# yoxu515/aot-benchmark

Hardware: NVIDIA H100
Metric: frames/sec (480p, 10 obj) (higher is better)
Workload: dtype f32

## Files before the change

### aot_benchmark_b200/csrc/conv_tc.cu

```cuda
#include <type_traits>

#include "common.cuh"
#include "tc_common.cuh"

namespace aotb {
namespace tc {

constexpr int CONV_A_BYTES = 128 * 128;

template <int BN>
__device__ __forceinline__ void wgmma_conv(float* acc, uint64_t a, uint64_t b) {
    if (BN == 256) wgmma_ss_n256(acc, a, b, 1u);
    else if (BN == 128) wgmma_ss_n128(acc, a, b, 1u);
    else wgmma_ss_n64(acc, a, b, 1u);
}

template <int BN>
__device__ __forceinline__ void conv_acc_to_staging(const float* acc, float* stg, int ld) {
    const int warp = threadIdx.x >> 5, lane = threadIdx.x & 31;
    const int row0 = (warp >> 2) * 64 + (warp & 3) * 16 + (lane >> 2), cq = (lane & 3) * 2;
#pragma unroll
    for (int j = 0; j < BN / 2; j += 2)
        *reinterpret_cast<float2*>(stg + (row0 + 8 * ((j >> 1) & 1)) * ld + 8 * (j >> 2) + cq) = make_float2(acc[j], acc[j + 1]);
}

struct ConvTcArgs {
    const float* in;
    const float* bias;
    const float* wscale;
    const float* res;
    float* out;
    int B, H, W, Cin, ldin;
    int Ho, Wo, Cout, ldout, ldres;
    int KH, KW, stride, pad;
    int M, mtiles, nchunks;
    int act;
    int splits;
    int spin;
    int const_w;
    long long* prof;
};

constexpr int AOTB_CONV_CONST_WEIGHTS = 256;
static int g_conv_tiling = 0;
static int g_conv_grid_cap = 0;

struct RowInfo { int pix_base, iy0, ix0, valid; };

template <int BN, int S, int NB>
__device__ __forceinline__ void conv_finish_tile(const ConvTcArgs& a, const uint8_t* smem, int tid, int m0, int n0, int zrank) {
    constexpr int LD = BN + 4, C4 = BN / 4, RSTEP = 256 / C4, ROWS = 128 / S, ITERS = ROWS / RSTEP;
    constexpr int B = NB < ITERS ? NB : ITERS;
    static_assert(ITERS >= 1 && ITERS % B == 0, "finish tiling");
    const int c = (tid % C4) * 4, n = n0 + c;
    const int r0 = zrank * ROWS + tid / C4;
    const float4 b4 = a.bias ? __ldg(reinterpret_cast<const float4*>(a.bias + n)) : make_float4(0.f, 0.f, 0.f, 0.f);
    const float4 s4 = a.wscale ? __ldg(reinterpret_cast<const float4*>(a.wscale + n)) : make_float4(1.f, 1.f, 1.f, 1.f);
    const float* lbase = reinterpret_cast<const float*>(smem) + r0 * LD + c;
    const uint32_t sbase = smem_u32(lbase);
#pragma unroll 1
    for (int i0 = 0; i0 < ITERS; i0 += B) {
        float4 v[B][S], rs[B];
#pragma unroll
        for (int b = 0; b < B; ++b) {
            const int ro = (i0 + b) * RSTEP;
            if (S == 1) {
                v[b][0] = *reinterpret_cast<const float4*>(lbase + ro * LD);
            } else {
#pragma unroll
                for (int z = 0; z < S; ++z) v[b][z] = dsmem_ld_f4(dsmem_addr(sbase + (uint32_t)(ro * LD) * 4u, (uint32_t)z));
            }
            const int m = m0 + r0 + ro;
            rs[b] = (a.res && m < a.M) ? *reinterpret_cast<const float4*>(a.res + (size_t)m * a.ldres + n)
                                       : make_float4(0.f, 0.f, 0.f, 0.f);
        }
#pragma unroll
        for (int b = 0; b < B; ++b) {
            float4 o = v[b][0];
#pragma unroll
            for (int z = 1; z < S; ++z) { o.x += v[b][z].x; o.y += v[b][z].y; o.z += v[b][z].z; o.w += v[b][z].w; }
            o.x = fmaf(o.x, s4.x, b4.x); o.y = fmaf(o.y, s4.y, b4.y); o.z = fmaf(o.z, s4.z, b4.z); o.w = fmaf(o.w, s4.w, b4.w);
            o.x += rs[b].x; o.y += rs[b].y; o.z += rs[b].z; o.w += rs[b].w;
            o.x = apply_act(o.x, a.act); o.y = apply_act(o.y, a.act);
            o.z = apply_act(o.z, a.act); o.w = apply_act(o.w, a.act);
            const int m = m0 + r0 + (i0 + b) * RSTEP;
            if (m < a.M) *reinterpret_cast<float4*>(a.out + (size_t)m * a.ldout + n) = o;
        }
    }
}

__device__ __forceinline__ void prefetch_l1(const void* p) { asm volatile("prefetch.global.L1 [%0];" ::"l"(p)); }

template <int BN, int ACT>
__device__ __forceinline__ void conv_finish_frag(const ConvTcArgs& a, float* acc, const float* bs, int m0, int n0) {
    constexpr bool ROLL = ACT == ACT_GELU || ACT == ACT_SILU;
    constexpr int G = (ROLL || BN == 256) ? 1 : 8, NG = BN / 8, PF = 8;
    const int warp = threadIdx.x >> 5, lane = threadIdx.x & 31;
    const int r = m0 + (warp >> 2) * 64 + (warp & 3) * 16 + (lane >> 2);
    const int c = (lane & 3) * 2;
    const bool ok[2] = {r < a.M, r + 8 < a.M};
    auto res_at = [&](int h, int k) { return a.res + (size_t)(r + 8 * h) * a.ldres + n0 + c + 8 * k; };
    auto prefetch = [&](int k) {
        if (G == 1 && a.res && k < NG) {
            if (ok[0]) prefetch_l1(res_at(0, k));
            if (ok[1]) prefetch_l1(res_at(1, k));
        }
    };
    auto group = [&](int k, int h, float a0, float a1, float2 rs) {
        const int n = c + 8 * k;
        const float2 b2 = *reinterpret_cast<const float2*>(bs + n), s2 = *reinterpret_cast<const float2*>(bs + BN + n);
        float ox = fmaf(a0, s2.x, b2.x), oy = fmaf(a1, s2.y, b2.y);
        ox += rs.x; oy += rs.y;
        ox = apply_act(ox, ACT); oy = apply_act(oy, ACT);
        if (ok[h]) *reinterpret_cast<float2*>(a.out + (size_t)(r + 8 * h) * a.ldout + n0 + n) = make_float2(ox, oy);
    };
#pragma unroll
    for (int k = 0; k < PF; ++k) prefetch(k);
    if constexpr (ROLL) {
#pragma unroll 1
        for (int k = 0; k < NG; ++k) {
            prefetch(k + PF);
            float2 rs[2];
#pragma unroll
            for (int h = 0; h < 2; ++h)
                rs[h] = (a.res && ok[h]) ? *reinterpret_cast<const float2*>(res_at(h, k)) : make_float2(0.f, 0.f);
#pragma unroll
            for (int h = 0; h < 2; ++h) group(k, h, acc[2 * h], acc[2 * h + 1], rs[h]);
#pragma unroll
            for (int i = 0; i < BN / 2 - 4; ++i) acc[i] = acc[i + 4];
        }
    } else {
#pragma unroll
        for (int k0 = 0; k0 < NG; k0 += G) {
            prefetch(k0 + PF);
            float2 rs[G][2];
#pragma unroll
            for (int k = 0; k < G; ++k)
#pragma unroll
                for (int h = 0; h < 2; ++h)
                    rs[k][h] = (a.res && ok[h]) ? *reinterpret_cast<const float2*>(res_at(h, k0 + k)) : make_float2(0.f, 0.f);
#pragma unroll
            for (int k = 0; k < G; ++k)
#pragma unroll
                for (int h = 0; h < 2; ++h) group(k0 + k, h, acc[4 * (k0 + k) + 2 * h], acc[4 * (k0 + k) + 2 * h + 1], rs[k][h]);
        }
    }
}

template <int BN, int STAGES, bool SPLIT, bool PERSIST>
struct ConvSmem {
    static constexpr int A_BYTES = CONV_A_BYTES;
    static constexpr int B_BYTES = BN * 128;
    static constexpr int PARTS = SPLIT ? 2 : 1;
    static constexpr int STAGE_BYTES = PARTS * A_BYTES + PARTS * B_BYTES;
    static constexpr int STG_LD = BN + 4;
    static_assert(128 * STG_LD * 4 <= STAGES * STAGE_BYTES, "staging tile must fit in the operand stages");
    static constexpr int RTABLES = PERSIST ? 2 : 1, BS_FLOATS = PERSIST ? 2 * 2 * BN : 0;
    static constexpr int TOTAL = STAGES * STAGE_BYTES + RTABLES * 128 * (int)sizeof(RowInfo) + BS_FLOATS * 4 + 3 * STAGES * 8 + 1024;
    static_assert(TOTAL <= 227 * 1024, "shared memory of one CTA");
};

template <int BN, int STAGES, bool SPLIT, bool PERSIST>
__global__ void __launch_bounds__(384, 1)
conv_tc_kernel(const __grid_constant__ CUtensorMap tmWh, const __grid_constant__ CUtensorMap tmWl, const ConvTcArgs a) {
    using SM = ConvSmem<BN, STAGES, SPLIT, PERSIST>;
    extern __shared__ uint8_t smem_raw[];
    uint8_t* smem = reinterpret_cast<uint8_t*>((reinterpret_cast<uintptr_t>(smem_raw) + 1023) & ~(uintptr_t)1023);
    RowInfo* rinfo = reinterpret_cast<RowInfo*>(smem + STAGES * SM::STAGE_BYTES);
    float* bsm = reinterpret_cast<float*>(rinfo + SM::RTABLES * 128);
    uint64_t* a_full = reinterpret_cast<uint64_t*>(bsm + SM::BS_FLOATS);
    uint64_t* b_full = a_full + STAGES;
    uint64_t* s_free = b_full + STAGES;

    const int tid = threadIdx.x, warp = tid >> 5;
    const int ntn = a.Cout / BN, ntiles = a.mtiles * ntn;
    const int ntc = !PERSIST ? 1 : (int)blockIdx.x < ntiles ? (ntiles - 1 - (int)blockIdx.x) / (int)gridDim.x + 1 : 0;
    auto tile_m0 = [&](int j) {
        if constexpr (PERSIST) return ((int)(blockIdx.x + j * gridDim.x) / ntn) * 128;
        else return (int)blockIdx.x * 128;
    };
    auto tile_n0 = [&](int j) {
        if constexpr (PERSIST) return ((int)(blockIdx.x + j * gridDim.x) % ntn) * BN;
        else return (int)blockIdx.y * BN;
    };
    long long* prof = a.prof ? a.prof + 12 * ((size_t)(blockIdx.z * gridDim.y + blockIdx.y) * gridDim.x + blockIdx.x) : nullptr;
    auto stamp = [&](int slot) { if (prof) prof[slot] = clock64(); };
    if (tid == 0) stamp(0);
    pdl_trigger();

    const int per = PERSIST ? a.nchunks : (a.nchunks + a.splits - 1) / a.splits;
    const int kbeg = PERSIST ? 0 : blockIdx.z * per;
    const int nloc = max(0, min(per, a.nchunks - kbeg));
    const int nchk = ntc * nloc;
    const int npre = a.const_w ? min(STAGES, nchk) : 0;
    auto issue_b = [&](int g) {
        const int j = PERSIST ? g / nloc : 0, it = g - j * nloc, s = g % STAGES;
        uint8_t* Bh = smem + s * SM::STAGE_BYTES + SM::PARTS * SM::A_BYTES;
        mbar_arrive_expect_tx(&b_full[s], SM::PARTS * SM::B_BYTES);
        tma_load_2d(Bh, &tmWh, &b_full[s], (kbeg + it) * 64, tile_n0(j));
        if constexpr (SPLIT) tma_load_2d(Bh + SM::B_BYTES, &tmWl, &b_full[s], (kbeg + it) * 64, tile_n0(j));
    };
    auto write_rows = [&](int j, int p) {
        const int m = tile_m0(j) + p;
        RowInfo ri;
        if (m < a.M) {
            const int HoWo = a.Ho * a.Wo;
            const int b = m / HoWo, r = m - b * HoWo;
            const int oy = r / a.Wo, ox = r - oy * a.Wo;
            ri.pix_base = b * a.H * a.W;
            ri.iy0 = oy * a.stride - a.pad;
            ri.ix0 = ox * a.stride - a.pad;
            ri.valid = 1;
        } else {
            ri.pix_base = 0; ri.iy0 = 0; ri.ix0 = 0; ri.valid = 0;
        }
        rinfo[(j & 1) * 128 + p] = ri;
    };

    if (tid == 0) {
        for (int s = 0; s < STAGES; ++s) { mbar_init(&a_full[s], 128); mbar_init(&b_full[s], 1); mbar_init(&s_free[s], 8); }
        fence_mbar_init();
    }
    if (tid >= 256) {
        for (int j = 0; j < min(ntc, 2); ++j) write_rows(j, tid - 256);
    }
    __syncthreads();
    if (tid == 0) stamp(1);
    if (tid == 256) {
        tma_prefetch_desc(&tmWh);
        if constexpr (SPLIT) tma_prefetch_desc(&tmWl);
        for (int g = 0; g < npre; ++g) issue_b(g);
    }
    pdl_wait();
    const int cpt = (a.Cin % 64 == 0) ? (a.Cin >> 6) : 0;

    const int wg = __shfl_sync(0xffffffffu, tid >> 7, 0);
    if (wg < 2) {
        const uint64_t dA0 = smem_desc_sw128(smem_u32(smem + wg * 64 * 128));
        const uint64_t dB0 = smem_desc_sw128(smem_u32(smem + SM::PARTS * SM::A_BYTES));
        int g = 0;
#pragma unroll 1
        for (int j = 0; j < ntc; ++j) {
            float acc[BN / 2];
#pragma unroll
            for (int i = 0; i < BN / 2; ++i) acc[i] = 0.f;
            float* bs = bsm + (j & 1) * 2 * BN;
            if (PERSIST && tid < BN) {
                const int n = tile_n0(j) + tid;
                bs[tid] = a.bias ? __ldg(a.bias + n) : 0.f;
                bs[BN + tid] = a.wscale ? __ldg(a.wscale + n) : 1.f;
            }
#pragma unroll 1
            for (int it = 0; it < nloc; ++it, ++g) {
                const int s = g % STAGES;
                const uint32_t ph = (g / STAGES) & 1;
                mbar_wait_cp(&a_full[s], ph, a.spin);
                mbar_wait_cp(&b_full[s], ph, a.spin);
                if (g == 0 && tid == 0) stamp(3);
                const uint64_t so = (uint64_t)((s * SM::STAGE_BYTES) >> 4);
                const uint64_t ah = dA0 + so, al = ah + (SM::A_BYTES >> 4), bh = dB0 + so, bl = bh + (uint64_t)(SM::B_BYTES >> 4);
                reg_fence<BN / 2>(acc);
                wgmma_fence();
#pragma unroll
                for (int ks = 0; ks < 4; ++ks) {
                    wgmma_conv<BN>(acc, ah + 2 * ks, bh + 2 * ks);
                    if constexpr (SPLIT) {
                        wgmma_conv<BN>(acc, al + 2 * ks, bh + 2 * ks);
                        wgmma_conv<BN>(acc, ah + 2 * ks, bl + 2 * ks);
                    }
                }
                wgmma_commit();
                reg_fence<BN / 2>(acc);
                wgmma_wait<1>();
                if (it > 0) mbar_arrive_warp(&s_free[(g - 1) % STAGES]);
            }
            wgmma_wait<0>();
            reg_fence<BN / 2>(acc);
            if (tid == 0) { if (PERSIST && j == 0) stamp(10); stamp(4); }
            if constexpr (PERSIST) {
                if (nloc > 0) mbar_arrive_warp(&s_free[(g - 1) % STAGES]);
                asm volatile("bar.sync 1, 256;" ::: "memory");
                const int m0 = tile_m0(j), n0 = tile_n0(j);
                switch (a.act) {
                    case ACT_RELU: conv_finish_frag<BN, ACT_RELU>(a, acc, bs, m0, n0); break;
                    case ACT_GELU: conv_finish_frag<BN, ACT_GELU>(a, acc, bs, m0, n0); break;
                    case ACT_SILU: conv_finish_frag<BN, ACT_SILU>(a, acc, bs, m0, n0); break;
                    case ACT_RELU6: conv_finish_frag<BN, ACT_RELU6>(a, acc, bs, m0, n0); break;
                    default: conv_finish_frag<BN, ACT_NONE>(a, acc, bs, m0, n0); break;
                }
                if (tid == 0) { if (j == 0) stamp(8); stamp(9); }
            } else {
                asm volatile("bar.sync 1, 256;" ::: "memory");
                conv_acc_to_staging<BN>(acc, reinterpret_cast<float*>(smem), SM::STG_LD);
                if (tid == 0) stamp(6);
            }
        }
    } else {
        const int p = tid - 256, q = p & 15, rsub = p >> 4;
        const uint32_t soff = rsub * 128 + (((q >> 1) ^ rsub) << 4) + ((q & 1) << 3);
        const float4* in4 = reinterpret_cast<const float4*>(a.in);
        uint32_t off[16];
        int cur_tap = -1, c4 = 0;
        const RowInfo* rows = rinfo;
        auto load_half = [&](int h, auto part_c, float4* v) {
            constexpr int part = decltype(part_c)::value;
            if (part == 0) {
                const int g = h >> 1, j = PERSIST ? g / nloc : 0, it = g - j * nloc;
                if (PERSIST && it == 0) {
                    cur_tap = -1;
                    rows = rinfo + (j & 1) * 128;
                    if (j > 0) {
                        asm volatile("bar.sync 2, 128;" ::: "memory");
                        if (j + 1 < ntc) write_rows(j + 1, p);
                    }
                }
                const int kc = kbeg + it;
                int tap, c0;
                if (cpt > 0) { tap = kc / cpt; c0 = ((kc - tap * cpt) << 6) + q * 4; }
                else { const int k = kc * 64 + q * 4; tap = k / a.Cin; c0 = k - tap * a.Cin; }
                c4 = c0 >> 2;
                if (tap != cur_tap) {
                    cur_tap = tap;
                    const bool kvalid = tap < a.KH * a.KW;
                    const int ky = tap / a.KW, kx = tap - ky * a.KW;
#pragma unroll
                    for (int i = 0; i < 16; ++i) {
                        const RowInfo ri = rows[rsub + i * 8];
                        const int iy = ri.iy0 + ky, ix = ri.ix0 + kx;
                        off[i] = (kvalid && ri.valid && iy >= 0 && iy < a.H && ix >= 0 && ix < a.W)
                                     ? (uint32_t)(((size_t)(ri.pix_base + iy * a.W + ix) * a.ldin) >> 2)
                                     : ~0u;
                    }
                }
            }
#pragma unroll
            for (int i = 0; i < 8; ++i) {
                const uint32_t o = off[part * 8 + i];
                v[i] = o != ~0u ? __ldg(in4 + ((size_t)o + c4)) : make_float4(0.f, 0.f, 0.f, 0.f);
            }
        };
        auto store_half = [&](int h, auto part_c, const float4* v) {
            constexpr int part = decltype(part_c)::value;
            const int g = h >> 1, s = g % STAGES;
            uint8_t* stage = smem + s * SM::STAGE_BYTES;
            if (part == 0) {
                if (g >= STAGES) mbar_wait_cp(&s_free[s], ((g / STAGES) - 1) & 1, a.spin);
                if (p == 0 && g >= npre) issue_b(g);
            }
            uint8_t* Ah = stage + part * 64 * 128 + soff;
            uint8_t* Al = Ah + SM::A_BYTES;
#pragma unroll
            for (int i = 0; i < 8; ++i) {
                const __half2 h0 = __floats2half2_rn(v[i].x, v[i].y), h1 = __floats2half2_rn(v[i].z, v[i].w);
                if constexpr (!SPLIT) {
                    uint2 ph;
                    ph.x = *reinterpret_cast<const uint32_t*>(&h0); ph.y = *reinterpret_cast<const uint32_t*>(&h1);
                    *reinterpret_cast<uint2*>(Ah + i * 1024) = ph;
                    continue;
                }
                const __half2 l0 = __floats2half2_rn(v[i].x - __low2float(h0), v[i].y - __high2float(h0));
                const __half2 l1 = __floats2half2_rn(v[i].z - __low2float(h1), v[i].w - __high2float(h1));
                uint2 ph, pl;
                ph.x = *reinterpret_cast<const uint32_t*>(&h0); ph.y = *reinterpret_cast<const uint32_t*>(&h1);
                pl.x = *reinterpret_cast<const uint32_t*>(&l0); pl.y = *reinterpret_cast<const uint32_t*>(&l1);
                *reinterpret_cast<uint2*>(Ah + i * 1024) = ph;
                *reinterpret_cast<uint2*>(Al + i * 1024) = pl;
            }
            if (part == 1) {
                fence_proxy_async();
                mbar_arrive(&a_full[s]);
                if (g == 0 && p == 0) stamp(2);
            }
        };
        using P0 = std::integral_constant<int, 0>;
        using P1 = std::integral_constant<int, 1>;
        const int nh = 2 * nchk;
        float4 v0[8], v1[8], v2[8];
        if (nh > 0) { load_half(0, P0{}, v0); load_half(1, P1{}, v1); }
#pragma unroll 1
        for (int h = 0; h < nh; h += 6) {
            if (h + 2 < nh) load_half(h + 2, P0{}, v2);
            store_half(h, P0{}, v0);
            if (h + 3 < nh) load_half(h + 3, P1{}, v0);
            store_half(h + 1, P1{}, v1);
            if (h + 2 < nh) {
                if (h + 4 < nh) load_half(h + 4, P0{}, v1);
                store_half(h + 2, P0{}, v2);
                if (h + 5 < nh) load_half(h + 5, P1{}, v2);
                store_half(h + 3, P1{}, v0);
            }
            if (h + 4 < nh) {
                if (h + 6 < nh) load_half(h + 6, P0{}, v0);
                store_half(h + 4, P0{}, v1);
                if (h + 7 < nh) load_half(h + 7, P1{}, v1);
                store_half(h + 5, P1{}, v2);
            }
        }
        if (p == 0) stamp(5);
    }
    if constexpr (!PERSIST) {
        __syncwarp();
        cluster_sync_all();
        if (tid == 0) stamp(8);
        if (warp < 8) {
            const int zr = (int)blockIdx.z, m0 = tile_m0(0), n0 = tile_n0(0);
            if (a.splits == 2) conv_finish_tile<BN, 2, 4>(a, smem, tid, m0, n0, zr);
            else if (a.splits == 4) conv_finish_tile<BN, 4, 2>(a, smem, tid, m0, n0, zr);
            else conv_finish_tile<BN, 8, 2>(a, smem, tid, m0, n0, zr);
        }
        if (tid == 0) stamp(9);
        __syncwarp();
        cluster_sync_all();
    } else if (tid == 0 && prof) {
        prof[11] = ntc;
    }
    if (tid == 0) stamp(7);
}

static int make_tmap_weights(CUtensorMap* out, const void* base, int Kpad, int Cout, int BN) {
    PFN_encodeTiled fn = tensor_map_encoder();
    if (!fn) return AOTB_ERR_CUDA;
    cuuint64_t dims[2] = {(cuuint64_t)Kpad, (cuuint64_t)Cout};
    cuuint64_t strides[1] = {(cuuint64_t)Kpad * 2};
    cuuint32_t box[2] = {64, (cuuint32_t)BN};
    cuuint32_t estr[2] = {1, 1};
    CUresult r = fn(out, CU_TENSOR_MAP_DATA_TYPE_FLOAT16, 2, const_cast<void*>(base), dims, strides, box, estr,
                    CU_TENSOR_MAP_INTERLEAVE_NONE, CU_TENSOR_MAP_SWIZZLE_128B, CU_TENSOR_MAP_L2_PROMOTION_L2_256B,
                    CU_TENSOR_MAP_FLOAT_OOB_FILL_NONE);
    if (r != CUDA_SUCCESS) {
        set_error("cuTensorMapEncodeTiled(weights) failed (%d)", (int)r);
        return AOTB_ERR_CUDA;
    }
    return AOTB_OK;
}

static int sm_count() {
    static int n = 0;
    if (n == 0) {
        int dev = 0;
        if (cudaGetDevice(&dev) != cudaSuccess || cudaDeviceGetAttribute(&n, cudaDevAttrMultiProcessorCount, dev) != cudaSuccess)
            n = 132;
    }
    return n;
}

static dim3 conv_grid(const ConvTcArgs& a, int BN) {
    if (a.splits > 1) return dim3(a.mtiles, a.Cout / BN, a.splits);
    const int cap = g_conv_grid_cap > 0 ? g_conv_grid_cap : sm_count();
    return dim3(min(a.mtiles * (a.Cout / BN), cap), 1, 1);
}

template <int BN, int STAGES, bool SPLIT, bool PERSIST>
static int launch_conv_tc_as(const CUtensorMap& th, const CUtensorMap& tl, const ConvTcArgs& a, cudaStream_t st) {
    constexpr int smem = ConvSmem<BN, STAGES, SPLIT, PERSIST>::TOTAL;
    static bool configured = false;
    if (!configured) {
        cudaError_t e = cudaFuncSetAttribute(conv_tc_kernel<BN, STAGES, SPLIT, PERSIST>,
                                             cudaFuncAttributeMaxDynamicSharedMemorySize, smem);
        if (e != cudaSuccess) {
            set_error("aotb_conv2d_nhwc_tc: cudaFuncSetAttribute: %s", cudaGetErrorString(e));
            return AOTB_ERR_CUDA;
        }
        configured = true;
    }
    launch_cluster(conv_tc_kernel<BN, STAGES, SPLIT, PERSIST>, conv_grid(a, BN), dim3(384), smem, st, a.splits, th, tl, a);
    return check_launch("aotb_conv2d_nhwc_tc");
}

template <int BN, int STAGES, bool SPLIT>
static int launch_conv_tc(const CUtensorMap& th, const CUtensorMap& tl, const ConvTcArgs& a, cudaStream_t st) {
    return a.splits > 1 ? launch_conv_tc_as<BN, STAGES, SPLIT, false>(th, tl, a, st)
                        : launch_conv_tc_as<BN, STAGES, SPLIT, true>(th, tl, a, st);
}

}
}

using namespace aotb;

extern "C" int aotb_set_conv_tiling(int mode) {
    AOTB_REQUIRE(mode >= 0 && mode < (1 << 12), "aotb_set_conv_tiling: mode is a 12-bit mask");
    tc::g_conv_tiling = mode;
    return AOTB_OK;
}

extern "C" int aotb_set_conv_grid_cap(int ctas) {
    AOTB_REQUIRE(ctas >= 0, "aotb_set_conv_grid_cap: negative cap");
    tc::g_conv_grid_cap = ctas;
    return AOTB_OK;
}

extern "C" int aotb_conv2d_nhwc_tc(const float* in, const void* wh, const void* wl, const float* bias, const float* wscale,
                                   const float* res, float* out, int B, int H, int W, int Cin, int ldin, int Cout, int ldout, int ldres,
                                   int KH, int KW, int stride, int pad, int act, void* workspace, size_t workspace_bytes,
                                   void* stream) {
    AOTB_REQUIRE(in && wh && out, "aotb_conv2d_nhwc_tc: null pointer");
    const bool split = wl != nullptr;
    const int const_w = (act & tc::AOTB_CONV_CONST_WEIGHTS) ? 1 : 0;
    act &= ~tc::AOTB_CONV_CONST_WEIGHTS;
    AOTB_REQUIRE(Cin % 4 == 0 && Cout % 64 == 0, "aotb_conv2d_nhwc_tc: Cin must be a multiple of 4, Cout of 64");
    AOTB_REQUIRE(act >= aotb::ACT_NONE && act <= aotb::ACT_RELU6, "aotb_conv2d_nhwc_tc: activation %d not supported (0-4)", act);
    AOTB_REQUIRE(ldin % 4 == 0 && ldout % 4 == 0 && (!res || ldres % 4 == 0) && ((uintptr_t)in % 16 == 0) &&
                     ((uintptr_t)out % 16 == 0) && (!res || (uintptr_t)res % 16 == 0) && (!bias || (uintptr_t)bias % 16 == 0) &&
                     (!wscale || (uintptr_t)wscale % 16 == 0),
                 "aotb_conv2d_nhwc_tc: 16-byte alignment required");
    AOTB_REQUIRE((size_t)B * H * W * ldin / 4 < 0xFFFFFFFFull, "aotb_conv2d_nhwc_tc: input larger than 2^32 float4");
    tc::ConvTcArgs a;
    a.in = in; a.bias = bias; a.wscale = wscale; a.res = res; a.out = out;
    a.B = B; a.H = H; a.W = W; a.Cin = Cin; a.ldin = ldin;
    a.Ho = (H + 2 * pad - KH) / stride + 1;
    a.Wo = (W + 2 * pad - KW) / stride + 1;
    AOTB_REQUIRE(a.Ho > 0 && a.Wo > 0, "aotb_conv2d_nhwc_tc: empty output");
    a.Cout = Cout; a.ldout = ldout; a.ldres = ldres; a.KH = KH; a.KW = KW; a.stride = stride; a.pad = pad;
    a.M = B * a.Ho * a.Wo;
    a.mtiles = cdiv(a.M, 128);
    const int K = ((KH * KW * Cin + 63) / 64) * 64;
    a.nchunks = K / 64;
    a.act = act;
    a.const_w = const_w;
    const int mt = cdiv(a.M, 128);
    int BN = 64, best_s = 1;
    const float kGather = 2.5f, kGather1 = 2.0f;
    if ((tc::g_conv_tiling & 1) == 0) {
        float best = 1e30f;
        const int bns[3] = {256, 128, 64};
        const float t_mma[3] = {4.0f, 2.0f, 1.0f}, t_mma1[3] = {4.0f / 3, 2.0f / 3, 1.0f / 3};
        const float t_fin[3] = {8.0f, 4.0f, 2.0f};
        for (int bi = 0; bi < 3; ++bi) {
            const float tf = t_fin[bi] * (bi == 0 && res ? 2.0f : 1.0f);
            if (Cout % bns[bi]) continue;
            const float tm = split ? t_mma[bi] : t_mma1[bi], tc = fmaxf(split ? kGather : kGather1, tm);
            for (int sp = 1; sp <= 8; sp <<= 1) {
                if (sp > a.nchunks) break;
                const int ctas = mt * (Cout / bns[bi]) * sp;
                const int slots = sp == 8 ? 128 : 132;
                if (sp > 1 && ctas > slots) continue;
                float t;
                if (sp == 1) {
                    const int tpc = cdiv(ctas, 132);
                    t = 3.0f + tpc * a.nchunks * tc + tf + (tpc - 1) * fmaxf(0.f, a.nchunks * (tm - tc) + tf);
                } else {
                    t = cdiv(ctas, slots) * (3.0f + cdiv(a.nchunks, sp) * tc + t_fin[bi]);
                }
                if (t < best) { best = t; BN = bns[bi]; best_s = sp; }
            }
        }
    } else {
        if (Cout % 128 == 0 && mt * (Cout / 128) >= 120) BN = 128;
        const int ctas = mt * (Cout / BN);
        if (ctas < 100 && a.nchunks >= 4) {
            best_s = 8;
            while (best_s > 1 && (ctas * best_s > 160 || a.nchunks / best_s < 2)) best_s >>= 1;
        }
    }
    const int force_bn = (tc::g_conv_tiling >> 4) & 15, force_s = (tc::g_conv_tiling >> 8) & 15;
    if (force_bn) {
        BN = 32 << force_bn;
        AOTB_REQUIRE((BN == 64 || BN == 128 || BN == 256) && Cout % BN == 0, "aotb_conv2d_nhwc_tc: forced tile %d invalid", BN);
    }
    a.splits = force_bn ? 1 : best_s;
    if (force_s) {
        AOTB_REQUIRE((force_s == 1 || force_s == 2 || force_s == 4 || force_s == 8) && force_s <= a.nchunks,
                     "aotb_conv2d_nhwc_tc: forced split %d invalid", force_s);
        a.splits = force_s;
    }
    a.spin = (tc::g_conv_tiling & 2) ? 1 : 0;
    a.prof = nullptr;
    if (tc::g_conv_tiling & 4) {
        const dim3 grid = tc::conv_grid(a, BN);
        const size_t need = (size_t)grid.x * grid.y * grid.z * 12 * sizeof(long long);
        AOTB_REQUIRE(workspace && workspace_bytes >= need, "aotb_conv2d_nhwc_tc: profile mode needs %zu workspace bytes", need);
        a.prof = (long long*)workspace;
    }
    CUtensorMap th, tl;
    int rc;
    if ((rc = tc::make_tmap_weights(&th, wh, K, Cout, BN)) != AOTB_OK) return rc;
    cudaStream_t st = (cudaStream_t)stream;
    if (!split) {
        if (BN == 256) return tc::launch_conv_tc<256, 4, false>(th, th, a, st);
        if (BN == 128) return tc::launch_conv_tc<128, 6, false>(th, th, a, st);
        return tc::launch_conv_tc<64, 8, false>(th, th, a, st);
    }
    if ((rc = tc::make_tmap_weights(&tl, wl, K, Cout, BN)) != AOTB_OK) return rc;
    if (BN == 256) return tc::launch_conv_tc<256, 2, true>(th, tl, a, st);
    if (BN == 128) return tc::launch_conv_tc<128, 3, true>(th, tl, a, st);
    return tc::launch_conv_tc<64, 4, true>(th, tl, a, st);
}
```

### aot_benchmark_b200/csrc/tc_common.cuh

```cuda
#pragma once
#include <cuda.h>
#include <cuda_fp16.h>
#include <cuda_runtime.h>
#include <cstdint>

namespace aotb {
namespace tc {

__device__ __forceinline__ uint32_t smem_u32(const void* p) { return (uint32_t)__cvta_generic_to_shared(p); }

__device__ __forceinline__ bool elect_one() {
    uint32_t pred;
    asm volatile(
        "{\n\t.reg .pred P;\n\telect.sync _|P, 0xffffffff;\n\tselp.b32 %0, 1, 0, P;\n\t}\n" : "=r"(pred));
    return pred != 0;
}

__device__ __forceinline__ void mbar_init(uint64_t* bar, uint32_t count) {
    asm volatile("mbarrier.init.shared::cta.b64 [%0], %1;" ::"r"(smem_u32(bar)), "r"(count) : "memory");
}
__device__ __forceinline__ void fence_mbar_init() { asm volatile("fence.mbarrier_init.release.cluster;" ::: "memory"); }
__device__ __forceinline__ void mbar_arrive_warp(uint64_t* bar) {
    __syncwarp();
    if ((threadIdx.x & 31) == 0) asm volatile("mbarrier.arrive.shared::cta.b64 _, [%0];" ::"r"(smem_u32(bar)) : "memory");
}
__device__ __forceinline__ void mbar_arrive(uint64_t* bar) {
    asm volatile("mbarrier.arrive.shared::cta.b64 _, [%0];" ::"r"(smem_u32(bar)) : "memory");
}
__device__ __forceinline__ void mbar_arrive_expect_tx(uint64_t* bar, uint32_t bytes) {
    asm volatile("mbarrier.arrive.expect_tx.shared::cta.b64 _, [%0], %1;" ::"r"(smem_u32(bar)), "r"(bytes) : "memory");
}
__device__ __forceinline__ void mbar_wait(uint64_t* bar, uint32_t parity) {
    const uint32_t addr = smem_u32(bar);
    uint32_t done = 0;
    uint32_t spins = 0;
    while (true) {
        asm volatile(
            "{\n\t.reg .pred P;\n\tmbarrier.try_wait.parity.shared::cta.b64 P, [%1], %2, %3;\n\tselp.b32 %0, 1, 0, P;\n\t}\n"
            : "=r"(done)
            : "r"(addr), "r"(parity), "r"(20000u)
            : "memory");
        if (done) break;
        if (++spins > (1u << 24)) __trap();
    }
}

__device__ __forceinline__ void mbar_wait_spin(uint64_t* bar, uint32_t parity) {
    const uint32_t addr = smem_u32(bar);
    uint32_t done = 0;
    uint32_t spins = 0;
    while (true) {
        asm volatile(
            "{\n\t.reg .pred P;\n\tmbarrier.try_wait.parity.shared::cta.b64 P, [%1], %2;\n\tselp.b32 %0, 1, 0, P;\n\t}\n"
            : "=r"(done)
            : "r"(addr), "r"(parity)
            : "memory");
        if (done) break;
        if (++spins > (1u << 28)) __trap();
    }
}

__device__ __forceinline__ void mbar_wait_cp(uint64_t* bar, uint32_t parity, int spin) {
    if (spin) mbar_wait_spin(bar, parity);
    else mbar_wait(bar, parity);
}

__device__ __forceinline__ void tma_prefetch_desc(const CUtensorMap* m) {
    asm volatile("prefetch.tensormap [%0];" ::"l"(reinterpret_cast<uint64_t>(m)) : "memory");
}
__device__ __forceinline__ void tma_load_2d(void* dst, const CUtensorMap* m, uint64_t* bar, int c0, int c1) {
    asm volatile(
        "cp.async.bulk.tensor.2d.shared::cluster.global.mbarrier::complete_tx::bytes [%0], [%1, {%3, %4}], [%2];"
        ::"r"(smem_u32(dst)), "l"(reinterpret_cast<uint64_t>(m)), "r"(smem_u32(bar)), "r"(c0), "r"(c1)
        : "memory");
}
__device__ __forceinline__ void tma_load_3d(void* dst, const CUtensorMap* m, uint64_t* bar, int c0, int c1, int c2) {
    asm volatile(
        "cp.async.bulk.tensor.3d.shared::cluster.global.mbarrier::complete_tx::bytes [%0], [%1, {%3, %4, %5}], [%2];"
        ::"r"(smem_u32(dst)), "l"(reinterpret_cast<uint64_t>(m)), "r"(smem_u32(bar)), "r"(c0), "r"(c1), "r"(c2)
        : "memory");
}
__device__ __forceinline__ void fence_proxy_async() { asm volatile("fence.proxy.async.shared::cta;" ::: "memory"); }

__device__ __forceinline__ uint64_t smem_desc_sw128(uint32_t saddr) {
    uint64_t d = 0;
    d |= (uint64_t)((saddr & 0x3FFFF) >> 4);
    d |= (uint64_t)1 << 16;
    d |= (uint64_t)(1024 >> 4) << 32;
    d |= (uint64_t)1 << 62;
    return d;
}
__device__ __forceinline__ void wgmma_fence() { asm volatile("wgmma.fence.sync.aligned;" ::: "memory"); }
__device__ __forceinline__ void wgmma_commit() { asm volatile("wgmma.commit_group.sync.aligned;" ::: "memory"); }
template <int N>
__device__ __forceinline__ void wgmma_wait() { asm volatile("wgmma.wait_group.sync.aligned %0;" ::"n"(N) : "memory"); }
template <int R>
__device__ __forceinline__ void reg_fence(float* d) {
#pragma unroll
    for (int i = 0; i < R; ++i) asm volatile("" : "+f"(d[i])::"memory");
}

__device__ __forceinline__ void wgmma_ss_n64(float* d, uint64_t a_desc, uint64_t b_desc, uint32_t scale_d) {
    asm volatile(
        "{\n\t.reg .pred p;\n\tsetp.ne.b32 p, %34, 0;\n\t"
        "wgmma.mma_async.sync.aligned.m64n64k16.f32.f16.f16 "
        "{%0, %1, %2, %3, %4, %5, %6, %7, %8, %9, %10, %11, %12, %13, %14, %15, "
        "%16, %17, %18, %19, %20, %21, %22, %23, %24, %25, %26, %27, %28, %29, %30, %31}, "
        "%32, %33, p, 1, 1, 0, 0;\n\t}\n"
        : "+f"(d[0]), "+f"(d[1]), "+f"(d[2]), "+f"(d[3]), "+f"(d[4]), "+f"(d[5]), "+f"(d[6]), "+f"(d[7]),
          "+f"(d[8]), "+f"(d[9]), "+f"(d[10]), "+f"(d[11]), "+f"(d[12]), "+f"(d[13]), "+f"(d[14]), "+f"(d[15]),
          "+f"(d[16]), "+f"(d[17]), "+f"(d[18]), "+f"(d[19]), "+f"(d[20]), "+f"(d[21]), "+f"(d[22]), "+f"(d[23]),
          "+f"(d[24]), "+f"(d[25]), "+f"(d[26]), "+f"(d[27]), "+f"(d[28]), "+f"(d[29]), "+f"(d[30]), "+f"(d[31])
        : "l"(a_desc), "l"(b_desc), "r"(scale_d));
}

__device__ __forceinline__ void wgmma_ss_n128(float* d, uint64_t a_desc, uint64_t b_desc, uint32_t scale_d) {
    asm volatile(
        "{\n\t.reg .pred p;\n\tsetp.ne.b32 p, %66, 0;\n\t"
        "wgmma.mma_async.sync.aligned.m64n128k16.f32.f16.f16 "
        "{%0, %1, %2, %3, %4, %5, %6, %7, %8, %9, %10, %11, %12, %13, %14, %15, "
        "%16, %17, %18, %19, %20, %21, %22, %23, %24, %25, %26, %27, %28, %29, %30, %31, "
        "%32, %33, %34, %35, %36, %37, %38, %39, %40, %41, %42, %43, %44, %45, %46, %47, "
        "%48, %49, %50, %51, %52, %53, %54, %55, %56, %57, %58, %59, %60, %61, %62, %63}, "
        "%64, %65, p, 1, 1, 0, 0;\n\t}\n"
        : "+f"(d[0]), "+f"(d[1]), "+f"(d[2]), "+f"(d[3]), "+f"(d[4]), "+f"(d[5]), "+f"(d[6]), "+f"(d[7]),
          "+f"(d[8]), "+f"(d[9]), "+f"(d[10]), "+f"(d[11]), "+f"(d[12]), "+f"(d[13]), "+f"(d[14]), "+f"(d[15]),
          "+f"(d[16]), "+f"(d[17]), "+f"(d[18]), "+f"(d[19]), "+f"(d[20]), "+f"(d[21]), "+f"(d[22]), "+f"(d[23]),
          "+f"(d[24]), "+f"(d[25]), "+f"(d[26]), "+f"(d[27]), "+f"(d[28]), "+f"(d[29]), "+f"(d[30]), "+f"(d[31]),
          "+f"(d[32]), "+f"(d[33]), "+f"(d[34]), "+f"(d[35]), "+f"(d[36]), "+f"(d[37]), "+f"(d[38]), "+f"(d[39]),
          "+f"(d[40]), "+f"(d[41]), "+f"(d[42]), "+f"(d[43]), "+f"(d[44]), "+f"(d[45]), "+f"(d[46]), "+f"(d[47]),
          "+f"(d[48]), "+f"(d[49]), "+f"(d[50]), "+f"(d[51]), "+f"(d[52]), "+f"(d[53]), "+f"(d[54]), "+f"(d[55]),
          "+f"(d[56]), "+f"(d[57]), "+f"(d[58]), "+f"(d[59]), "+f"(d[60]), "+f"(d[61]), "+f"(d[62]), "+f"(d[63])
        : "l"(a_desc), "l"(b_desc), "r"(scale_d));
}

__device__ __forceinline__ void wgmma_ss_n256(float* d, uint64_t a_desc, uint64_t b_desc, uint32_t scale_d) {
    asm volatile(
        "{\n\t.reg .pred p;\n\tsetp.ne.b32 p, %130, 0;\n\t"
        "wgmma.mma_async.sync.aligned.m64n256k16.f32.f16.f16 "
        "{%0, %1, %2, %3, %4, %5, %6, %7, %8, %9, %10, %11, %12, %13, %14, %15, "
        "%16, %17, %18, %19, %20, %21, %22, %23, %24, %25, %26, %27, %28, %29, %30, %31, "
        "%32, %33, %34, %35, %36, %37, %38, %39, %40, %41, %42, %43, %44, %45, %46, %47, "
        "%48, %49, %50, %51, %52, %53, %54, %55, %56, %57, %58, %59, %60, %61, %62, %63, "
        "%64, %65, %66, %67, %68, %69, %70, %71, %72, %73, %74, %75, %76, %77, %78, %79, "
        "%80, %81, %82, %83, %84, %85, %86, %87, %88, %89, %90, %91, %92, %93, %94, %95, "
        "%96, %97, %98, %99, %100, %101, %102, %103, %104, %105, %106, %107, %108, %109, %110, %111, "
        "%112, %113, %114, %115, %116, %117, %118, %119, %120, %121, %122, %123, %124, %125, %126, %127}, "
        "%128, %129, p, 1, 1, 0, 0;\n\t}\n"
        : "+f"(d[0]), "+f"(d[1]), "+f"(d[2]), "+f"(d[3]), "+f"(d[4]), "+f"(d[5]), "+f"(d[6]), "+f"(d[7]),
          "+f"(d[8]), "+f"(d[9]), "+f"(d[10]), "+f"(d[11]), "+f"(d[12]), "+f"(d[13]), "+f"(d[14]), "+f"(d[15]),
          "+f"(d[16]), "+f"(d[17]), "+f"(d[18]), "+f"(d[19]), "+f"(d[20]), "+f"(d[21]), "+f"(d[22]), "+f"(d[23]),
          "+f"(d[24]), "+f"(d[25]), "+f"(d[26]), "+f"(d[27]), "+f"(d[28]), "+f"(d[29]), "+f"(d[30]), "+f"(d[31]),
          "+f"(d[32]), "+f"(d[33]), "+f"(d[34]), "+f"(d[35]), "+f"(d[36]), "+f"(d[37]), "+f"(d[38]), "+f"(d[39]),
          "+f"(d[40]), "+f"(d[41]), "+f"(d[42]), "+f"(d[43]), "+f"(d[44]), "+f"(d[45]), "+f"(d[46]), "+f"(d[47]),
          "+f"(d[48]), "+f"(d[49]), "+f"(d[50]), "+f"(d[51]), "+f"(d[52]), "+f"(d[53]), "+f"(d[54]), "+f"(d[55]),
          "+f"(d[56]), "+f"(d[57]), "+f"(d[58]), "+f"(d[59]), "+f"(d[60]), "+f"(d[61]), "+f"(d[62]), "+f"(d[63]),
          "+f"(d[64]), "+f"(d[65]), "+f"(d[66]), "+f"(d[67]), "+f"(d[68]), "+f"(d[69]), "+f"(d[70]), "+f"(d[71]),
          "+f"(d[72]), "+f"(d[73]), "+f"(d[74]), "+f"(d[75]), "+f"(d[76]), "+f"(d[77]), "+f"(d[78]), "+f"(d[79]),
          "+f"(d[80]), "+f"(d[81]), "+f"(d[82]), "+f"(d[83]), "+f"(d[84]), "+f"(d[85]), "+f"(d[86]), "+f"(d[87]),
          "+f"(d[88]), "+f"(d[89]), "+f"(d[90]), "+f"(d[91]), "+f"(d[92]), "+f"(d[93]), "+f"(d[94]), "+f"(d[95]),
          "+f"(d[96]), "+f"(d[97]), "+f"(d[98]), "+f"(d[99]), "+f"(d[100]), "+f"(d[101]), "+f"(d[102]), "+f"(d[103]),
          "+f"(d[104]), "+f"(d[105]), "+f"(d[106]), "+f"(d[107]), "+f"(d[108]), "+f"(d[109]), "+f"(d[110]), "+f"(d[111]),
          "+f"(d[112]), "+f"(d[113]), "+f"(d[114]), "+f"(d[115]), "+f"(d[116]), "+f"(d[117]), "+f"(d[118]), "+f"(d[119]),
          "+f"(d[120]), "+f"(d[121]), "+f"(d[122]), "+f"(d[123]), "+f"(d[124]), "+f"(d[125]), "+f"(d[126]), "+f"(d[127])
        : "l"(a_desc), "l"(b_desc), "r"(scale_d));
}

__device__ __forceinline__ void wgmma_rs_n64_tb(float* d, const uint32_t* a, uint64_t b_desc) {
    asm volatile(
        "{\n\t.reg .pred p;\n\tsetp.ne.b32 p, 1, 0;\n\t"
        "wgmma.mma_async.sync.aligned.m64n64k16.f32.f16.f16 "
        "{%0, %1, %2, %3, %4, %5, %6, %7, %8, %9, %10, %11, %12, %13, %14, %15, "
        "%16, %17, %18, %19, %20, %21, %22, %23, %24, %25, %26, %27, %28, %29, %30, %31}, "
        "{%32, %33, %34, %35}, %36, p, 1, 1, 1;\n\t}\n"
        : "+f"(d[0]), "+f"(d[1]), "+f"(d[2]), "+f"(d[3]), "+f"(d[4]), "+f"(d[5]), "+f"(d[6]), "+f"(d[7]),
          "+f"(d[8]), "+f"(d[9]), "+f"(d[10]), "+f"(d[11]), "+f"(d[12]), "+f"(d[13]), "+f"(d[14]), "+f"(d[15]),
          "+f"(d[16]), "+f"(d[17]), "+f"(d[18]), "+f"(d[19]), "+f"(d[20]), "+f"(d[21]), "+f"(d[22]), "+f"(d[23]),
          "+f"(d[24]), "+f"(d[25]), "+f"(d[26]), "+f"(d[27]), "+f"(d[28]), "+f"(d[29]), "+f"(d[30]), "+f"(d[31])
        : "r"(a[0]), "r"(a[1]), "r"(a[2]), "r"(a[3]), "l"(b_desc));
}


__device__ __forceinline__ float ex2(float x) {
    float y;
    asm("ex2.approx.ftz.f32 %0, %1;" : "=f"(y) : "f"(x));
    return y;
}
__device__ __forceinline__ uint32_t cvt_h2(float lo, float hi) {
    uint32_t r;
    asm("cvt.rn.f16x2.f32 %0, %1, %2;" : "=r"(r) : "f"(hi), "f"(lo));
    return r;
}

__device__ __forceinline__ void cluster_sync_all() {
    asm volatile("barrier.cluster.arrive.release.aligned;\n\tbarrier.cluster.wait.acquire.aligned;" ::: "memory");
}
__device__ __forceinline__ uint32_t dsmem_addr(uint32_t local_saddr, uint32_t cta_rank) {
    uint32_t r;
    asm volatile("mapa.shared::cluster.u32 %0, %1, %2;" : "=r"(r) : "r"(local_saddr), "r"(cta_rank));
    return r;
}
__device__ __forceinline__ float4 dsmem_ld_f4(uint32_t cluster_saddr) {
    float4 v;
    asm volatile("ld.shared::cluster.v4.f32 {%0, %1, %2, %3}, [%4];"
                 : "=f"(v.x), "=f"(v.y), "=f"(v.z), "=f"(v.w)
                 : "r"(cluster_saddr));
    return v;
}

typedef CUresult (*PFN_encodeTiled)(CUtensorMap*, CUtensorMapDataType, cuuint32_t, void*, const cuuint64_t*,
                                    const cuuint64_t*, const cuuint32_t*, const cuuint32_t*, CUtensorMapInterleave,
                                    CUtensorMapSwizzle, CUtensorMapL2promotion, CUtensorMapFloatOOBfill);
PFN_encodeTiled tensor_map_encoder();

int make_tmap_rows64(CUtensorMap* out, const void* base, int rows, int heads, int box_rows);

}
}
```

### aot_benchmark_b200/engine.py

```python
from __future__ import annotations

import functools
import math

import numpy as np
import torch
import torch.nn as nn

from . import ops
from .plan import get_plan

A_NONE, A_RELU, A_GELU, A_SILU, A_RELU6 = ops.ACT_NONE, ops.ACT_RELU, ops.ACT_GELU, ops.ACT_SILU, ops.ACT_RELU6
A_HSWISH = ops.ACT_HSWISH

LT_PROBE = None
import os as _os
LT_IMPL = _os.environ.get("AOTB_LT_IMPL", "tc_exact")
LOCAL_IMPL = _os.environ.get("AOTB_LOCAL_IMPL", "tile")
DEAOT_LT = _os.environ.get("AOTB_DEAOT_LT", "tc")
SHARD_XCHG = _os.environ.get("AOTB_SHARD_XCHG", "nccl")
SHARD_SMAX = 16
SUB_ENGINE_STREAMS = _os.environ.get("AOTB_SUB_ENGINE_STREAMS", "1") == "1"
SHARD_GRAPHS = _os.environ.get("AOTB_SHARD_GRAPHS", "1") == "1"


def _symm_alloc(numel, device, group):
    import torch.distributed as dist
    import torch.distributed._symmetric_memory as symm_mem
    t = symm_mem.empty(numel, dtype=torch.float32, device=device)
    hdl = symm_mem.rendezvous(t, group if group is not None else dist.group.WORLD)
    return hdl, (lambda r, sizes, off: hdl.get_buffer(r, sizes, torch.float32, off))


GEMM_GROW_FRAMES = int(_os.environ.get("AOTB_GEMM_GROW_FRAMES", "8"))
_LT_NAMES = {"simt": "attn_f32_kernel<32,32> (fp32 SIMT flash attention)",
             "tc_exact": "attn_tc_kernel<1,1> (wgmma fp16x2 exact: 6+8 MMAs per 64-key tile)",
             "tc_fast": "attn_tc_kernel<1,1> (wgmma fp16 fast: 2+4 MMAs per 64-key tile)"}
_DEAOT_LT_NAMES = {"simt": "attn_f32_kernel<128,256> (fp32 SIMT flash attention, DeAOT 1 x 128 / 1024 head)",
                   "gemm": "conv_tc_kernel (Q K^T) -> row_softmax_kernel -> conv_tc_kernel (P V): wgmma GEMMs over split-fp16 "
                           "copies of the bank (deaot_lt.cu)",
                   "tc": "attn_tc_kernel<4,2> (fused wgmma flash attention, 128 queries x 64 value channels per CTA)"}


def deaot_lt_kernel_name():
    return _DEAOT_LT_NAMES.get(DEAOT_LT, DEAOT_LT)


LT_KERNEL_NAME = _LT_NAMES.get(LT_IMPL, LT_IMPL) + (f", layout '{ops.LT_VARIANT}'" if LT_IMPL.startswith("tc") else "")


USE_GRAPHS = _os.environ.get("AOTB_GRAPHS", "1") == "1"
USE_PDL = _os.environ.get("AOTB_PDL", "1") == "1"
CONV_TILING = _os.environ.get("AOTB_CONV_TILING", "model")
_CONV_TILING_MASK = {"model": 0, "narrow": 1}


def _apply_pdl():
    from ._lib import lib, check
    lib().aotb_set_pdl(1 if USE_PDL else 0)
    check(lib().aotb_set_conv_tiling(_CONV_TILING_MASK[CONV_TILING]), "aotb_set_conv_tiling")
BANK_INIT_FRAMES = int(_os.environ.get("AOTB_BANK_FRAMES", "24"))


def _resolve_mem_max(aot_model, long_term_mem_max):
    m = getattr(aot_model.cfg, "TEST_LONG_TERM_MEM_MAX", None) if long_term_mem_max is None else long_term_mem_max
    if m is None:
        return None
    if int(m) != m or m < 2:
        raise ValueError(f"long_term_mem_max must be an integer >= 2 (the first memory frame and at least one recent one), got {m}")
    return int(m)


MEM_POLICIES = ("fifo", "usage")
USAGE_MAX_SLOTS = 32


def _resolve_mem_policy(aot_model, policy, mem_max):
    p = getattr(aot_model.cfg, "TEST_LONG_TERM_MEM_POLICY", None) if policy is None else policy
    if p is None:
        return "fifo"
    if p not in MEM_POLICIES:
        raise ValueError(f"long_term_mem_policy must be one of {MEM_POLICIES}, got {p!r}")
    if p == "usage":
        if mem_max is None:
            raise ValueError("long_term_mem_policy='usage' chooses which frame a full bounded bank evicts; it needs "
                             "long_term_mem_max (or cfg.TEST_LONG_TERM_MEM_MAX)")
        if mem_max > USAGE_MAX_SLOTS:
            raise NotImplementedError(f"long_term_mem_policy='usage' counts at most {USAGE_MAX_SLOTS} memory slots, "
                                      f"got long_term_mem_max={mem_max}")
        if aot_model.cfg.MODEL_VOS == "deaot":
            if DEAOT_LT != "tc":
                raise NotImplementedError(f"long_term_mem_policy='usage' counts attention mass in DeAOT's fused tensor-core "
                                          f"attention; AOTB_DEAOT_LT={DEAOT_LT} selects another path")
        elif LT_IMPL == "simt":
            raise NotImplementedError("long_term_mem_policy='usage' counts attention mass in the tensor-core long-term "
                                      "attention; AOTB_LT_IMPL=simt selects the fp32 CUDA-core kernel")
        elif ops.LT_VARIANT != "tile":
            raise NotImplementedError(f"long_term_mem_policy='usage' runs the default 'tile' layout of the tensor-core "
                                      f"long-term attention; AOTB_LT_VARIANT={ops.LT_VARIANT} selects another")
    return p


def _resolve_precision(aot_model, precision):
    p = getattr(aot_model.cfg, "TEST_PRECISION", None) if precision is None else precision
    if p is None:
        return "fp32"
    if p not in ops.PRECISIONS:
        raise ValueError(f"precision must be one of {ops.PRECISIONS}, got {p!r}")
    if p == "fp16":
        if ops.CONV_IMPL == "simt":
            raise NotImplementedError("precision='fp16' runs the tensor-core conv; AOTB_CONV_IMPL=simt selects the fp32 "
                                      "CUDA-core conv")
        if LT_IMPL == "simt":
            raise NotImplementedError("precision='fp16' runs the tensor-core long-term attention; AOTB_LT_IMPL=simt selects "
                                      "the fp32 CUDA-core kernel")
        if aot_model.cfg.MODEL_VOS == "deaot" and DEAOT_LT in ("gemm", "simt"):
            raise NotImplementedError(f"precision='fp16' runs DeAOT's attention on the fused tensor-core kernel; "
                                      f"AOTB_DEAOT_LT={DEAOT_LT} selects another path")
    return p


def _in_precision(fn):
    @functools.wraps(fn)
    def wrapper(self, *args, **kwargs):
        with ops.precision(self.precision):
            return fn(self, *args, **kwargs)
    return wrapper


REPLAYED_KERNELS = [0]


class GraphCache:

    def __init__(self):
        self.slots = {}

    def clear(self):
        self.slots.clear()

    def run(self, key, fn, enabled=True):
        if not (enabled and USE_GRAPHS and LT_PROBE is None):
            return fn()
        slot = self.slots.get(key)
        if slot is None:
            slot = self.slots[key] = [0, None, None]
        if slot[1] is not None:
            slot[1].replay()
            REPLAYED_KERNELS[0] += slot[3]
            return slot[2]
        if slot[0] < 1:
            slot[0] += 1
            return fn()
        from ._lib import lib
        n0 = lib().aotb_launch_count()
        g = torch.cuda.CUDAGraph()
        with torch.cuda.graph(g):
            out = fn()
        n_kernels = int(lib().aotb_launch_count() - n0)
        g.replay()
        slot[1], slot[2] = g, out
        slot.append(n_kernels)
        return out


def _cur_stream():
    return torch.cuda.current_stream().cuda_stream


def fork_join(owner, items, fn):
    if len(items) == 1 or not SUB_ENGINE_STREAMS:
        return [fn(i, x) for i, x in enumerate(items)]
    cur = torch.cuda.current_stream()
    side = getattr(owner, "_side_streams", [])
    while len(side) < len(items) - 1:
        side.append(torch.cuda.Stream())
    owner._side_streams = side
    side = side[: len(items) - 1]
    for s in side:
        s.wait_stream(cur)
    outs = [None] * len(items)
    for i in range(1, len(items)):
        with torch.cuda.stream(side[i - 1]):
            outs[i] = fn(i, items[i])
    outs[0] = fn(0, items[0])
    for s in side:
        cur.wait_stream(s)
    return outs


def lt_splits(n_queries, heads, tk, sms=132, variant=None):
    pair = (ops.LT_VARIANT if variant is None else variant) == "pair"
    qrows, slots = (64, 2 * sms) if pair else (128, sms)
    base = ((n_queries + qrows - 1) // qrows) * heads
    tiles = (tk + 127) // 128
    effs = []
    for s in range(1, 17):
        if s > 1 and tiles < 2 * s:
            break
        ctas = base * s
        effs.append((s, ctas / (((ctas + slots - 1) // slots) * slots)))
    top = max(e for _, e in effs)
    return next(s for s, e in effs if e >= top - 0.05)


def _pos_emb_sine(h, w, npf=128):
    y = torch.arange(h, dtype=torch.float32).view(h, 1).expand(h, w)
    x = torch.arange(w, dtype=torch.float32).view(1, w).expand(h, w)
    eps = 1e-6
    y = y / (y[-1:, :] + eps) * (2 * math.pi)
    x = x / (x[:, -1:] + eps) * (2 * math.pi)
    dim_t = torch.arange(npf, dtype=torch.float32)
    dim_t = 10000 ** (2 * (dim_t // 2) / npf)
    px = x[:, :, None] / dim_t
    py = y[:, :, None] / dim_t
    px = torch.stack((px[..., 0::2].sin(), px[..., 1::2].cos()), dim=3).flatten(2)
    py = torch.stack((py[..., 0::2].sin(), py[..., 1::2].cos()), dim=3).flatten(2)
    return torch.cat((py, px), dim=2).reshape(h * w, 2 * npf).contiguous()


class EncEmbs(list):
    nhwc = None


class _Encoder:
    def __init__(self, plan, H, W):
        self.plan = plan
        self.H, self.W = H, W
        dev = plan.device
        self.bufs = {}
        self.dev = dev

    def _buf(self, key, shape):
        b = self.bufs.get(key)
        if b is None or tuple(b.shape) != tuple(shape):
            b = torch.empty(shape, dtype=torch.float32, device=self.dev)
            self.bufs[key] = b
        return b

    @staticmethod
    def _osz(n, k, s, p, d=1):
        return (n + 2 * p - d * (k - 1) - 1) // s + 1

    def __call__(self, img, st):
        P = self.plan
        if img.dim() != 4 or img.shape[0] != 1 or img.shape[1] != 3:
            raise ValueError("expected an image tensor [1,3,H,W]")
        if P.encoder_name == "swin_base" and (img.shape[2] % 4 or img.shape[3] % 4):
            img = torch.nn.functional.pad(img, (0, -img.shape[3] % 4, 0, -img.shape[2] % 4))
        H, W = img.shape[2], img.shape[3]
        if getattr(self, "_gkey", None) != (id(P), H, W):
            self.graphs = GraphCache()
            self._gkey = (id(P), H, W)
        x = self._buf("in", (1, H, W, 4))
        ops.image_to_nhwc4(img.float(), x, stream=st)
        nhwc = self.graphs.run("enc", lambda: self._body(x))
        out = EncEmbs(t.permute(0, 3, 1, 2) for t in nhwc)
        out.nhwc = nhwc
        return out

    def _body(self, x):
        P = self.plan
        st = _cur_stream()
        if P.encoder_name in ("resnet50", "resnet101"):
            feats = self._resnet(x, st)
        elif P.encoder_name in ("resnest50", "resnest101"):
            feats = self._resnest(x, st)
        elif P.encoder_name == "swin_base":
            feats = self._swin(x, st)
        elif P.encoder_name == "mobilenetv3":
            feats = self._mobilenetv3(x, st)
        else:
            feats = self._mobilenet(x, st)
        f16 = feats[-1]
        proj = self._buf("proj", (1, f16.shape[1], f16.shape[2], P.C))
        ops.conv2d(f16, P.proj.w, P.proj.b, proj, stream=st)
        return [feats[0], feats[1], feats[2], proj]

    def _resnet(self, x, st):
        e = self.plan.enc
        H, W = x.shape[1], x.shape[2]
        h1, w1 = self._osz(H, 7, 2, 3), self._osz(W, 7, 2, 3)
        c1 = self._buf("stem", (1, h1, w1, 64))
        ops.conv2d(x, e.stem.w, e.stem.b, c1, KH=7, KW=7, stride=2, pad=3, act=A_RELU, stream=st)
        h, w = self._osz(h1, 3, 2, 1), self._osz(w1, 3, 2, 1)
        cur = self._buf("pool", (1, h, w, 64))
        ops.maxpool3x3s2(c1, cur, stream=st)
        feats = []
        for si, blocks in enumerate(e.stages):
            for bi, b in enumerate(blocks):
                ho, wo = self._osz(h, 3, b.stride, 1), self._osz(w, 3, b.stride, 1)
                t1 = self._buf(f"s{si}b{bi}t1", (1, h, w, b.c1.cout))
                ops.conv2d(cur, b.c1.w, b.c1.b, t1, act=A_RELU, stream=st)
                t2 = self._buf(f"s{si}b{bi}t2", (1, ho, wo, b.c2.cout))
                ops.conv2d(t1, b.c2.w, b.c2.b, t2, KH=3, KW=3, stride=b.stride, pad=1, act=A_RELU, stream=st)
                if b.down is not None:
                    res = self._buf(f"s{si}ds", (1, ho, wo, b.down.cout))
                    ops.conv2d(cur, b.down.w, b.down.b, res, stride=b.stride, stream=st)
                else:
                    res = cur
                out = self._buf(f"s{si}o{bi % 2}", (1, ho, wo, b.c3.cout))
                ops.conv2d(t2, b.c3.w, b.c3.b, out, res=res, act=A_RELU, stream=st)
                cur, h, w = out, ho, wo
            feats.append(cur)
        return feats

    def _resnest(self, x, st):
        e = self.plan.enc
        H, W = x.shape[1], x.shape[2]
        h, w = self._osz(H, 3, 2, 1), self._osz(W, 3, 2, 1)
        s0 = self._buf("stem0", (1, h, w, e.stem[0].cout))
        ops.conv2d(x, e.stem[0].w, e.stem[0].b, s0, KH=3, KW=3, stride=2, pad=1, act=A_RELU, stream=st)
        s1 = self._buf("stem1", (1, h, w, e.stem[1].cout))
        ops.conv2d(s0, e.stem[1].w, e.stem[1].b, s1, KH=3, KW=3, pad=1, act=A_RELU, stream=st)
        s2 = self._buf("stem2", (1, h, w, e.stem[2].cout))
        ops.conv2d(s1, e.stem[2].w, e.stem[2].b, s2, KH=3, KW=3, pad=1, act=A_RELU, stream=st)
        h, w = self._osz(h, 3, 2, 1), self._osz(w, 3, 2, 1)
        cur = self._buf("pool", (1, h, w, s2.shape[3]))
        ops.maxpool3x3s2(s2, cur, stream=st)
        ws = self.bufs.get("splat_ws")
        if ws is None:
            ws = self.bufs["splat_ws"] = ops.splat_workspace(max(b.gw for blocks in e.stages for b in blocks), self.dev)
        feats = []
        for si, blocks in enumerate(e.stages):
            for bi, b in enumerate(blocks):
                gw, s = b.gw, b.stride
                ho, wo = (ops.pool2d_size(h, 3, s, 1), ops.pool2d_size(w, 3, s, 1)) if s > 1 else (h, w)
                t1 = self._buf(f"s{si}b{bi}t1", (1, h, w, gw))
                ops.conv2d(cur, b.c1.w, b.c1.b, t1, act=A_RELU, stream=st)
                t2 = self._buf(f"s{si}b{bi}t2", (1, h, w, 2 * gw))
                for g, cg in enumerate(b.groups):
                    ops.conv2d(t1[..., g * gw // 2:(g + 1) * gw // 2], cg.w, cg.b, t2[..., g * gw:(g + 1) * gw], KH=3, KW=3,
                               pad=1, act=A_RELU, stream=st)
                att = self._buf(f"s{si}b{bi}att", (2 * gw,))
                ops.splat_attention(t2, b.fc1_w, b.fc1_b, b.fc2_w, b.fc2_b, att, ws, stream=st)
                comb = self._buf(f"s{si}b{bi}sum", (1, ho, wo, gw))
                ops.splat_combine(t2, att, comb, pool_stride=s if s > 1 else 0, stream=st)
                if b.down is not None:
                    dsrc = cur
                    if s > 1:
                        dsrc = self._buf(f"s{si}dp", (1, ops.pool2d_size(h, s, s, 0, True), ops.pool2d_size(w, s, s, 0, True),
                                                      cur.shape[3]))
                        ops.avgpool(cur, dsrc, s, s, 0, ceil_mode=True, count_include_pad=False, stream=st)
                    res = self._buf(f"s{si}ds", (1, ho, wo, b.down.cout))
                    ops.conv2d(dsrc, b.down.w, b.down.b, res, stream=st)
                else:
                    res = cur
                out = self._buf(f"s{si}o{bi % 2}", (1, ho, wo, b.c3.cout))
                ops.conv2d(comb, b.c3.w, b.c3.b, out, res=res, act=A_RELU, stream=st)
                cur, h, w = out, ho, wo
            feats.append(cur)
        return feats

    def _swin(self, x4, st):
        e = self.plan.enc
        H, W, C = x4.shape[1] // 4, x4.shape[2] // 4, e.embed
        pe = self._buf("pe", (1, H, W, C))
        ops.conv2d(x4, e.patch.w, e.patch.b, pe, KH=4, KW=4, stride=4, pad=0, stream=st)
        x = self._buf("s0x", (H * W, C))
        ops.layernorm(pe.view(H * W, C), e.patch_norm[0], e.patch_norm[1], x, stream=st)
        feats = []
        for si, stg in enumerate(e.stages):
            N = H * W
            ln = self._buf(f"s{si}ln", (N, C))
            qkv = self._buf(f"s{si}qkv", (N, 3 * C))
            att = self._buf(f"s{si}att", (N, C))
            hid = self._buf(f"s{si}hid", (N, 4 * C))
            for b in stg.blocks:
                ops.layernorm(x, b.norm1[0], b.norm1[1], ln, stream=st)
                ops.linear(ln, b.qkv_w, b.qkv_b, qkv, stream=st)
                ops.window_attention(qkv, b.qkv_b, b.relb, att, H, W, stg.heads, b.shift, window=e.window, stream=st)
                ops.linear(att, b.proj_w, b.proj_b, x, res=x, stream=st)
                ops.layernorm(x, b.norm2[0], b.norm2[1], ln, stream=st)
                ops.linear(ln, b.fc1_w, b.fc1_b, hid, act=A_GELU, stream=st)
                ops.linear(hid, b.fc2_w, b.fc2_b, x, res=x, stream=st)
            f = self._buf(f"s{si}f", (1, H, W, C))
            ops.layernorm(x, stg.norm[0], stg.norm[1], f.view(N, C), stream=st)
            feats.append(f)
            if stg.down is not None:
                H2, W2 = (H + 1) // 2, (W + 1) // 2
                mg = self._buf(f"s{si}mg", (H2 * W2, 4 * C))
                ops.patch_merge(x, mg, H, W, stream=st)
                mln = self._buf(f"s{si}mln", (H2 * W2, 4 * C))
                ops.layernorm(mg, stg.down.norm[0], stg.down.norm[1], mln, stream=st)
                x = self._buf(f"s{si + 1}x", (H2 * W2, 2 * C))
                ops.linear(mln, stg.down.w, stg.down.b, x, stream=st)
                H, W, C = H2, W2, 2 * C
        return feats

    def _mobilenetv3(self, x, st):
        e = self.plan.enc
        H, W = x.shape[1], x.shape[2]
        h, w = self._osz(H, 3, 2, 1), self._osz(W, 3, 2, 1)
        cur = self._buf("stem", (1, h, w, e.stem.cout))
        ops.conv2d(x, e.stem.w, e.stem.b, cur, KH=3, KW=3, stride=2, pad=1, act=A_HSWISH, stream=st)
        ws = self.bufs.get("se_ws")
        if ws is None:
            ws = self.bufs["se_ws"] = ops.splat_workspace(max(b.dw.cout for b in e.blocks if b.se is not None), self.dev)
        feats = []
        for i, b in enumerate(e.blocks):
            act = A_HSWISH if b.hs else A_RELU
            y = cur
            if b.expand is not None:
                t = self._buf(f"b{i}e", (1, h, w, b.expand.cout))
                ops.conv2d(y, b.expand.w, b.expand.b, t, act=act, stream=st)
                y = t
            pad = (b.k - 1) // 2 * b.dil
            ho, wo = self._osz(h, b.k, b.stride, pad, b.dil), self._osz(w, b.k, b.stride, pad, b.dil)
            t = self._buf(f"b{i}d", (1, ho, wo, b.dw.cout))
            ops.dwconv(y, b.dw.w, b.dw.b, t, K=b.k, stride=b.stride, pad=pad, dil=b.dil,
                       act=A_NONE if b.se is not None else act, stream=st)
            if b.se is not None:
                gate = self._buf(f"b{i}gate", (b.dw.cout,))
                ops.se_gate(t, b.se.w1, b.se.b1, b.se.w2, b.se.b2, gate, ws, stream=st)
                g = self._buf(f"b{i}g", (1, ho, wo, b.dw.cout))
                ops.gate_scale(t, gate, g, act=act, stream=st)
                t = g
            o = self._buf(f"b{i}o", (1, ho, wo, b.pw.cout))
            ops.conv2d(t, b.pw.w, b.pw.b, o, res=cur if b.res else None, stream=st)
            cur, h, w = o, ho, wo
            if b.tap:
                feats.append(cur)
        last = self._buf("last", (1, h, w, e.last.cout))
        ops.conv2d(cur, e.last.w, e.last.b, last, act=A_HSWISH, stream=st)
        feats.append(last)
        return feats

    def _mobilenet(self, x, st):
        e = self.plan.enc
        H, W = x.shape[1], x.shape[2]
        h, w = self._osz(H, 3, 2, 1), self._osz(W, 3, 2, 1)
        cur = self._buf("stem", (1, h, w, 32))
        ops.conv2d(x, e.stem.w, e.stem.b, cur, KH=3, KW=3, stride=2, pad=1, act=A_RELU6, stream=st)
        feats = []
        for i, b in enumerate(e.blocks):
            y = cur
            if b.expand is not None:
                t = self._buf(f"b{i}e", (1, h, w, b.expand.cout))
                ops.conv2d(y, b.expand.w, b.expand.b, t, act=A_RELU6, stream=st)
                y = t
            pad = b.dil
            ho, wo = self._osz(h, 3, b.stride, pad, b.dil), self._osz(w, 3, b.stride, pad, b.dil)
            t = self._buf(f"b{i}d", (1, ho, wo, b.dw.cout))
            ops.dwconv(y, b.dw.w, b.dw.b, t, K=3, stride=b.stride, pad=pad, dil=b.dil, act=A_RELU6, stream=st)
            o = self._buf(f"b{i}o", (1, ho, wo, b.pw.cout))
            ops.conv2d(t, b.pw.w, b.pw.b, o, res=cur if b.res else None, stream=st)
            cur, h, w = o, ho, wo
            if b.tap:
                feats.append(cur)
        last = self._buf("last", (1, h, w, e.last.cout))
        ops.conv2d(cur, e.last.w, e.last.b, last, act=A_RELU6, stream=st)
        feats.append(last)
        return feats


class AOTEngine(nn.Module):
    def __init__(self, aot_model, gpu_id=0, long_term_mem_gap=9999, short_term_mem_skip=1, long_term_mem_max=None,
                 precision=None, long_term_mem_policy=None):
        super().__init__()
        self.precision = _resolve_precision(aot_model, precision)
        self.cfg = aot_model.cfg
        self.align_corners = aot_model.cfg.MODEL_ALIGN_CORNERS
        self.AOT = aot_model
        self.max_obj_num = aot_model.max_obj_num
        self.gpu_id = gpu_id
        self.long_term_mem_gap = long_term_mem_gap
        self.short_term_mem_skip = short_term_mem_skip
        self.long_term_mem_max = _resolve_mem_max(aot_model, long_term_mem_max)
        self.long_term_mem_policy = _resolve_mem_policy(aot_model, long_term_mem_policy, self.long_term_mem_max)
        self.losses = None
        self._enc = None
        self._ws = None
        self._ws_key = None
        self._P = None
        self.graphs = GraphCache()
        self.tk_dev = None
        self.wr_dev = None
        self.kv_shard = None
        self.restart_engine()

    def forward(self, *args, **kwargs):
        raise NotImplementedError("training step (BASELINE config 5) is a 'next' row (SURVEY 8f); this engine "
                                  "implements the eval protocol")

    def restart_engine(self, batch_size=1, enable_id_shuffle=False):
        if batch_size != 1 or enable_id_shuffle:
            raise NotImplementedError("batch_size > 1 / id shuffle are training-only (SURVEY 8f)")
        self.batch_size = 1
        self.frame_step = 0
        self.last_mem_step = -1
        self.enable_id_shuffle = False
        self.freeze_id = False
        self.obj_nums = None
        self.pos_emb = None
        self.enc_size_2d = None
        self.enc_hw = None
        self.input_size_2d = None
        self.bank_len = 0
        self.enable_offline_enc = False
        self.curr_enc_embs = None
        self.curr_id_embs = None
        self.pred_id_logits = None
        self._have_lstt = False
        self._mem_frames = 0
        if self.tk_dev is not None:
            self.tk_dev.zero_()
            self.wr_dev.zero_()
        self._zero_usage()

    def _zero_usage(self):
        if getattr(self._ws, "usage_U", None) is not None:
            self._ws.usage_U.zero_()
            self._ws.usage_A.zero_()

    def _usage(self):
        return self.long_term_mem_policy == "usage" and self.long_term_mem_max is not None

    def enable_kv_sharding(self, rank, world, group=None):
        if self.precision == "fp16":
            raise NotImplementedError("a long-term bank sharded over GPUs is not built for precision='fp16'")
        if not (LT_IMPL.startswith("tc") and not self._plan_is_deaot()):
            raise NotImplementedError("sharded long-term attention is implemented for the AOT tensor-core kernel")
        if self.long_term_mem_max is not None:
            raise NotImplementedError("a bounded long-term bank (long_term_mem_max) cannot be sharded over GPUs: each rank "
                                      "would need its own ring")
        self.kv_shard = (int(rank), int(world), group)

    def _plan_is_deaot(self):
        return self.AOT.cfg.MODEL_VOS == "deaot"

    def update_size(self, input_size, enc_size):
        self.input_size_2d = tuple(int(s) for s in input_size)
        self.enc_size_2d = tuple(int(s) for s in enc_size)
        self.enc_hw = self.enc_size_2d[0] * self.enc_size_2d[1]

    def _plan(self):
        if self._P is None:
            self._P = get_plan(self.AOT)
        return self._P

    def _alloc(self):
        P = self._plan()
        dev = P.device
        N = self.enc_hw
        C = P.C
        L = P.L
        M = self.long_term_mem_max
        if M is not None and P.deaot and DEAOT_LT == "gemm":
            raise NotImplementedError("a bounded long-term bank (long_term_mem_max) is not built for AOTB_DEAOT_LT=gemm: its "
                                      "transposed value copies have no ring store; use the default fused kernel")
        usage = self._usage()
        key = (id(P), N, tuple(self.enc_size_2d), tuple(self.input_size_2d), LT_IMPL, DEAOT_LT, M, usage)
        if self._ws is not None and self._ws_key == key:
            self.bank_len = 0
            self.tk_dev.zero_()
            self.wr_dev.zero_()
            self._zero_usage()
            self._st_ring = []
            return
        self._ws_key = key
        self.graphs.clear()
        self.tk_dev = torch.zeros(1, dtype=torch.int32, device=dev)
        self.wr_dev = torch.zeros(1, dtype=torch.int32, device=dev)
        f = lambda *s: torch.empty(s, dtype=torch.float32, device=dev)
        ws = type("WS", (), {})()
        ws.N = N
        ws.gn_ws = ops.groupnorm_workspace(1, 32, dev)
        ws.id_emb = f(N, C)
        if not P.deaot:
            ws.x = f(N, C)
            ws.ln = f(N, C)
            ws.ln_pos = f(N, C)
            ws.qk = f(N, 2 * C)
            ws.v = f(N, C)
            ws.core = f(N, 2 * C)
            ws.tmp = f(N, C)
            ws.ff = f(N, 4 * C)
            ws.ff2 = f(N, 4 * C)
            ws.cat = f(N, (L + 1) * C)
            self.curr_Q = [f(N, C) for _ in range(L)]
            self.curr_V = [f(N, C) for _ in range(L)]
            self.st_K = [f(N, C) for _ in range(L)]
            self.st_V = [f(N, C) for _ in range(L)]
            self._kdim, self._vdim = C, C
        else:
            d = C // 2
            ws.xz = f(N, 2 * C)
            ws.ln = f(N, C)
            ws.qv = f(N, d + 2 * C)
            ws.catU = f(N, 4 * C)
            ws.idin = f(N, 2 * C)
            ws.core = f(N, 4 * C)
            ws.gated = f(N, 4 * C)
            ws.dw = f(N, 8 * C)
            ws.c = f(N, 2 * C)
            ws.sa_qk = f(N, d)
            ws.sa_v = f(N, 4 * C)
            ws.sa_u = f(N, 4 * C)
            ws.cat = f(N, 2 * C)
            self.curr_Q = [f(N, d) for _ in range(L)]
            self.curr_V = [f(N, 2 * C) for _ in range(L)]
            self.curr_IDV = [None] + [f(N, C) for _ in range(L - 1)]
            self.st_K = [f(N, d) for _ in range(L)]
            self.st_V = [f(N, 4 * C) for _ in range(L)]
            self._kdim, self._vdim = d, 4 * C
        ws.mask = f(*self.input_size_2d)
        self._dec_out = {}
        cap = (min(BANK_INIT_FRAMES, GEMM_GROW_FRAMES) if (P.deaot and DEAOT_LT == "gemm") else BANK_INIT_FRAMES) * N
        if M is not None:
            cap = M * N
        self.bank_cap = cap
        self.bank_K = [f(cap, self._kdim) for _ in range(L)]
        self.bank_V = [f(cap, self._vdim) for _ in range(L)]
        self.bank_len = 0
        self._gemm_lt = bool(P.deaot and DEAOT_LT == "gemm")
        if self._gemm_lt:
            self._alloc_gemm_lt(cap, ws=ws)
        self._gp_tc = bool(P.deaot and DEAOT_LT == "tc")
        if self._gp_tc:
            hz = lambda *s: torch.zeros(s, dtype=torch.float16, device=dev)
            ws.gpQp = hz(self._kdim // 32, ((N + 127) // 128) * 128, 64)
            ncap = ((N + 63) // 64) * 64 + 64
            ws.gpSaK = hz(self._kdim // 32, ncap, 64)
            ws.gpSaV = hz(self._vdim // 32, ncap, 64)
            self.bank_gpK = [hz(self._kdim // 32, cap, 64) for _ in range(L)]
            self.bank_gpV = [hz(self._vdim // 32, cap, 64) for _ in range(L)]
            ws.gp_part = {}
        self._tc = LT_IMPL.startswith("tc") and (not P.deaot) and (C // P.H == 32)
        if self._tc:
            hz = lambda *s: torch.zeros(s, dtype=torch.float16, device=dev)
            ws.Qp = hz(P.H, ((N + 255) // 256) * 256, 64)
            ws.saKp = hz(P.H, ((N + 127) // 128) * 128, 64)
            ws.saVp = hz(P.H, ((N + 127) // 128) * 128, 64)
            self.bank_Kp = [hz(P.H, cap, 64) for _ in range(L)]
            self.bank_Vp = [hz(P.H, cap, 64) for _ in range(L)]
            ws.part = {}
        if usage:
            if not (self._tc or self._gp_tc):
                raise NotImplementedError("long_term_mem_policy='usage' needs the tensor-core long-term attention, which "
                                          f"this model's head shape ({P.H} x {C // P.H}) does not run on")
            ws.usage_U = torch.zeros(M, dtype=torch.float32, device=dev)
            ws.usage_A = torch.zeros(M, dtype=torch.int32, device=dev)
            ws.usage_ws = ops.attn_merge_usage_workspace(M, dev)
            H, dv = (1, self._vdim) if P.deaot else (P.H, C)
            ws.usage_part = (f(M, N, dv), f(M, H, N), f(M, H, N))
        self._st_ring = []
        self._ws = ws
        self._dec_bufs = {}

    def _alloc_gemm_lt(self, cap, old_len=0, old=None, ws=None):
        P = self._plan()
        dev = P.device
        capw = ((cap + 63) // 64) * 64
        hz = lambda *s: torch.zeros(s, dtype=torch.float16, device=dev)
        Kh, Kl = [hz(capw, self._kdim) for _ in range(P.L)], [hz(capw, self._kdim) for _ in range(P.L)]
        Vh, Vl = [hz(self._vdim, capw) for _ in range(P.L)], [hz(self._vdim, capw) for _ in range(P.L)]
        if old is not None:
            for new_l, old_l in zip((Kh, Kl), old[:2]):
                for a, b in zip(new_l, old_l):
                    a[:old_len].copy_(b[:old_len])
            for new_l, old_l in zip((Vh, Vl), old[2:]):
                for a, b in zip(new_l, old_l):
                    a[:, :old_len].copy_(b[:, :old_len])
        self.bank_Kh, self.bank_Kl, self.bank_VhT, self.bank_VlT = Kh, Kl, Vh, Vl
        self._capw = capw
        (self._ws if ws is None else ws).S = torch.empty((self.enc_hw, capw), dtype=torch.float32, device=dev)

    def _bank_reserve(self, rows):
        if self.bank_len + rows <= self.bank_cap or self.long_term_mem_max is not None:
            return
        new_cap = max(2 * self.bank_cap, self.bank_len + rows)
        if getattr(self, "_gemm_lt", False):
            new_cap = max(self.bank_cap + GEMM_GROW_FRAMES * self.enc_hw, self.bank_len + rows)
        for lst in (self.bank_K, self.bank_V):
            for i, old in enumerate(lst):
                nb = torch.empty((new_cap, old.shape[1]), dtype=torch.float32, device=old.device)
                nb[: self.bank_len].copy_(old[: self.bank_len])
                lst[i] = nb
        if self._tc:
            for lst in (self.bank_Kp, self.bank_Vp):
                for i, old in enumerate(lst):
                    nb = torch.zeros((old.shape[0], new_cap, 64), dtype=torch.float16, device=old.device)
                    nb[:, : self.bank_len].copy_(old[:, : self.bank_len])
                    lst[i] = nb
        if getattr(self, "_gemm_lt", False):
            self._alloc_gemm_lt(new_cap, self.bank_len, (self.bank_Kh, self.bank_Kl, self.bank_VhT, self.bank_VlT))
        if getattr(self, "_gp_tc", False):
            for lst in (self.bank_gpK, self.bank_gpV):
                for i, old in enumerate(lst):
                    nb = torch.zeros((old.shape[0], new_cap, 64), dtype=torch.float16, device=old.device)
                    nb[:, : self.bank_len].copy_(old[:, : self.bank_len])
                    lst[i] = nb
        self.bank_cap = new_cap
        self.graphs.clear()

    @property
    def long_term_memories(self):
        if self.bank_len == 0:
            return None
        P = self._plan()
        n = self.bank_len
        out = []
        for li in range(P.L):
            K = self.bank_K[li][:n].unsqueeze(1)
            V = self.bank_V[li][:n]
            if P.deaot:
                c2 = 2 * P.C
                out.append([K, V[:, :c2].unsqueeze(1), None, V[:, c2:].unsqueeze(1)])
            else:
                out.append([K, V.unsqueeze(1)])
        return out

    @property
    def long_term_memory_usage(self):
        if not self._usage() or getattr(self._ws, "usage_U", None) is None:
            return None
        return self._ws.usage_U.clone(), self._ws.usage_A.clone()

    @property
    def short_term_memories(self):
        if not self._have_lstt:
            return None
        P = self._plan()
        h, w = self.enc_size_2d
        to2d = lambda t: t.view(h, w, 1, -1).permute(2, 3, 0, 1)
        out = []
        for li in range(P.L):
            if P.deaot:
                c2 = 2 * P.C
                out.append([to2d(self.st_K[li]), to2d(self.st_V[li][:, :c2]), None, to2d(self.st_V[li][:, c2:])])
            else:
                out.append([to2d(self.st_K[li]), to2d(self.st_V[li])])
        return out

    @_in_precision
    def _encode(self, img, st):
        if self._enc is None:
            self._enc = _Encoder(self._plan(), img.shape[2], img.shape[3])
        self._enc.plan = self._plan()
        return self._enc(img, st)

    def _check_img(self, img):
        if not img.is_cuda:
            raise RuntimeError("aot_benchmark_b200 engines run on CUDA tensors only (there is no CPU path)")

    @_in_precision
    def assign_identity_from_mask(self, mask, st):
        P = self._plan()
        ws = self._ws
        if mask.dim() == 4 and mask.shape[1] != 1:
            x = torch.empty((1, mask.shape[2], mask.shape[3], mask.shape[1]), dtype=torch.float32, device=mask.device)
            ops.nchw_to_nhwc(mask.float().contiguous(), x, stream=st)
            ops.conv2d(x, P.id_wt, P.id_b, ws.id_emb.view(1, *self.enc_size_2d, P.C), KH=P.id_k, KW=P.id_k,
                       stride=P.id_stride, pad=P.id_pad, stream=st)
            if P.deaot:
                ops.layernorm(ws.id_emb, P.id_norm[0], P.id_norm[1], ws.id_emb, stream=st)
            return ws.id_emb
        m2 = mask.reshape(mask.shape[-2], mask.shape[-1]).float().contiguous()
        if tuple(m2.shape) == tuple(ws.mask.shape):
            ops.eltwise(ops.EW_COPY, m2, None, ws.mask, stream=st)
            m2 = ws.mask
        self._id_from_static_mask(m2, st)
        return ws.id_emb

    def _id_from_static_mask(self, m2, st):
        P = self._plan()
        if P.C == 256:
            ops.id_embed_runs(m2, P.id_wp, P.id_b, self._ws.id_emb, P.C, P.nid, P.id_k, P.id_stride, P.id_pad,
                              ln_gamma=P.id_norm[0] if P.deaot else None, ln_beta=P.id_norm[1] if P.deaot else None,
                              stream=st)
        else:
            ops.id_embed(m2, P.id_wt, P.id_b, self._ws.id_emb, P.C, P.nid, P.id_k, P.id_stride, P.id_pad,
                         ln_gamma=P.id_norm[0] if P.deaot else None, ln_beta=P.id_norm[1] if P.deaot else None, stream=st)

    @_in_precision
    def add_reference_frame(self, img=None, mask=None, frame_step=-1, obj_nums=None, img_embs=None):
        if self.obj_nums is None and obj_nums is None:
            print('No objects for reference frame!')
            exit()
        elif obj_nums is not None:
            self.obj_nums = obj_nums
        if frame_step == -1:
            frame_step = self.frame_step
        if img_embs is None and img is None:
            print('No image for reference frame!')
            exit()
        if mask is None:
            print('No mask for reference frame!')
            exit()
        st = torch.cuda.current_stream().cuda_stream
        _apply_pdl()
        self._P = get_plan(self.AOT)
        if img_embs is None:
            self._check_img(img)
            img_embs = self._encode(img, st)
        if self.input_size_2d is None:
            f16 = img_embs.nhwc[-1]
            in_size = img.shape[2:] if img is not None else (f16.shape[1] * 16, f16.shape[2] * 16)
            self.update_size(in_size, (f16.shape[1], f16.shape[2]))
            self._alloc()
        self.curr_enc_embs = img_embs
        if self.pos_emb is None:
            if getattr(self._ws, "pos_emb", None) is None:
                self._ws.pos_emb = _pos_emb_sine(*self.enc_size_2d, npf=self._plan().C // 2).to(self._plan().device)
            self.pos_emb = self._ws.pos_emb
        id_emb = self.assign_identity_from_mask(mask, st)
        self.curr_id_embs = id_emb
        self._lstt_forward(img_embs, id_emb, st)
        if self._claim_memory_frame():
            self._bank_reserve(self.enc_hw)
            self._append_short_to_bank(st)
            self.bank_len = self._bank_len_after_store()
        self.last_mem_step = self.frame_step
        self._have_lstt = True

    @_in_precision
    def match_propogate_one_frame(self, img=None, img_embs=None):
        self.frame_step += 1
        st = torch.cuda.current_stream().cuda_stream
        if img_embs is None:
            self._check_img(img)
            img_embs = self._encode(img, st)
        self.curr_enc_embs = img_embs
        splits = lt_splits(self.enc_hw, self._plan().H, max(self.bank_len, 1)) if getattr(self, "_tc", False) else 0
        if getattr(self, "_gp_tc", False):
            splits = self._gp_splits(self.bank_len)
        if self._usage():
            splits = "usage"
        if self.kv_shard is not None:
            splits = ("shard", self._shard_splits(), self.bank_len > 0, SHARD_XCHG)
        self.graphs.run(("lstt", splits, img_embs.nhwc[-1].data_ptr()),
                        lambda: self._lstt_forward(img_embs, None, _cur_stream()),
                        enabled=self.short_term_mem_skip <= 1 and (self.kv_shard is None or SHARD_GRAPHS))

    @_in_precision
    def update_short_term_memory(self, curr_mask, curr_id_emb=None, skip_long_term_update=False):
        st = torch.cuda.current_stream().cuda_stream
        append = False
        if self.frame_step - self.last_mem_step >= self.long_term_mem_gap:
            append = not skip_long_term_update
            self.last_mem_step = self.frame_step
        append = append and self._claim_memory_frame()
        if append:
            self._bank_reserve(self.enc_hw)
        ws = self._ws
        label_map = curr_id_emb is None and not (curr_mask.dim() == 4 and curr_mask.shape[1] != 1) and \
            tuple(curr_mask.shape[-2:]) == tuple(ws.mask.shape)
        if label_map and self.short_term_mem_skip <= 1:
            m2 = curr_mask.reshape(ws.mask.shape).float().contiguous()
            ops.eltwise(ops.EW_COPY, m2, None, ws.mask, stream=st)

            def body():
                s2 = _cur_stream()
                self._id_from_static_mask(ws.mask, s2)
                self._fuse_memories(ws.id_emb, s2)
                if append:
                    self._append_short_to_bank(s2)
            self.graphs.run(("upd", append), body)
        else:
            id_emb = self.assign_identity_from_mask(curr_mask, st) if curr_id_emb is None else curr_id_emb
            self._fuse_memories(id_emb, st)
            if append:
                self._append_short_to_bank(st)
        if append:
            self.bank_len = self._bank_len_after_store()

    def _bank_len_after_store(self):
        n = self.bank_len + self.enc_hw
        return n if self.long_term_mem_max is None else min(n, self.bank_cap)

    def _claim_memory_frame(self):
        f = self._mem_frames
        self._mem_frames += 1
        return self.kv_shard is None or f % self.kv_shard[1] == self.kv_shard[0]

    def _append_short_to_bank(self, st):
        N = self.enc_hw
        K_src, V_src = self._latest_kv()
        if self.long_term_mem_max is not None:
            packed = (self.bank_Kp, self.bank_Vp) if self._tc else (self.bank_gpK, self.bank_gpV) if self._gp_tc else None
            if self._usage():
                ops.ring_select_usage(self.tk_dev, self.wr_dev, self._ws.usage_U, self._ws.usage_A, N, self.bank_cap, N,
                                      stream=st)
            for li in range(self._plan().L):
                ops.bank_ring_store(K_src[li], V_src[li], self.bank_K[li], self.bank_V[li],
                                    packed[0][li] if packed else None, packed[1][li] if packed else None, self.wr_dev, stream=st)
            ops.ring_advance(self.tk_dev, self.wr_dev, N, self.bank_cap, N, stream=st)
            return
        off = self.tk_dev
        for li in range(self._plan().L):
            ops.bank_append(K_src[li], self.bank_K[li], 0, offset_dev=off, stream=st)
            ops.bank_append(V_src[li], self.bank_V[li], 0, offset_dev=off, stream=st)
            if self._tc:
                ops.tc_pack_rows(K_src[li], self.bank_Kp[li], 0, row_off_dev=off, stream=st)
                ops.tc_pack_rows(V_src[li], self.bank_Vp[li], 0, row_off_dev=off, stream=st)
            if self._gemm_lt:
                ops.split_rows(K_src[li], self.bank_Kh[li], self.bank_Kl[li], row_off_dev=off, stream=st)
                ops.split_cols(V_src[li], self.bank_VhT[li], self.bank_VlT[li], col_off_dev=off, stream=st)
            if getattr(self, "_gp_tc", False):
                ops.tc_pack_rows(K_src[li], self.bank_gpK[li], 0, row_off_dev=off, stream=st)
                ops.tc_pack_rows(V_src[li], self.bank_gpV[li], 0, row_off_dev=off, stream=st)
        ops.counter_add(off, N, stream=st)

    def _latest_kv(self):
        return self._new_K, self._new_V

    def _lstt_forward(self, embs, id_emb, st):
        P = self._plan()
        ws = self._ws
        N, C, H = self.enc_hw, P.C, P.H
        h, w = self.enc_size_2d
        d = C // H
        proj = embs.nhwc[-1].view(N, C)
        ops.eltwise(ops.EW_COPY, proj, None, ws.x, stream=st)
        ops.eltwise(ops.EW_COPY, proj, None, ws.cat[:, :C], stream=st)
        x = ws.x
        is_ref = id_emb is not None
        if is_ref:
            stK, stV = self._next_short_slot()
        else:
            stK, stV = self.st_K, self.st_V
        for li in range(P.L):
            Lw = P.layers[li]
            ops.layernorm(x, Lw.norm1[0], Lw.norm1[1], ws.ln, add=self.pos_emb, out2=ws.ln_pos, stream=st)
            ops.linear(ws.ln_pos, Lw.sa_qk_w, Lw.sa_qk_b, ws.qk, stream=st)
            ops.linear(ws.ln, Lw.sa_v_w, Lw.sa_v_b, ws.v, stream=st)
            if self._tc:
                self._tc_attention(ws.qk[:, :C], ws.qk[:, C:], ws.v, None, None, N, ws.core[:, :C], st)
            else:
                ops.attention(ws.qk[:, :C], ws.qk[:, C:], ws.v, ws.core[:, :C], H, d, d, Tk=N, stream=st)
            ops.linear(ws.core[:, :C], Lw.sa_proj_w, Lw.sa_proj_b, x, res=x, stream=st)
            cQ, cV = self.curr_Q[li], self.curr_V[li]
            ops.layernorm(x, Lw.norm2[0], Lw.norm2[1], cV, stream=st)
            ops.linear(cV, Lw.linQ_w, Lw.linQ_b, cQ, stream=st)
            if is_ref:
                ops.eltwise(ops.EW_ADD, cV, id_emb, ws.tmp, stream=st)
                ops.linear(ws.tmp, Lw.linV_w, Lw.linV_b, stV[li], stream=st)
                ops.eltwise(ops.EW_COPY, cQ, None, stK[li], stream=st)
                gK, gV, Tk = stK[li], stV[li], N
            else:
                gK, gV, Tk = self.bank_K[li], self.bank_V[li], self.bank_len
            self._long_term_attention(li, cQ, gK, gV, Tk, ws.core[:, :C], st)
            if d == 32 and LOCAL_IMPL == "tile":
                ops.local_attention_tile(cQ, stK[li], stV[li], Lw.relk_w, Lw.relk_b, Lw.relv_t, ws.core[:, C:], h, w, H,
                                         stream=st)
            else:
                ops.local_attention(cQ, stK[li], stV[li], Lw.relk_w, Lw.relk_b, Lw.relv, ws.core[:, C:], h, w, H, d, d,
                                    stream=st)
            ops.linear(ws.core, Lw.lst_proj_w, Lw.lst_proj_b, x, res=x, stream=st)
            ops.layernorm(x, Lw.norm3[0], Lw.norm3[1], ws.ln, stream=st)
            ops.linear(ws.ln, Lw.lin1_w, Lw.lin1_b, ws.ff, stream=st)
            ops.groupnorm(ws.ff.view(1, N, 4 * C), Lw.gn[0], Lw.gn[1], ws.ff.view(1, N, 4 * C), 32, A_GELU, ws.gn_ws,
                          stream=st)
            ops.dwconv(ws.ff.view(1, h, w, 4 * C), Lw.dw_w, None, ws.ff2.view(1, h, w, 4 * C), K=5, pad=2, stream=st)
            ops.linear(ws.ff2, Lw.lin2_w, Lw.lin2_b, x, res=x, stream=st)
            ops.layernorm(x, Lw.dec_norm[0], Lw.dec_norm[1], ws.cat[:, (li + 1) * C:(li + 2) * C], stream=st)
        if is_ref:
            self._commit_short_slot(stK, stV)
        self._have_lstt = True

    def _long_term_attention(self, li, Q, K, V, Tk, out, st):
        P = self._plan()
        d = P.C // P.H
        probe = LT_PROBE
        use_tc = self._tc and (K is self.bank_K[li])
        if use_tc:
            ops.tc_pack_rows(Q, self._ws.Qp, 0, div=math.sqrt(d), stream=st)
        if probe is not None:
            e0, e1 = torch.cuda.Event(enable_timing=True), torch.cuda.Event(enable_timing=True)
            e0.record()
        if use_tc and self.kv_shard is not None:
            self._sharded_attention(li, out, st)
        elif self.kv_shard is not None and K is self.bank_K[li]:
            raise ops.AotbError("sharded long-term bank needs the tensor-core attention kernel (8 heads x 32); this model's "
                                "head shape runs on the fp32 kernel, which has no partial (m, l, O) outputs")
        elif use_tc and self._usage():
            self._usage_attention(li, self._ws.Qp, self.bank_Kp[li], self.bank_Vp[li], out, st)
        elif use_tc:
            self._tc_attention(None, None, None, self.bank_Kp[li], self.bank_Vp[li], Tk, out, st, Tk_dev=self.tk_dev)
        elif self._tc:
            self._tc_attention(Q, K, V, None, None, Tk, out, st)
        else:
            ops.attention(Q, K, V, out, P.H, d, d, Tk=Tk, Tk_dev=self.tk_dev if K is self.bank_K[li] else None,
                          stream=st)
        if probe is not None:
            e1.record()
            probe.append((e0, e1, 4.0 * Q.shape[0] * Tk * P.C))

    def _tc_attention(self, Q, K, V, Kp, Vp, Tk, out, st, Tk_dev=None):
        P = self._plan()
        ws = self._ws
        d = P.C // P.H
        N = self.enc_hw
        if Q is not None:
            ops.tc_pack_rows(Q, ws.Qp, 0, div=math.sqrt(d), stream=st)
        if Kp is None:
            ops.tc_pack_rows(K, ws.saKp, 0, stream=st)
            ops.tc_pack_rows(V, ws.saVp, 0, stream=st)
            Kp, Vp = ws.saKp, ws.saVp
        splits = lt_splits(N, P.H, Tk)
        part = None
        if splits > 1:
            part = ws.part.get(splits)
            if part is None:
                fz = lambda *s: torch.empty(s, dtype=torch.float32, device=out.device)
                part = (fz(splits, N, P.C), fz(splits, P.H, N), fz(splits, P.H, N))
                ws.part[splits] = part
        exact = LT_IMPL == "tc_exact" and self.precision == "fp32"
        ops.lt_attention_tc(ws.Qp, Kp, Vp, N, Tk, O=out, Tk_dev=Tk_dev, splits=splits, exact=exact, part=part, stream=st)

    def _usage_attention(self, li, Qp, Kp, Vp, out, st):
        P = self._plan()
        ws = self._ws
        M, N = self.long_term_mem_max, self.enc_hw
        if P.deaot:
            H = 1
            ops.gp_attention_tc_slots(Qp, Kp, Vp, N, self.tk_dev, M, N, ws.usage_part, exact=self.precision == "fp32",
                                      stream=st)
        else:
            H = P.H
            ops.lt_attention_tc_slots(Qp, Kp, Vp, N, self.tk_dev, M, N, ws.usage_part,
                                      exact=LT_IMPL == "tc_exact" and self.precision == "fp32", stream=st)
        ops.attn_merge_usage(*ws.usage_part, out, H, out.shape[1] // H, ws.usage_U, ws.usage_A if li == 0 else None,
                             self.tk_dev, N, P.L, ws.usage_ws, stream=st)

    def _shard_splits(self):
        world = self.kv_shard[1]
        frames_per_rank = (self._mem_frames + world - 1) // world
        s = max(2, lt_splits(self.enc_hw, self._plan().H, max(frames_per_rank, 1) * self.enc_hw))
        if s > SHARD_SMAX:
            raise ops.AotbError(f"sharded long-term attention: {s} KV splits exceed the exchange buffer capacity {SHARD_SMAX}")
        return s

    def _sharded_attention(self, li, out, st):
        import torch.distributed as dist
        rank, world, group = self.kv_shard
        P = self._plan()
        ws = self._ws
        N, C, H = self.enc_hw, P.C, P.H
        splits = self._shard_splits()
        if st != torch.cuda.current_stream().cuda_stream:
            raise ops.AotbError("sharded long-term attention must run on torch's current stream (the collective / the "
                                "symmetric-memory barrier are issued there)")
        if SHARD_XCHG == "p2p":
            return self._sharded_attention_p2p(li, out, st, splits)
        key = ("shard", splits)
        bufs = ws.part.get(key)
        if bufs is None:
            nO, nM = splits * N * C, splits * H * N
            mine = torch.empty(nO + 2 * nM, dtype=torch.float32, device=out.device)
            allr = torch.empty(world * (nO + 2 * nM), dtype=torch.float32, device=out.device)
            sl = lambda t: (t[:nO].view(splits, N, C), t[nO:nO + nM].view(splits, H, N), t[nO + nM:].view(splits, H, N))
            per_rank = [sl(allr[r * (nO + 2 * nM):(r + 1) * (nO + 2 * nM)]) for r in range(world)]
            bufs = ws.part[key] = (mine, allr, sl(mine), per_rank)
        mine, allr, (Op, Mp, Lp), per_rank = bufs
        if self.bank_len > 0:
            ops.lt_attention_tc(ws.Qp, self.bank_Kp[li], self.bank_Vp[li], N, self.bank_len, O=None, Tk_dev=self.tk_dev,
                                splits=splits, exact=(LT_IMPL == "tc_exact"), part=(Op, Mp, Lp), stream=st, merge=False)
        else:
            ops.eltwise(ops.EW_FILL, None, None, mine[:Op.numel()].view(1, -1), scalar=0.0, stream=st)
            ops.eltwise(ops.EW_FILL, None, None, Mp.view(1, -1), scalar=float("-inf"), stream=st)
            ops.eltwise(ops.EW_FILL, None, None, Lp.view(1, -1), scalar=0.0, stream=st)
        dist.all_gather_into_tensor(allr, mine, group=group)
        ops.attn_merge_peers([v[0] for v in per_rank], [v[1] for v in per_rank], [v[2] for v in per_rank], out, splits, H,
                             C // H, stream=st)

    def _sharded_attention_p2p(self, li, out, st, splits):
        rank, world, group = self.kv_shard
        P = self._plan()
        ws = self._ws
        N, C, H = self.enc_hw, P.C, P.H
        key = ("p2p", li)
        buf = ws.part.get(key)
        if buf is None:
            nO, nM = SHARD_SMAX * N * C, SHARD_SMAX * H * N
            hdl, view = _symm_alloc(nO + 2 * nM, out.device, group)
            views = [(view(r, (SHARD_SMAX, N, C), 0), view(r, (SHARD_SMAX, H, N), nO), view(r, (SHARD_SMAX, H, N), nO + nM))
                     for r in range(world)]
            buf = ws.part[key] = (hdl, views)
        hdl, views = buf
        Op, Mp, Lp = (t[:splits] for t in views[rank])
        if self.bank_len > 0:
            ops.lt_attention_tc(ws.Qp, self.bank_Kp[li], self.bank_Vp[li], N, self.bank_len, O=None, Tk_dev=self.tk_dev,
                                splits=splits, exact=(LT_IMPL == "tc_exact"), part=(Op, Mp, Lp), stream=st, merge=False)
        else:
            ops.eltwise(ops.EW_FILL, None, None, Op.reshape(1, -1), scalar=0.0, stream=st)
            ops.eltwise(ops.EW_FILL, None, None, Mp.reshape(1, -1), scalar=float("-inf"), stream=st)
            ops.eltwise(ops.EW_FILL, None, None, Lp.reshape(1, -1), scalar=0.0, stream=st)
        hdl.barrier()
        ops.attn_merge_peers([v[0] for v in views], [v[1] for v in views], [v[2] for v in views], out, splits, H, C // H,
                             stream=st)
        if P.L < 2:
            hdl.barrier()

    def _next_short_slot(self):
        if self.short_term_mem_skip <= 1:
            return self.st_K, self.st_V
        K = [torch.empty_like(t) for t in self.st_K]
        V = [torch.empty_like(t) for t in self.st_V]
        return K, V

    def _commit_short_slot(self, K, V, reset=True):
        self._new_K, self._new_V = K, V
        if self.short_term_mem_skip <= 1:
            return
        if reset:
            self._st_ring = [(K, V)]
        else:
            self._st_ring.append((K, V))
            self._st_ring = self._st_ring[-self.short_term_mem_skip:]
        self.st_K, self.st_V = self._st_ring[0]

    def _fuse_memories(self, id_emb, st):
        P = self._plan()
        ws = self._ws
        K, V = self._next_short_slot()
        for li in range(P.L):
            Lw = P.layers[li]
            ops.eltwise(ops.EW_ADD, self.curr_V[li], id_emb, ws.tmp, stream=st)
            ops.linear(ws.tmp, Lw.linV_w, Lw.linV_b, V[li], stream=st)
            ops.eltwise(ops.EW_COPY, self.curr_Q[li], None, K[li], stream=st)
        self._commit_short_slot(K, V, reset=False)

    def _dbuf(self, key, shape):
        b = self._dec_bufs.get(key)
        if b is None or tuple(b.shape) != tuple(shape):
            b = torch.empty(shape, dtype=torch.float32, device=self._plan().device)
            self._dec_bufs[key] = b
        return b

    def _decode(self, st):
        P = self._plan()
        D = P.dec
        ws = self._ws
        ac = P.align_corners
        x4, x8, x16, _ = self.curr_enc_embs.nhwc
        h, w = self.enc_size_2d
        C = P.C
        gws = ws.gn_ws

        def conv_gn(x, blk, key, k, pad, res=None):
            o = self._dbuf(key, (1, x.shape[1], x.shape[2], blk.cout))
            ops.conv2d(x, blk.w, blk.b, o, KH=k, KW=k, pad=pad, stream=st)
            ov = o.view(1, -1, blk.cout)
            ops.groupnorm(ov, blk.gn[0], blk.gn[1], ov, 8, A_RELU, gws, stream=st)
            return o

        cat = ws.cat.view(1, h, w, -1)
        x = conv_gn(cat, D.conv_in, "in", 1, 0)
        a = self._dbuf("a16", (1, h, w, D.adapter_16x.cout))
        ops.conv2d(x16, D.adapter_16x.w, D.adapter_16x.b, a, res=x, stream=st)
        x = conv_gn(a, D.conv_16x, "c16", 3, 1)
        up = self._dbuf("up8", (1, x8.shape[1], x8.shape[2], x.shape[3]))
        ops.bilinear(x, up, ac, stream=st)
        a = self._dbuf("a8", (1, x8.shape[1], x8.shape[2], D.adapter_8x.cout))
        ops.conv2d(x8, D.adapter_8x.w, D.adapter_8x.b, a, res=up, stream=st)
        x = conv_gn(a, D.conv_8x, "c8", 3, 1)
        up = self._dbuf("up4", (1, x4.shape[1], x4.shape[2], x.shape[3]))
        ops.bilinear(x, up, ac, stream=st)
        a = self._dbuf("a4", (1, x4.shape[1], x4.shape[2], D.adapter_4x.cout))
        ops.conv2d(x4, D.adapter_4x.w, D.adapter_4x.b, a, res=up, stream=st)
        x = conv_gn(a, D.conv_4x, "c4", 3, 1)
        lg = self._dbuf("logit", (1, x.shape[1], x.shape[2], D.conv_out.cout))
        ops.conv2d(x, D.conv_out.w, D.conv_out.b, lg, stream=st)
        return lg

    @_in_precision
    def decode_current_logits(self, output_size=None):
        P = self._plan()
        size = None if output_size is None else (int(output_size[0]), int(output_size[1]))
        obj = int(self.obj_nums[0])

        def body():
            st = _cur_stream()
            lg = self._decode(st)
            h4, w4, NC = lg.shape[1], lg.shape[2], lg.shape[3]
            bufs = self._dec_out.get(size)
            if bufs is None:
                lo = torch.empty((1, NC, h4, w4), dtype=torch.float32, device=lg.device)
                out = None if size is None else torch.empty((1, NC) + size, dtype=torch.float32, device=lg.device)
                bufs = self._dec_out[size] = (lo, out)
            ops.logits_postproc(lg, bufs[0], bufs[1], obj, P.align_corners, stream=st)
            return bufs

        enc_ptrs = tuple(t.data_ptr() for t in self.curr_enc_embs.nhwc[:3])
        lo, out = self.graphs.run(("dec", size, obj) + enc_ptrs, body)
        self.pred_id_logits = lo
        return lo if out is None else out

    def predict_current_mask(self, output_size=None, return_prob=False):
        if output_size is None:
            output_size = self.input_size_2d
        st = torch.cuda.current_stream().cuda_stream
        oh, ow = int(output_size[0]), int(output_size[1])
        label = torch.empty((1, oh, ow), dtype=torch.float32, device=self.pred_id_logits.device)
        ops.logits_argmax(self.pred_id_logits, label, self._plan().align_corners, stream=st)
        if return_prob:
            raise NotImplementedError("return_prob is used by the training path only (SURVEY 8f)")
        return label.long()


class DeAOTEngine(AOTEngine):

    def __init__(self, aot_model, gpu_id=0, long_term_mem_gap=9999, short_term_mem_skip=1,
                 layer_loss_scaling_ratio=2., long_term_mem_max=None, precision=None, long_term_mem_policy=None):
        super().__init__(aot_model, gpu_id, long_term_mem_gap, short_term_mem_skip, long_term_mem_max=long_term_mem_max,
                         precision=precision, long_term_mem_policy=long_term_mem_policy)
        self.layer_loss_scaling_ratio = layer_loss_scaling_ratio

    def _gated_tail(self, core, U, dw_w, out_slice, h, w, st):
        ws = self._ws
        N = core.shape[0]
        C4 = core.shape[1]
        ops.eltwise(ops.EW_MUL, core, U, ws.gated, stream=st)
        ops.dwconv(ws.gated.view(1, h, w, C4), dw_w, None, out_slice.unflatten(0, (1, h, w)), K=5, pad=2, stream=st)

    def _lstt_forward(self, embs, id_emb, st):
        P = self._plan()
        ws = self._ws
        N, C = self.enc_hw, P.C
        h, w = self.enc_size_2d
        d = C // 2
        C2, C4 = 2 * C, 4 * C
        proj = embs.nhwc[-1].view(N, C)
        x, z = ws.xz[:, :C], ws.xz[:, C:]
        ops.eltwise(ops.EW_COPY, proj, None, x, stream=st)
        ops.eltwise(ops.EW_FILL, None, None, z, scalar=0.0, stream=st)
        is_ref = id_emb is not None
        if is_ref:
            stK, stV = self._next_short_slot()
        else:
            stK, stV = self.st_K, self.st_V
        for li in range(P.L):
            Lw = P.layers[li]
            cQ, cV = self.curr_Q[li], self.curr_V[li]
            ops.layernorm(x, Lw.norm1[0], Lw.norm1[1], ws.ln, stream=st)
            ops.linear(ws.ln, Lw.qv_w, Lw.qv_b, ws.qv, stream=st)
            ops.eltwise(ops.EW_COPY, ws.qv[:, :d], None, cQ, stream=st)
            ops.eltwise(ops.EW_SILU, ws.qv[:, d:], None, cV, stream=st)
            ops.linear(ws.ln, Lw.u_w, Lw.u_b, ws.catU[:, :C2], act=A_SILU, stream=st)
            if li == 0:
                ops.eltwise(ops.EW_FILL, None, None, ws.catU[:, C2:], scalar=1.0, stream=st)
                cIDV = None
            else:
                cIDV = self.curr_IDV[li]
                ops.layernorm(z, Lw.id_norm1[0], Lw.id_norm1[1], cIDV, stream=st)
                ops.linear(cIDV, Lw.idu_w, Lw.idu_b, ws.catU[:, C2:], act=A_SILU, stream=st)
            if is_ref:
                ops.eltwise(ops.EW_COPY, cQ, None, stK[li], stream=st)
                ops.eltwise(ops.EW_COPY, cV, None, stV[li][:, :C2], stream=st)
                self._fuse_id(li, cIDV, id_emb, stV[li][:, C2:], st)
                gK, gV, Tk = stK[li], stV[li], N
            else:
                gK, gV, Tk = self.bank_K[li], self.bank_V[li], self.bank_len
            probe = LT_PROBE if not is_ref else None
            if probe is not None:
                e0, e1 = torch.cuda.Event(enable_timing=True), torch.cuda.Event(enable_timing=True)
                e0.record()
            if self._gp_tc and not is_ref and self._usage():
                ops.tc_pack_rows(cQ, ws.gpQp, 0, div=math.sqrt(self._kdim), stream=st)
                self._usage_attention(li, ws.gpQp, self.bank_gpK[li], self.bank_gpV[li], ws.core, st)
            elif self._gp_tc and not is_ref:
                self._gp_attention(cQ, None, None, self.bank_gpK[li], self.bank_gpV[li], Tk, self.tk_dev, ws.core, st)
            elif self._gp_tc:
                self._gp_attention(cQ, gK, gV, None, None, N, None, ws.core, st)
            elif self._gemm_lt and not is_ref:
                ops.linear_tc(cQ, self.bank_Kh[li], self.bank_Kl[li], None, ws.S, stream=st)
                ops.row_softmax(ws.S, self._capw, Tk, 1.0 / math.sqrt(d), Tk_dev=self.tk_dev, stream=st)
                ops.linear_tc(ws.S, self.bank_VhT[li], self.bank_VlT[li], None, ws.core, stream=st)
            else:
                ops.attention(cQ, gK, gV, ws.core, 1, d, C4, Tk=Tk, Tk_dev=None if is_ref else self.tk_dev, stream=st)
            if probe is not None:
                e1.record()
                probe.append((e0, e1, 2.0 * N * Tk * (d + C4)))
            self._gated_tail(ws.core, ws.catU, Lw.lt_dw, ws.dw[:, :C4], h, w, st)
            if LOCAL_IMPL == "tile" and d == 128 and C4 == 1024:
                ops.local_gated_tile(cQ, stK[li], stV[li], Lw.relk_w, Lw.relk_b, ws.core, h, w, stream=st)
            else:
                ops.local_attention(cQ, stK[li], stV[li], Lw.relk_w, Lw.relk_b, None, ws.core, h, w, 1, d, C4, stream=st)
            self._gated_tail(ws.core, ws.catU, Lw.st_dw, ws.dw[:, C4:], h, w, st)
            ops.linear(ws.dw, Lw.lst_proj_w, Lw.lst_proj_b, ws.xz, res=ws.xz, stream=st)
            ops.layernorm(x, Lw.norm2[0], Lw.norm2[1], ws.c[:, :C], stream=st)
            ops.layernorm(z, Lw.id_norm2[0], Lw.id_norm2[1], ws.c[:, C:], stream=st)
            ops.linear(ws.c, Lw.sa_qk_w, Lw.sa_qk_b, ws.sa_qk, stream=st)
            ops.linear(ws.c[:, :C], Lw.sa_v1[0], Lw.sa_v1[1], ws.sa_v[:, :C2], act=A_SILU, stream=st)
            ops.linear(ws.c[:, C:], Lw.sa_v2[0], Lw.sa_v2[1], ws.sa_v[:, C2:], act=A_SILU, stream=st)
            ops.linear(ws.c[:, :C], Lw.sa_u1[0], Lw.sa_u1[1], ws.sa_u[:, :C2], act=A_SILU, stream=st)
            ops.linear(ws.c[:, C:], Lw.sa_u2[0], Lw.sa_u2[1], ws.sa_u[:, C2:], act=A_SILU, stream=st)
            if self._gp_tc:
                self._gp_attention(ws.sa_qk, ws.sa_qk, ws.sa_v, None, None, N, None, ws.core, st)
            else:
                ops.attention(ws.sa_qk, ws.sa_qk, ws.sa_v, ws.core, 1, d, C4, Tk=N, stream=st)
            self._gated_tail(ws.core, ws.sa_u, Lw.sa_dw, ws.dw[:, :C4], h, w, st)
            ops.linear(ws.dw[:, :C4], Lw.sa_proj_w, Lw.sa_proj_b, ws.xz, res=ws.xz, stream=st)
        ops.groupnorm(ws.xz.view(1, N, C2), P.final_gn[0], P.final_gn[1], ws.cat.view(1, N, C2), 2, A_NONE, ws.gn_ws,
                      stream=st)
        if is_ref:
            self._commit_short_slot(stK, stV)
        self._have_lstt = True

    def _gp_attention(self, Q, K, V, Kp, Vp, Tk, Tk_dev, out, st):
        ws = self._ws
        N = self.enc_hw
        ops.tc_pack_rows(Q, ws.gpQp, 0, div=math.sqrt(self._kdim), stream=st)
        if Kp is None:
            ops.tc_pack_rows(K, ws.gpSaK, 0, stream=st)
            ops.tc_pack_rows(V, ws.gpSaV, 0, stream=st)
            Kp, Vp = ws.gpSaK, ws.gpSaV
        splits = self._gp_splits(Tk)
        part = None
        if splits > 1:
            part = ws.gp_part.get(splits)
            if part is None:
                fz = lambda *s: torch.empty(s, dtype=torch.float32, device=out.device)
                part = ws.gp_part[splits] = (fz(splits, N, out.shape[1]), fz(splits, 1, N), fz(splits, 1, N))
        ops.gp_attention_tc(ws.gpQp, Kp, Vp, N, Tk, O=out, Tk_dev=Tk_dev, splits=splits, exact=self.precision == "fp32",
                            part=part, stream=st)

    def _gp_splits(self, Tk):
        base = ((self.enc_hw + 127) // 128) * (4 * self._plan().C // 64)
        tiles = (max(Tk, 1) + 63) // 64
        return max(1, min(tiles // 4 if tiles >= 8 else 1, max(1, (2 * 132) // base)))

    def _fuse_id(self, li, cIDV, id_emb, out, st):
        Lw = self._plan().layers[li]
        ws = self._ws
        C = self._plan().C
        if cIDV is None:
            ops.linear(id_emb, Lw.idv_w, Lw.idv_b, out, act=A_SILU, stream=st)
        else:
            ops.eltwise(ops.EW_COPY, cIDV, None, ws.idin[:, :C], stream=st)
            ops.eltwise(ops.EW_COPY, id_emb, None, ws.idin[:, C:], stream=st)
            ops.linear(ws.idin, Lw.idv_w, Lw.idv_b, out, act=A_SILU, stream=st)

    def _fuse_memories(self, id_emb, st):
        P = self._plan()
        C2 = 2 * P.C
        K, V = self._next_short_slot()
        for li in range(P.L):
            ops.eltwise(ops.EW_COPY, self.curr_Q[li], None, K[li], stream=st)
            ops.eltwise(ops.EW_COPY, self.curr_V[li], None, V[li][:, :C2], stream=st)
            self._fuse_id(li, self.curr_IDV[li], id_emb, V[li][:, C2:], st)
        self._commit_short_slot(K, V, reset=False)


class AOTInferEngine(nn.Module):
    _engine_cls = AOTEngine

    def __init__(self, aot_model, gpu_id=0, long_term_mem_gap=9999, short_term_mem_skip=1, max_aot_obj_num=None,
                 long_term_mem_max=None, precision=None, long_term_mem_policy=None):
        super().__init__()
        self.precision = _resolve_precision(aot_model, precision)
        self.cfg = aot_model.cfg
        self.AOT = aot_model
        if max_aot_obj_num is None or max_aot_obj_num > aot_model.max_obj_num:
            self.max_aot_obj_num = aot_model.max_obj_num
        else:
            self.max_aot_obj_num = max_aot_obj_num
        self.gpu_id = gpu_id
        self.long_term_mem_gap = long_term_mem_gap
        self.short_term_mem_skip = short_term_mem_skip
        self.long_term_mem_max = _resolve_mem_max(aot_model, long_term_mem_max)
        self.long_term_mem_policy = _resolve_mem_policy(aot_model, long_term_mem_policy, self.long_term_mem_max)
        self.aot_engines = []
        self._kv_shard = None
        self.restart_engine()

    def enable_kv_sharding(self, rank, world, group=None):
        if self.precision == "fp16":
            raise NotImplementedError("a long-term bank sharded over GPUs is not built for precision='fp16'")
        if self.long_term_mem_max is not None:
            raise NotImplementedError("a bounded long-term bank (long_term_mem_max) cannot be sharded over GPUs: each rank "
                                      "would need its own ring")
        self._kv_shard = (rank, world, group)
        for e in self.aot_engines:
            e.enable_kv_sharding(rank, world, group)

    def restart_engine(self):
        self._pool = getattr(self, "_pool", []) + list(self.aot_engines)
        self.aot_engines = []
        self.obj_nums = None

    def _run_engines(self, fn):
        return fork_join(self, self.aot_engines, fn)

    def separate_mask(self, mask, obj_nums):
        n = len(self.aot_engines)
        if mask is None:
            return [None] * n
        if n == 1:
            return [mask], [obj_nums]
        per = self.max_aot_obj_num
        counts = [per] * n
        if obj_nums % per > 0:
            counts[-1] = obj_nums % per
        if mask.dim() == 3 or mask.shape[0] == 1:
            m = mask.float().contiguous()
            out = torch.empty((n,) + tuple(m.shape), dtype=torch.float32, device=m.device)
            ops.separate_labels(m, out, per)
            return [out[e] for e in range(n)], counts
        probs = []
        for e in range(n):
            fg = mask[e * per + 1:(e + 1) * per + 1]
            probs.append(torch.cat([1. - fg.sum(dim=1, keepdim=True), fg], dim=1))
        return probs, counts

    def soft_logit_aggregation(self, all_logits):
        if len(all_logits) == 1:
            return all_logits[0]
        per = self.max_aot_obj_num
        first = all_logits[0]
        key = (len(all_logits), tuple(first.shape[-2:]))
        buf = getattr(self, "_agg_out", None)
        if buf is None or buf[0] != key:
            buf = self._agg_out = (key, torch.empty((1, 1 + len(all_logits) * per) + tuple(first.shape[-2:]),
                                                    dtype=torch.float32, device=first.device))
        return ops.soft_logit_aggregation([t if t.is_contiguous() else t.contiguous() for t in all_logits], buf[1], per)

    def add_reference_frame(self, img, mask, obj_nums, frame_step=-1):
        if isinstance(obj_nums, list):
            obj_nums = obj_nums[0]
        self.obj_nums = obj_nums
        want = max(-(-int(obj_nums) // self.max_aot_obj_num), 1)
        while len(self.aot_engines) < want:
            eng = self._pool.pop(0) if self._pool else self._engine_cls(self.AOT, self.gpu_id, self.long_term_mem_gap,
                                                                       self.short_term_mem_skip,
                                                                       long_term_mem_max=self.long_term_mem_max,
                                                                       precision=self.precision,
                                                                       long_term_mem_policy=self.long_term_mem_policy)
            eng.long_term_mem_max = self.long_term_mem_max
            eng.long_term_mem_policy = self.long_term_mem_policy
            eng.restart_engine()
            eng.eval()
            if self._kv_shard is not None:
                eng.enable_kv_sharding(*self._kv_shard)
            self.aot_engines.append(eng)
        masks, counts = self.separate_mask(mask, obj_nums)
        first = self.aot_engines[0]
        first.add_reference_frame(img, masks[0], obj_nums=[counts[0]], frame_step=frame_step)
        embs = first.curr_enc_embs
        if len(self.aot_engines) > 1:
            self._run_engines(lambda i, e: None if i == 0 else e.add_reference_frame(
                img, masks[i], obj_nums=[counts[i]], frame_step=frame_step, img_embs=embs))
        self.update_size()

    def match_propogate_one_frame(self, img=None):
        first = self.aot_engines[0]
        if len(self.aot_engines) == 1:
            return first.match_propogate_one_frame(img)
        first._check_img(img)
        embs = first._encode(img, torch.cuda.current_stream().cuda_stream)
        self._run_engines(lambda i, e: e.match_propogate_one_frame(img, img_embs=embs))

    def decode_current_logits(self, output_size=None):
        all_logits = self._run_engines(lambda i, e: e.decode_current_logits(output_size))
        return self.soft_logit_aggregation(all_logits)

    def update_memory(self, curr_mask, skip_long_term_update=False):
        masks, _ = self.separate_mask(curr_mask, self.obj_nums)
        self._run_engines(lambda i, e: e.update_short_term_memory(masks[i], skip_long_term_update=skip_long_term_update))

    update_short_long_term_memory = update_memory

    def update_size(self):
        self.input_size_2d = self.aot_engines[0].input_size_2d
        self.enc_size_2d = self.aot_engines[0].enc_size_2d
        self.enc_hw = self.aot_engines[0].enc_hw

    @property
    def pred_id_logits(self):
        return self.aot_engines[0].pred_id_logits if self.aot_engines else None

    @property
    def long_term_memory_usage(self):
        return [e.long_term_memory_usage for e in self.aot_engines]


class DeAOTInferEngine(AOTInferEngine):
    _engine_cls = DeAOTEngine


_ENGINES = {("aotengine", "train"): AOTEngine, ("aotengine", "eval"): AOTInferEngine,
            ("deaotengine", "train"): DeAOTEngine, ("deaotengine", "eval"): DeAOTInferEngine}


def build_engine(name, phase='train', **kwargs):
    cls = _ENGINES.get((name, phase))
    if cls is None:
        raise NotImplementedError
    return cls(**kwargs)
```

### aot_benchmark_b200/ops.py

```python
from __future__ import annotations

import contextlib
import os

import torch

from ._lib import AotbError, check, lib

ACT_NONE, ACT_RELU, ACT_GELU, ACT_SILU, ACT_RELU6, ACT_HSWISH = 0, 1, 2, 3, 4, 5
EW_COPY, EW_ADD, EW_MUL, EW_SILU, EW_SILU_MUL, EW_FILL = 0, 1, 2, 3, 4, 5


def _st(stream):
    return torch.cuda.current_stream().cuda_stream if stream is None else stream


def _chk(*ts):
    for t in ts:
        if t is None:
            continue
        if not t.is_cuda or t.dtype != torch.float32:
            raise AotbError(f"aot_benchmark_b200 kernels need float32 CUDA tensors, got {t.dtype} on {t.device}")
        if t.dim() >= 1 and t.stride(-1) != 1:
            raise AotbError("innermost stride must be 1")


def _p(t):
    return None if t is None else t.data_ptr()


def _nhwc_ld(x):
    B, H, W, C = x.shape
    ld = x.stride(2)
    if x.stride(1) != W * ld or (B > 1 and x.stride(0) != H * W * ld):
        raise AotbError("NHWC tensor must be dense over pixels")
    return ld


_TC_WEIGHTS = {}
CONV_IMPL = os.environ.get("AOTB_CONV_IMPL", "tc")
PRECISIONS = ("fp32", "fp16")
_PRECISION = "fp32"


@contextlib.contextmanager
def precision(p):
    global _PRECISION
    if p not in PRECISIONS:
        raise ValueError(f"precision must be one of {PRECISIONS}, got {p!r}")
    old, _PRECISION = _PRECISION, p
    try:
        yield
    finally:
        _PRECISION = old


_TC_WS = {}
CONV_PROBE = None


class _ConvProbe:
    def __init__(self, flops, stream):
        self.on = CONV_PROBE is not None and stream in (None, torch.cuda.current_stream().cuda_stream)
        self.flops = flops

    def __enter__(self):
        if self.on:
            self.e0, self.e1 = torch.cuda.Event(enable_timing=True), torch.cuda.Event(enable_timing=True)
            self.e0.record()

    def __exit__(self, *a):
        if self.on:
            self.e1.record()
            CONV_PROBE.append((self.e0, self.e1, self.flops))


def _tc_workspace(device):
    ws = _TC_WS.get(device)
    if ws is None:
        ws = _TC_WS[device] = torch.zeros(1 << 20, dtype=torch.uint8, device=device)
    return ws


def register_tc_weights(w, wh, wl, wscale=None):
    _TC_WEIGHTS[w.data_ptr()] = (wh, wl, wscale, w)


def split_fp16(w_kn):
    K = w_kn.shape[0]
    wt = w_kn.t().contiguous()
    if K % 64:
        wt = torch.nn.functional.pad(wt, (0, 64 - K % 64))
    hi = wt.half()
    lo = (wt - hi.float()).half()
    return hi.contiguous(), lo.contiguous()


def weight_scale_exponents(w_kn):
    amax = w_kn.abs().amax(dim=0).float()
    _, ex = torch.frexp(amax)
    e = (14 - ex).clamp(max=126)
    return torch.where(amax > 0, e, torch.zeros_like(e)).to(torch.int32)


def split_fp16_scaled(w_kn):
    e = weight_scale_exponents(w_kn)
    hi, lo = split_fp16(w_kn.float() * _pow2(e))
    return hi, lo, _pow2(-e)


def _pow2(e):
    return ((e + 127) << 23).to(torch.int32).view(torch.float32)


CONV_CONST_WEIGHTS = 256

CONV_CHAIN = False


def conv2d_tc(x, wh, wl, bias, out, res=None, KH=1, KW=1, stride=1, pad=0, act=ACT_NONE, stream=None, wscale=None,
              const_w=False):
    _chk(x, bias, out, res, wscale)
    B, H, W, Cin = x.shape
    Cout = wh.shape[0]
    ws = _tc_workspace(x.device)
    with _ConvProbe(2.0 * out.shape[0] * out.shape[1] * out.shape[2] * Cout * KH * KW * Cin, stream):
        check(lib().aotb_conv2d_nhwc_tc(_p(x), wh.data_ptr(), _p(wl), _p(bias), _p(wscale), _p(res), _p(out), B, H, W, Cin,
                                        _nhwc_ld(x), Cout, _nhwc_ld(out), _nhwc_ld(res) if res is not None else 0, KH, KW,
                                        stride, pad, act | (CONV_CONST_WEIGHTS if const_w else 0), ws.data_ptr(), ws.numel(),
                                        _st(stream)), "aotb_conv2d_nhwc_tc")
    return out


def conv2d(x, w, bias, out, res=None, KH=1, KW=1, stride=1, pad=0, dil=1, act=ACT_NONE, stream=None):
    if CONV_IMPL == "tc" and dil == 1:
        t = _TC_WEIGHTS.get(w.data_ptr())
        if t is not None:
            return conv2d_tc(x, t[0], None if _PRECISION == "fp16" else t[1], bias, out, res=res, KH=KH, KW=KW, stride=stride, pad=pad, act=act,
                             stream=stream, wscale=t[2], const_w=True)
    _chk(x, w, bias, out, res)
    B, H, W, Cin = x.shape
    Cout = w.shape[1]
    check(lib().aotb_conv2d_nhwc_f32(_p(x), _p(w), _p(bias), _p(res), _p(out), B, H, W, Cin, _nhwc_ld(x), Cout,
                                     _nhwc_ld(out), _nhwc_ld(res) if res is not None else 0, KH, KW, stride, pad,
                                     dil, act, _st(stream)), "aotb_conv2d_nhwc_f32")
    return out


def linear(x, wt, bias, out, res=None, act=ACT_NONE, stream=None):
    if CONV_IMPL == "tc":
        t = _TC_WEIGHTS.get(wt.data_ptr())
        if t is not None:
            _chk(x, bias, out, res, t[2])
            M, K = x.shape
            N = wt.shape[1]
            ws = _tc_workspace(x.device)
            with _ConvProbe(2.0 * M * N * K, stream):
                wl = None if _PRECISION == "fp16" else t[1]
                check(lib().aotb_conv2d_nhwc_tc(_p(x), t[0].data_ptr(), _p(wl), _p(bias), _p(t[2]), _p(res), _p(out),
                                                1, M, 1, K, x.stride(0), N, out.stride(0), res.stride(0) if res is not None else 0,
                                                1, 1, 1, 0, act | CONV_CONST_WEIGHTS, ws.data_ptr(), ws.numel(), _st(stream)),
                      "aotb_conv2d_nhwc_tc")
            return out
    _chk(x, wt, bias, out, res)
    M, K = x.shape
    N = wt.shape[1]
    check(lib().aotb_linear_f32(_p(x), _p(wt), _p(bias), _p(res), _p(out), M, K, x.stride(0), N, out.stride(0),
                                res.stride(0) if res is not None else 0, act, _st(stream)), "aotb_linear_f32")
    return out


def linear_tc(x, wh, wl, bias, out, res=None, act=ACT_NONE, stream=None):
    _chk(x, bias, out, res)
    if wh.dtype != torch.float16 or wl.dtype != torch.float16 or wh.shape != wl.shape or not wh.is_contiguous() \
            or not wl.is_contiguous():
        raise AotbError("linear_tc: wh / wl must be contiguous fp16 tensors of the same shape [N, K]")
    M, K = x.shape
    N = wh.shape[0]
    if wh.shape[1] != K or K % 64 or N % 64 or out.shape[0] != M or out.shape[1] != N:
        raise AotbError(f"linear_tc: shapes x {tuple(x.shape)}, w {tuple(wh.shape)}, out {tuple(out.shape)}")
    ws = _tc_workspace(x.device)
    check(lib().aotb_conv2d_nhwc_tc(_p(x), wh.data_ptr(), wl.data_ptr(), _p(bias), None, _p(res), _p(out), 1, M, 1, K,
                                    x.stride(0), N, out.stride(0), res.stride(0) if res is not None else 0, 1, 1, 1, 0,
                                    act, ws.data_ptr(), ws.numel(), _st(stream)), "aotb_conv2d_nhwc_tc")
    return out


def split_rows(src, hi, lo, row_off=0, row_off_dev=None, stream=None):
    _chk(src)
    rows, C = src.shape
    check(lib().aotb_split_rows_f16x2(_p(src), src.stride(0), hi.data_ptr(), lo.data_ptr(), hi.stride(0), rows, C,
                                      int(row_off), row_off_dev.data_ptr() if row_off_dev is not None else None,
                                      _st(stream)), "aotb_split_rows_f16x2")


def split_cols(src, hiT, loT, col_off=0, col_off_dev=None, stream=None):
    _chk(src)
    rows, C = src.shape
    check(lib().aotb_split_cols_f16x2(_p(src), src.stride(0), hiT.data_ptr(), loT.data_ptr(), hiT.stride(0), rows, C,
                                      int(col_off), col_off_dev.data_ptr() if col_off_dev is not None else None,
                                      _st(stream)), "aotb_split_cols_f16x2")


def row_softmax(S, cols, Tk, scale, Tk_dev=None, stream=None):
    _chk(S)
    check(lib().aotb_row_softmax_f32(_p(S), S.stride(0), S.shape[0], int(cols), int(Tk),
                                     Tk_dev.data_ptr() if Tk_dev is not None else None, float(scale), _st(stream)),
          "aotb_row_softmax_f32")
    return S


def nchw_to_nhwc(x, out, stream=None):
    _chk(x, out)
    B, C, H, W = x.shape
    check(lib().aotb_nchw_to_nhwc_f32(_p(x.contiguous()), _p(out), B, C, H * W, _st(stream)), "aotb_nchw_to_nhwc_f32")
    return out


def image_to_nhwc4(img, out, stream=None):
    _chk(img, out)
    check(lib().aotb_image_to_nhwc4_f32(_p(img.contiguous()), _p(out), img.shape[2] * img.shape[3], _st(stream)),
          "aotb_image_to_nhwc4_f32")
    return out


def nhwc_to_nchw(x, out, stream=None):
    _chk(x, out)
    B, H, W, C = x.shape
    check(lib().aotb_nhwc_to_nchw_f32(_p(x), _p(out), B, C, H * W, _st(stream)), "aotb_nhwc_to_nchw_f32")
    return out


def maxpool3x3s2(x, out, stream=None):
    _chk(x, out)
    B, H, W, C = x.shape
    check(lib().aotb_maxpool3x3s2_nhwc_f32(_p(x), _p(out), B, H, W, C, _st(stream)), "aotb_maxpool3x3s2_nhwc_f32")
    return out


def dwconv(x, w, bias, out, K=5, stride=1, pad=2, dil=1, act=ACT_NONE, stream=None):
    _chk(x, w, bias, out)
    B, H, W, C = x.shape
    check(lib().aotb_dwconv_nhwc_f32(_p(x), _p(w), _p(bias), _p(out), B, H, W, C, _nhwc_ld(x), _nhwc_ld(out), K, K,
                                     stride, pad, dil, act, _st(stream)), "aotb_dwconv_nhwc_f32")
    return out


def bilinear(x, out, align_corners, stream=None):
    _chk(x, out)
    B, H, W, C = x.shape
    check(lib().aotb_bilinear_nhwc_f32(_p(x), _p(out), B, H, W, C, out.shape[1], out.shape[2],
                                       1 if align_corners else 0, _st(stream)), "aotb_bilinear_nhwc_f32")
    return out


def eltwise(op, a, b, out, scalar=0.0, stream=None):
    _chk(a, b, out)
    rows, cols = out.shape
    check(lib().aotb_eltwise_f32(op, _p(a), a.stride(0) if a is not None else 0, _p(b),
                                 b.stride(0) if b is not None else 0, _p(out), out.stride(0), rows, cols,
                                 float(scalar), _st(stream)), "aotb_eltwise_f32")
    return out


def layernorm(x, gamma, beta, out, add=None, out2=None, stream=None):
    _chk(x, gamma, beta, out, add, out2)
    rows, C = x.shape
    check(lib().aotb_layernorm_f32(_p(x), x.stride(0), _p(gamma), _p(beta), _p(add),
                                   add.stride(0) if add is not None else 0, _p(out), out.stride(0), _p(out2),
                                   out2.stride(0) if out2 is not None else 0, rows, C, _st(stream)),
          "aotb_layernorm_f32")
    return out


def window_attention(qkv, qkv_bias, rel_bias, out, H, W, heads, shift, window=7, stream=None):
    _chk(qkv, qkv_bias, rel_bias, out)
    C = out.shape[1]
    if qkv.shape[0] != H * W or qkv.shape[1] != 3 * C or out.shape[0] != H * W:
        raise AotbError("window_attention: qkv must be [H*W, 3C], out [H*W, C]")
    T = window * window
    if tuple(rel_bias.shape) != (heads, T, T) or not rel_bias.is_contiguous():
        raise AotbError(f"window_attention: rel_bias must be contiguous [{heads}, {T}, {T}], got {tuple(rel_bias.shape)}")
    if qkv_bias.numel() != 3 * C or not qkv_bias.is_contiguous():
        raise AotbError(f"window_attention: qkv_bias must be contiguous with {3 * C} elements, got {qkv_bias.numel()}")
    check(lib().aotb_window_attention_f32(_p(qkv), qkv.stride(0), _p(qkv_bias), _p(rel_bias), _p(out), out.stride(0),
                                          H, W, C, heads, window, shift, _st(stream)), "aotb_window_attention_f32")
    return out


def patch_merge(x, out, H, W, stream=None):
    _chk(x, out)
    C = x.shape[1]
    if x.shape[0] != H * W or out.shape[0] != ((H + 1) // 2) * ((W + 1) // 2) or out.shape[1] != 4 * C:
        raise AotbError("patch_merge: shape mismatch")
    check(lib().aotb_patch_merge_f32(_p(x), x.stride(0), _p(out), out.stride(0), H, W, C, _st(stream)),
          "aotb_patch_merge_f32")
    return out


def groupnorm_workspace(B, G, device):
    n = lib().aotb_groupnorm_workspace_bytes(B, G)
    return torch.zeros((n + 7) // 8, dtype=torch.float64, device=device)


def groupnorm(x, gamma, beta, out, G, act, workspace, stream=None):
    _chk(x, gamma, beta, out)
    B, P, C = x.shape
    check(lib().aotb_groupnorm_nhwc_f32(_p(x), x.stride(1), _p(gamma), _p(beta), _p(out), out.stride(1), B, P, C, G,
                                        act, workspace.data_ptr(), _st(stream)), "aotb_groupnorm_nhwc_f32")
    return out


def splat_workspace(C, device):
    n = lib().aotb_splat_workspace_bytes(C)
    return torch.zeros((n + 7) // 8, dtype=torch.float64, device=device)


def splat_attention(x, w1, b1, w2, b2, att, workspace, radix=2, stream=None):
    _chk(x, w1, b1, w2, b2, att)
    x2 = x.reshape(-1, x.shape[-1]) if x.dim() == 4 else x
    HW, ld = x2.shape[0], (_nhwc_ld(x) if x.dim() == 4 else x.stride(0))
    C, inter = w1.shape
    if w2.shape != (inter, radix * C) or b1.numel() != inter or b2.numel() != radix * C or att.numel() != radix * C \
            or x.shape[-1] < radix * C or not (w1.is_contiguous() and w2.is_contiguous() and att.is_contiguous()):
        raise AotbError("splat_attention: shapes x [.., >= radix*C], w1 [C, inter], w2 [inter, radix*C], att [radix*C]")
    check(lib().aotb_splat_attention_f32(_p(x), ld, HW, C, radix, _p(w1), _p(b1), inter, _p(w2), _p(b2), _p(att),
                                         workspace.data_ptr(), _st(stream)), "aotb_splat_attention_f32")
    return att


def splat_combine(x, att, out, radix=2, pool_stride=0, stream=None):
    _chk(x, att, out)
    _, H, W, _ = x.shape
    C = out.shape[3]
    Ho, Wo = (pool2d_size(H, 3, pool_stride, 1), pool2d_size(W, 3, pool_stride, 1)) if pool_stride else (H, W)
    if att.numel() != radix * C or x.shape[3] < radix * C or tuple(out.shape[1:3]) != (Ho, Wo):
        raise AotbError(f"splat_combine: x {tuple(x.shape)}, att {tuple(att.shape)}, out {tuple(out.shape)}")
    check(lib().aotb_splat_combine_f32(_p(x), _nhwc_ld(x), _p(att), _p(out), _nhwc_ld(out), H, W, C, radix, int(pool_stride),
                                       _st(stream)), "aotb_splat_combine_f32")
    return out


def se_gate(x, w1, b1, w2, b2, gate, workspace, stream=None):
    _chk(x, w1, b1, w2, b2, gate)
    x2 = x.reshape(-1, x.shape[-1]) if x.dim() == 4 else x
    HW, ld = x2.shape[0], (_nhwc_ld(x) if x.dim() == 4 else x.stride(0))
    C, inter = w1.shape
    if w2.shape != (inter, C) or b1.numel() != inter or b2.numel() != C or gate.numel() != C or x.shape[-1] != C \
            or not (w1.is_contiguous() and w2.is_contiguous() and gate.is_contiguous()):
        raise AotbError("se_gate: shapes x [.., C], w1 [C, inter], w2 [inter, C], gate [C]")
    check(lib().aotb_se_gate_f32(_p(x), ld, HW, C, _p(w1), _p(b1), inter, _p(w2), _p(b2), _p(gate), workspace.data_ptr(),
                                 _st(stream)), "aotb_se_gate_f32")
    return gate


def gate_scale(x, gate, out, act=ACT_NONE, stream=None):
    _chk(x, gate, out)
    B, H, W, C = x.shape
    if B != 1 or tuple(out.shape) != (1, H, W, C) or gate.numel() != C:
        raise AotbError(f"gate_scale: x {tuple(x.shape)}, gate {tuple(gate.shape)}, out {tuple(out.shape)}")
    check(lib().aotb_gate_scale_f32(_p(x), _nhwc_ld(x), _p(gate), _p(out), _nhwc_ld(out), H * W, C, int(act), _st(stream)),
          "aotb_gate_scale_f32")
    return out


def pool2d_size(n, k, s, pad=0, ceil_mode=False):
    o = (n + 2 * pad - k + (s - 1 if ceil_mode else 0)) // s + 1
    if ceil_mode and (o - 1) * s >= n + pad:
        o -= 1
    return o


def avgpool(x, out, k, s, pad=0, ceil_mode=False, count_include_pad=True, stream=None):
    _chk(x, out)
    B, H, W, C = x.shape
    if tuple(out.shape) != (B, pool2d_size(H, k, s, pad, ceil_mode), pool2d_size(W, k, s, pad, ceil_mode), C):
        raise AotbError(f"avgpool: out {tuple(out.shape)} does not match x {tuple(x.shape)} pooled ({k}, {s}, {pad})")
    check(lib().aotb_avgpool_nhwc_f32(_p(x), _nhwc_ld(x), _p(out), _nhwc_ld(out), B, H, W, C, k, s, pad, 1 if ceil_mode else 0,
                                      1 if count_include_pad else 0, _st(stream)), "aotb_avgpool_nhwc_f32")
    return out


def attention(Q, K, V, O, H, d_qk, d_v, Tk=None, Tk_dev=None, Mout=None, Lout=None, stream=None):
    _chk(Q, K, V, O, Mout, Lout)
    N = Q.shape[0]
    tk = K.shape[0] if Tk is None else int(Tk)
    check(lib().aotb_attention_f32(_p(Q), Q.stride(0), _p(K), K.stride(0), _p(V), V.stride(0), _p(O), O.stride(0),
                                   N, tk, Tk_dev.data_ptr() if Tk_dev is not None else None, H, d_qk, d_v,
                                   _p(Mout), _p(Lout), _st(stream)), "aotb_attention_f32")
    return O


def attn_merge(Opart, Mpart, Lpart, O, H, d_v, stream=None):
    _chk(Opart, Mpart, Lpart, O)
    R, N = Opart.shape[0], Opart.shape[1]
    check(lib().aotb_attn_merge_f32(_p(Opart), _p(Mpart), _p(Lpart), _p(O), R, N, H, d_v, O.stride(0), _st(stream)),
          "aotb_attn_merge_f32")
    return O


def attn_merge_usage_workspace(R, device):
    n = int(lib().aotb_attn_merge_usage_workspace_bytes(int(R)))
    return torch.zeros((n + 7) // 8, dtype=torch.float64, device=device)


def attn_merge_usage(Opart, Mpart, Lpart, O, H, d_v, U, A, live_dev, rows, layers, workspace, stream=None):
    _chk(Opart, Mpart, Lpart, O, U)
    R, N = Opart.shape[0], Opart.shape[1]
    if U.numel() != R or not U.is_contiguous() or (A is not None and (A.dtype != torch.int32 or A.numel() != R or
                                                                      not A.is_cuda)):
        raise AotbError(f"attn_merge_usage: U must be float32 [{R}] and A int32 [{R}] CUDA tensors")
    check(lib().aotb_attn_merge_usage_f32(_p(Opart), _p(Mpart), _p(Lpart), _p(O), R, N, H, d_v, O.stride(0), _p(U), _p(A),
                                          _counter("attn_merge_usage: live_dev", live_dev) if A is not None else None,
                                          int(rows), int(layers), workspace.data_ptr(), _st(stream)),
          "aotb_attn_merge_usage_f32")
    return O


def attn_merge_peers(Oparts, Mparts, Lparts, O, splits, H, d_v, stream=None):
    import ctypes
    _chk(O, *Oparts, *Mparts, *Lparts)
    R, N = len(Oparts), O.shape[0]
    arr = lambda ts: (ctypes.c_void_p * R)(*[t.data_ptr() for t in ts])
    check(lib().aotb_attn_merge_peers_f32(arr(Oparts), arr(Mparts), arr(Lparts), R, int(splits), _p(O), N, H, d_v,
                                          O.stride(0), _st(stream)), "aotb_attn_merge_peers_f32")
    return O


def local_attention(q, k, v, relk_w, relk_b, relv, out, h, w, H, d_att, d_v, stream=None):
    _chk(q, k, v, relk_w, relk_b, relv, out)
    check(lib().aotb_local_attention_f32(_p(q), q.stride(0), _p(k), k.stride(0), _p(v), v.stride(0), _p(relk_w),
                                         _p(relk_b), _p(relv), _p(out), out.stride(0), h, w, H, d_att, d_v,
                                         _st(stream)), "aotb_local_attention_f32")
    return out


def local_gated_tile(q, k, v, relk_w, relk_b, out, h, w, stream=None):
    _chk(q, k, v, relk_w, relk_b, out)
    if q.shape[1] != 128 or k.shape[1] != 128 or v.shape[1] != 1024 or out.shape[1] != 1024 or not relk_w.is_contiguous():
        raise AotbError("local_gated_tile: q / k [hw, 128], v / out [hw, 1024], contiguous relative_emb_k weights [225, 128]")
    check(lib().aotb_local_gated_tile_f32(_p(q), q.stride(0), _p(k), k.stride(0), _p(v), v.stride(0), _p(relk_w), _p(relk_b),
                                          _p(out), out.stride(0), h, w, _st(stream)), "aotb_local_gated_tile_f32")
    return out


def local_attention_tile(q, k, v, relk_w, relk_b, relv_t, out, h, w, H, stream=None):
    _chk(q, k, v, relk_w, relk_b, relv_t, out)
    check(lib().aotb_local_attention_tile_f32(_p(q), q.stride(0), _p(k), k.stride(0), _p(v), v.stride(0), _p(relk_w),
                                              _p(relk_b), _p(relv_t), _p(out), out.stride(0), h, w, H, _st(stream)),
          "aotb_local_attention_tile_f32")
    return out


def _id_embed_check(name, mask, table, table_shape, bias, out, C, ksize, stride, pad, ln_gamma, ln_beta):
    _chk(mask, table, bias, out, ln_gamma, ln_beta)
    if mask.dim() != 2 or not mask.is_contiguous():
        raise AotbError(f"{name}: mask must be a contiguous [Hm, Wm] map, got shape {tuple(mask.shape)}, "
                        f"strides {mask.stride()}")
    Hm, Wm = mask.shape
    ho, wo = (Hm + 2 * pad - ksize) // stride + 1, (Wm + 2 * pad - ksize) // stride + 1
    if tuple(table.shape) != tuple(table_shape) or not table.is_contiguous():
        raise AotbError(f"{name}: weight table must be a contiguous {list(table_shape)}, got {tuple(table.shape)}")
    if bias.numel() != C or any(t is not None and t.numel() != C for t in (ln_gamma, ln_beta)):
        raise AotbError(f"{name}: bias and LayerNorm parameters need {C} entries")
    if out.dim() != 2 or tuple(out.shape) != (ho * wo, C):
        raise AotbError(f"{name}: out must be [{ho * wo}, {C}] for a {Hm}x{Wm} mask, got {tuple(out.shape)}")
    return Hm, Wm


def id_embed(mask, wt, bias, out, C, nid, ksize, stride, pad, ln_gamma=None, ln_beta=None, stream=None):
    Hm, Wm = _id_embed_check("id_embed", mask, wt, (ksize * ksize * nid, C), bias, out, C, ksize, stride, pad, ln_gamma,
                             ln_beta)
    check(lib().aotb_id_embed_f32(_p(mask), Hm, Wm, _p(wt), _p(bias), _p(ln_gamma), _p(ln_beta), _p(out),
                                  out.stride(0), C, nid, ksize, stride, pad, _st(stream)), "aotb_id_embed_f32")
    return out


def id_embed_runs(mask, wp, bias, out, C, nid, ksize, stride, pad, ln_gamma=None, ln_beta=None, stream=None):
    Hm, Wm = _id_embed_check("id_embed_runs", mask, wp, (ksize, ksize + 1, nid, C), bias, out, C, ksize, stride, pad,
                             ln_gamma, ln_beta)
    check(lib().aotb_id_embed_runs_f32(_p(mask), Hm, Wm, _p(wp), _p(bias), _p(ln_gamma), _p(ln_beta), _p(out),
                                       out.stride(0), C, nid, ksize, stride, pad, _st(stream)), "aotb_id_embed_runs_f32")
    return out


def _dense_maps(name, t, shape3):
    if t.dim() < 3 or t.numel() != t.shape[-3] * t.shape[-2] * t.shape[-1] or not t.is_contiguous() \
            or any(want is not None and got != want for got, want in zip(t.shape[-3:], shape3)):
        want = "x".join("*" if v is None else str(v) for v in shape3)
        raise AotbError(f"{name}: need one contiguous [{want}] map, got shape {tuple(t.shape)}, strides {t.stride()}")


def logits_postproc(logits_nhwc, lowres_nchw, out_nchw, obj_num, align_corners, stream=None):
    _chk(logits_nhwc, lowres_nchw, out_nchw)
    _dense_maps("logits_postproc logits", logits_nhwc, (None, None, None))
    h, w, NC = logits_nhwc.shape[-3:]
    _dense_maps("logits_postproc lowres", lowres_nchw, (NC, h, w))
    if out_nchw is not None:
        _dense_maps("logits_postproc out", out_nchw, (NC, None, None))
    Ho, Wo = (out_nchw.shape[-2], out_nchw.shape[-1]) if out_nchw is not None else (0, 0)
    check(lib().aotb_logits_postproc_f32(_p(logits_nhwc), _p(lowres_nchw), _p(out_nchw), h, w, NC, obj_num, Ho, Wo,
                                         1 if align_corners else 0, _st(stream)), "aotb_logits_postproc_f32")
    return out_nchw


def logits_argmax(lowres_nchw, label, align_corners, stream=None):
    _chk(lowres_nchw, label)
    _dense_maps("logits_argmax lowres", lowres_nchw, (None, None, None))
    NC, h, w = lowres_nchw.shape[-3:]
    Ho, Wo = label.shape[-2:]
    if label.numel() != Ho * Wo or not label.is_contiguous():
        raise AotbError(f"logits_argmax: label must be one contiguous [Ho, Wo] map, got {tuple(label.shape)}")
    check(lib().aotb_logits_argmax_f32(_p(lowres_nchw), _p(label), h, w, NC, Ho, Wo, 1 if align_corners else 0,
                                       _st(stream)), "aotb_logits_argmax_f32")
    return label


def soft_logit_aggregation(logits, out, max_obj, stream=None):
    import ctypes
    _chk(out, *logits)
    E = len(logits)
    HW = out.shape[-2] * out.shape[-1]
    for t in logits:
        if not t.is_contiguous() or t.shape[1] != 1 + max_obj or t.shape[-2] * t.shape[-1] != HW:
            raise AotbError("soft_logit_aggregation: logit maps must be contiguous [1, 1 + max_obj, H, W] of one size")
    if not out.is_contiguous() or out.shape[1] != 1 + E * max_obj:
        raise AotbError("soft_logit_aggregation: out must be contiguous [1, 1 + E * max_obj, H, W]")
    arr = (ctypes.c_void_p * E)(*[t.data_ptr() for t in logits])
    check(lib().aotb_soft_logit_aggregation_f32(arr, E, int(max_obj), _p(out), HW, _st(stream)),
          "aotb_soft_logit_aggregation_f32")
    return out


def tta_merge(logits, flips, label, align_corners, new_label=None, prob=None, stream=None):
    import ctypes
    _chk(label, new_label, prob, *logits)
    E = len(logits)
    if not 1 <= E <= 8 or len(flips) != E:
        raise AotbError(f"tta_merge: 1 to 8 logit maps with one flip bit each, got {E} maps and {len(flips)} flips")
    for t in logits:
        _dense_maps("tta_merge logits", t, (logits[0].shape[-3], None, None))
    NC = int(logits[0].shape[-3])
    H, W = label.shape[-2:]
    for name, t in (("label", label), ("new_label", new_label)):
        if t is not None and (t.numel() != H * W or not t.is_contiguous() or tuple(t.shape[-2:]) != (H, W)):
            raise AotbError(f"tta_merge: {name} must be one contiguous [{H}, {W}] map, got {tuple(t.shape)}")
    if prob is not None:
        _dense_maps("tta_merge prob", prob, (NC, H, W))
    arr = (ctypes.c_void_p * E)(*[t.data_ptr() for t in logits])
    sizes = (ctypes.c_int * (2 * E))(*[int(v) for t in logits for v in t.shape[-2:]])
    fl = (ctypes.c_int * E)(*[1 if f else 0 for f in flips])
    check(lib().aotb_tta_merge_f32(arr, sizes, fl, E, NC, H, W, 1 if align_corners else 0, _p(new_label), _p(label), _p(prob),
                                   _st(stream)), "aotb_tta_merge_f32")
    return label


def tta_feedback(logits, out, output_size, align_corners, flip, new_label=None, stream=None):
    _chk(logits, out, new_label)
    H, W = int(output_size[0]), int(output_size[1])
    Hi, Wi = out.shape[-2:]
    if out.numel() != Hi * Wi or not out.is_contiguous():
        raise AotbError(f"tta_feedback: out must be one contiguous [Hi, Wi] map, got {tuple(out.shape)}")
    if new_label is not None and (new_label.numel() != H * W or not new_label.is_contiguous()
                                  or tuple(new_label.shape[-2:]) != (H, W)):
        raise AotbError(f"tta_feedback: new_label must be one contiguous [{H}, {W}] map, got {tuple(new_label.shape)}")
    NC, h, w = 0, 0, 0
    if logits is not None:
        _dense_maps("tta_feedback logits", logits, (None, None, None))
        NC, h, w = (int(v) for v in logits.shape[-3:])
    check(lib().aotb_tta_feedback_f32(_p(logits), h, w, NC, H, W, 1 if align_corners else 0, 1 if flip else 0, _p(new_label),
                                      _p(out), Hi, Wi, _st(stream)), "aotb_tta_feedback_f32")
    return out


def separate_labels(mask, out, max_obj, stream=None):
    _chk(mask, out)
    E, HW = out.shape[0], mask.numel()
    if not mask.is_contiguous() or not out.is_contiguous() or out.numel() != E * HW:
        raise AotbError("separate_labels: mask [HW] and out [E, HW] must be contiguous")
    check(lib().aotb_separate_labels_f32(_p(mask), E, int(max_obj), _p(out), HW, _st(stream)), "aotb_separate_labels_f32")
    return out


def preprocess_bgr_u8(img_u8, out, taps=None, flip=False, stream=None):
    if img_u8.dtype != torch.uint8 or not img_u8.is_cuda or not img_u8.is_contiguous() or img_u8.dim() != 3 or img_u8.shape[2] != 3:
        raise AotbError("preprocess_bgr_u8: image must be a contiguous uint8 CUDA tensor [H, W, 3]")
    _chk(out)
    if out.dim() != 4 or tuple(out.shape[:2]) != (1, 3) or not out.is_contiguous():
        raise AotbError(f"preprocess_bgr_u8: out must be contiguous [1, 3, Ho, Wo], got {tuple(out.shape)}")
    H, W = int(img_u8.shape[0]), int(img_u8.shape[1])
    Ho, Wo = int(out.shape[-2]), int(out.shape[-1])
    if taps is None:
        ptrs = (None, None, None, None)
    else:
        ix, cx, iy, cy = taps
        if ix.dtype != torch.int32 or iy.dtype != torch.int32 or cx.dtype != torch.float32 or cy.dtype != torch.float32 \
                or tuple(ix.shape) != (Wo, 4) or tuple(cx.shape) != (Wo, 4) or tuple(iy.shape) != (Ho, 4) or tuple(cy.shape) != (Ho, 4):
            raise AotbError("preprocess_bgr_u8: taps must be (int32 [Wo,4], fp32 [Wo,4], int32 [Ho,4], fp32 [Ho,4])")
        if not all(t.is_cuda and t.is_contiguous() for t in taps):
            raise AotbError("preprocess_bgr_u8: tap tables must be contiguous CUDA tensors")
        ptrs = tuple(t.data_ptr() for t in (ix, cx, iy, cy))
    check(lib().aotb_preprocess_bgr_u8(img_u8.data_ptr(), H, W, ptrs[0], ptrs[1], ptrs[2], ptrs[3], _p(out), Ho, Wo,
                                       1 if flip else 0, _st(stream)), "aotb_preprocess_bgr_u8")
    return out


def label_to_u8(label, out_u8, stream=None):
    _chk(label)
    if out_u8.dtype != torch.uint8 or not out_u8.is_cuda or not out_u8.is_contiguous() or not label.is_contiguous() \
            or out_u8.numel() != label.numel():
        raise AotbError("label_to_u8: contiguous float32 label and uint8 output of the same size on the device")
    check(lib().aotb_label_to_u8(_p(label), out_u8.data_ptr(), label.numel(), _st(stream)), "aotb_label_to_u8")
    return out_u8


def nearest_resize(x, out, stream=None):
    _chk(x, out)
    H, W = x.shape[-2:]
    Ho, Wo = out.shape[-2:]
    for t, n in ((x, H * W), (out, Ho * Wo)):
        if t.numel() != n or not t.is_contiguous():
            raise AotbError(f"nearest_resize: need contiguous single maps, got {tuple(t.shape)} with strides {t.stride()}")
    check(lib().aotb_nearest_resize_f32(_p(x), _p(out), H, W, Ho, Wo, _st(stream)), "aotb_nearest_resize_f32")
    return out


def bank_append(src, bank, offset, offset_dev=None, stream=None):
    _chk(src, bank)
    rows, cols = src.shape
    if bank.dim() != 2 or cols > bank.shape[1] or rows > bank.shape[0] or \
            (offset_dev is None and not 0 <= int(offset) <= bank.shape[0] - rows):
        raise AotbError(f"bank_append: {rows} x {cols} rows at offset {int(offset) if offset_dev is None else 'on device'} "
                        f"do not fit a bank of {tuple(bank.shape)}")
    check(lib().aotb_bank_append_f32(_p(src), src.stride(0), _p(bank), bank.stride(0), rows, cols, int(offset),
                                     offset_dev.data_ptr() if offset_dev is not None else None, _st(stream)),
          "aotb_bank_append_f32")
    return bank


def counter_add(counter, delta, stream=None):
    if not counter.is_cuda or counter.dtype != torch.int32:
        raise AotbError("counter must be an int32 CUDA tensor")
    check(lib().aotb_counter_add(counter.data_ptr(), int(delta), _st(stream)), "aotb_counter_add")
    return counter


def _counter(name, c):
    if c is None or not c.is_cuda or c.dtype != torch.int32 or c.numel() != 1:
        raise AotbError(f"{name} must be an int32 CUDA tensor [1]")
    return c.data_ptr()


def bank_ring_store(k_src, v_src, k_bank, v_bank, k_packed, v_packed, write_dev, stream=None):
    _chk(k_src, v_src, k_bank, v_bank)
    if k_src.dim() != 2 or v_src.dim() != 2 or k_src.shape[0] != v_src.shape[0]:
        raise AotbError("bank_ring_store: k_src and v_src must be [rows, C] with the same rows")
    rows = k_src.shape[0]
    caps = set()
    for name, src, bank, packed in (("k", k_src, k_bank, k_packed), ("v", v_src, v_bank, v_packed)):
        cols = src.shape[1]
        if bank is not None:
            if bank.dim() != 2 or bank.shape[1] < cols:
                raise AotbError(f"bank_ring_store: {name}_bank {tuple(bank.shape)} is narrower than the {cols} source channels")
            caps.add(bank.shape[0])
        if packed is not None:
            if packed.dtype != torch.float16 or not packed.is_cuda or not packed.is_contiguous() or packed.dim() != 3 or \
                    packed.shape[2] != 64 or packed.shape[0] * 32 != cols:
                raise AotbError(f"bank_ring_store: {name}_packed must be a contiguous fp16 CUDA tensor [{cols} / 32, cap, 64]")
            caps.add(packed.shape[1])
    if len(caps) != 1 or rows > min(caps):
        raise AotbError(f"bank_ring_store: the copies need one capacity of at least {rows} rows, got {sorted(caps)}")
    check(lib().aotb_bank_ring_store(_p(k_src), k_src.stride(0), k_src.shape[1], _p(v_src), v_src.stride(0), v_src.shape[1],
                                     rows, _p(k_bank), k_bank.stride(0) if k_bank is not None else 0, _p(v_bank),
                                     v_bank.stride(0) if v_bank is not None else 0, _p(k_packed), _p(v_packed), caps.pop(),
                                     _counter("bank_ring_store: write_dev", write_dev), _st(stream)), "aotb_bank_ring_store")


def ring_advance(live_dev, write_dev, rows, cap_rows, pinned_rows, stream=None):
    check(lib().aotb_ring_advance(_counter("ring_advance: live_dev", live_dev), _counter("ring_advance: write_dev", write_dev),
                                  int(rows), int(cap_rows), int(pinned_rows), _st(stream)), "aotb_ring_advance")


def ring_select_usage(live_dev, write_dev, U, A, rows, cap_rows, pinned_rows, stream=None):
    if U.dtype != torch.float32 or A.dtype != torch.int32 or not U.is_cuda or not A.is_cuda or \
            U.numel() * rows != cap_rows or A.numel() * rows != cap_rows:
        raise AotbError(f"ring_select_usage: U must be float32 and A int32 CUDA tensors of {cap_rows} / {rows} slots")
    check(lib().aotb_ring_select_usage(_counter("ring_select_usage: live_dev", live_dev),
                                       _counter("ring_select_usage: write_dev", write_dev), U.data_ptr(), A.data_ptr(),
                                       int(rows), int(cap_rows), int(pinned_rows), _st(stream)), "aotb_ring_select_usage")


def tc_pack_rows(src, dst, row_off=0, div=1.0, row_off_dev=None, stream=None):
    _chk(src)
    if dst.dtype != torch.float16 or not dst.is_cuda or not dst.is_contiguous():
        raise AotbError("packed operand buffer must be a contiguous fp16 CUDA tensor [H, cap, 64]")
    H, cap, _ = dst.shape
    rows = src.shape[0]
    check(lib().aotb_tc_pack_rows_f16x2(_p(src), src.stride(0), dst.data_ptr(), cap, rows, H, int(row_off),
                                        row_off_dev.data_ptr() if row_off_dev is not None else None, float(div),
                                        _st(stream)), "aotb_tc_pack_rows_f16x2")
    return dst


LT_VARIANT = os.environ.get("AOTB_LT_VARIANT", "tile")
LT_SPIN = os.environ.get("AOTB_LT_SPIN", "0") == "1"


def lt_attention_tc(Qp, Kp, Vp, N, Tk, O=None, Tk_dev=None, splits=1, exact=True, part=None, dbg=None, stream=None,
                    merge=True, variant=None):
    v = LT_VARIANT if variant is None else variant
    if v not in ("tile", "groups", "ahead", "pair"):
        raise AotbError(f"unknown long-term attention variant '{v}' (tile | groups | ahead | pair)")
    mode = (1 if exact else 0) | (2 if v == "groups" else 0) | (4 if LT_SPIN else 0) | (8 if v == "ahead" else 0) | \
        (16 if v == "pair" else 0)
    H, nq_cap, _ = Qp.shape
    kv_cap = Kp.shape[1]
    if splits > 1:
        Op, Mp, Lp = part
    else:
        Op = Mp = Lp = None
    check(lib().aotb_lt_attn_tc_f16x2(Qp.data_ptr(), nq_cap, Kp.data_ptr(), Vp.data_ptr(), kv_cap, N, int(Tk),
                                      Tk_dev.data_ptr() if Tk_dev is not None else None, H,
                                      _p(O) if splits == 1 else None, O.stride(0) if O is not None else 0,
                                      _p(Op), _p(Mp), _p(Lp), splits, mode, _p(dbg), _st(stream)),
          "aotb_lt_attn_tc_f16x2")
    if splits > 1 and merge:
        attn_merge(Op, Mp, Lp, O, H, 32, stream=stream)
    return O


def gp_attention_tc(Qp, Kp, Vp, N, Tk, O=None, Tk_dev=None, splits=1, exact=True, part=None, stream=None, merge=True):
    nq_cap, kv_cap, dv = Qp.shape[1], Kp.shape[1], Vp.shape[0] * 32
    if splits > 1:
        Op, Mp, Lp = part
    else:
        Op = Mp = Lp = None
    mode = (1 if exact else 0) | (4 if LT_SPIN else 0)
    check(lib().aotb_gp_attn_tc_f16x2(Qp.data_ptr(), nq_cap, Kp.data_ptr(), Vp.data_ptr(), kv_cap, N, int(Tk),
                                      Tk_dev.data_ptr() if Tk_dev is not None else None, dv,
                                      _p(O) if splits == 1 else None, O.stride(0) if O is not None else 0,
                                      _p(Op), _p(Mp), _p(Lp), splits, mode, _st(stream)), "aotb_gp_attn_tc_f16x2")
    if splits > 1 and merge:
        attn_merge(Op, Mp, Lp, O, 1, dv, stream=stream)
    return O


def lt_attention_tc_slots(Qp, Kp, Vp, N, Tk_dev, slots, slot_rows, part, exact=True, stream=None):
    H, nq_cap, _ = Qp.shape
    Op, Mp, Lp = part
    _chk(Op, Mp, Lp)
    check(lib().aotb_lt_attn_tc_slots_f16x2(Qp.data_ptr(), nq_cap, Kp.data_ptr(), Vp.data_ptr(), Kp.shape[1], N, 0,
                                            _counter("lt_attention_tc_slots: Tk_dev", Tk_dev), H, _p(Op), _p(Mp), _p(Lp),
                                            int(slots), int(slot_rows), (1 if exact else 0) | (4 if LT_SPIN else 0),
                                            _st(stream)), "aotb_lt_attn_tc_slots_f16x2")


def gp_attention_tc_slots(Qp, Kp, Vp, N, Tk_dev, slots, slot_rows, part, exact=True, stream=None):
    Op, Mp, Lp = part
    _chk(Op, Mp, Lp)
    check(lib().aotb_gp_attn_tc_slots_f16x2(Qp.data_ptr(), Qp.shape[1], Kp.data_ptr(), Vp.data_ptr(), Kp.shape[1], N, 0,
                                            _counter("gp_attention_tc_slots: Tk_dev", Tk_dev), Vp.shape[0] * 32, _p(Op),
                                            _p(Mp), _p(Lp), int(slots), int(slot_rows),
                                            (1 if exact else 0) | (4 if LT_SPIN else 0), _st(stream)),
          "aotb_gp_attn_tc_slots_f16x2")
```

### include/aotb200.h

```cpp
#ifndef AOTB200_H
#define AOTB200_H
#include <stddef.h>
#ifdef __cplusplus
extern "C" {
#endif

int aotb_version(void);
const char* aotb_arch(void);
const char* aotb_last_error_string(void);
unsigned long long aotb_launch_count(void);
void aotb_set_pdl(int on);
int aotb_set_conv_tiling(int mode);
int aotb_set_conv_grid_cap(int ctas);

int aotb_conv2d_nhwc_f32(const float* in, const float* w, const float* bias, const float* res, float* out,
                         int B, int H, int W, int Cin, int ldin, int Cout, int ldout, int ldres,
                         int KH, int KW, int stride, int pad, int dil, int act, void* stream);

#define AOTB_CONV_CONST_WEIGHTS 256
int aotb_conv2d_nhwc_tc(const float* in, const void* wh, const void* wl, const float* bias, const float* wscale,
                        const float* res, float* out, int B, int H, int W, int Cin, int ldin, int Cout, int ldout, int ldres,
                        int KH, int KW, int stride, int pad, int act, void* workspace, size_t workspace_bytes,
                        void* stream);

int aotb_linear_f32(const float* in, const float* wt, const float* bias, const float* res, float* out,
                    int M, int K, int ldin, int N, int ldout, int ldres, int act, void* stream);

int aotb_nchw_to_nhwc_f32(const float* in, float* out, int B, int C, int HW, void* stream);
int aotb_nhwc_to_nchw_f32(const float* in, float* out, int B, int C, int HW, void* stream);
int aotb_image_to_nhwc4_f32(const float* in, float* out, int HW, void* stream);

int aotb_maxpool3x3s2_nhwc_f32(const float* in, float* out, int B, int H, int W, int C, void* stream);

int aotb_dwconv_nhwc_f32(const float* in, const float* w, const float* bias, float* out, int B, int H, int W,
                         int C, int ldin, int ldout, int KH, int KW, int stride, int pad, int dil, int act,
                         void* stream);

int aotb_bilinear_nhwc_f32(const float* in, float* out, int B, int H, int W, int C, int Ho, int Wo,
                           int align_corners, void* stream);

int aotb_eltwise_f32(int op, const float* a, int lda, const float* b, int ldb, float* out, int ldo,
                     int rows, int cols, float scalar, void* stream);

int aotb_layernorm_f32(const float* x, int ldx, const float* gamma, const float* beta, const float* add,
                       int ldadd, float* out, int ldo, float* out2, int ldo2, int rows, int C, void* stream);

int aotb_window_attention_f32(const float* qkv, int ldqkv, const float* qkv_bias, const float* rel_bias, float* out,
                              int ldo, int H, int W, int C, int heads, int window, int shift, void* stream);

int aotb_patch_merge_f32(const float* x, int ldx, float* out, int ldo, int H, int W, int C, void* stream);

size_t aotb_groupnorm_workspace_bytes(int B, int G);
int aotb_groupnorm_nhwc_f32(const float* x, int ldx, const float* gamma, const float* beta, float* out, int ldo,
                            int B, int P, int C, int G, int act, void* workspace, void* stream);

size_t aotb_splat_workspace_bytes(int C);
int aotb_splat_attention_f32(const float* x, int ldx, int HW, int C, int radix, const float* w1, const float* b1, int inter,
                             const float* w2, const float* b2, float* att, void* workspace, void* stream);
int aotb_splat_combine_f32(const float* x, int ldx, const float* att, float* out, int ldo, int H, int W, int C, int radix,
                           int pool_stride, void* stream);
int aotb_se_gate_f32(const float* x, int ldx, int HW, int C, const float* w1, const float* b1, int inter, const float* w2,
                     const float* b2, float* gate, void* workspace, void* stream);
int aotb_gate_scale_f32(const float* x, int ldx, const float* gate, float* out, int ldo, int HW, int C, int act, void* stream);
int aotb_avgpool_nhwc_f32(const float* in, int ldin, float* out, int ldo, int B, int H, int W, int C, int k, int s, int pad,
                          int ceil_mode, int count_include_pad, void* stream);

int aotb_attention_f32(const float* Q, int ldq, const float* K, int ldk, const float* V, int ldv, float* O,
                       int ldo, int N, int Tk, const int* Tk_dev, int H, int d_qk, int d_v, float* Mout,
                       float* Lout, void* stream);
int aotb_attn_merge_f32(const float* Opart, const float* Mpart, const float* Lpart, float* O, int R, int N,
                        int H, int d_v, int ldo, void* stream);
size_t aotb_attn_merge_usage_workspace_bytes(int R);
int aotb_attn_merge_usage_f32(const float* Opart, const float* Mpart, const float* Lpart, float* O, int R, int N, int H,
                              int d_v, int ldo, float* U, int* A, const int* live, int rows, int layers, void* workspace,
                              void* stream);

int aotb_attn_merge_peers_f32(const void* const* Oparts, const void* const* Mparts, const void* const* Lparts, int ranks,
                              int splits, float* O, int N, int H, int d_v, int ldo, void* stream);

int aotb_local_attention_f32(const float* q, int ldq, const float* k, int ldk, const float* v, int ldv,
                             const float* relk_w, const float* relk_b, const float* relv, float* out, int ldo,
                             int h, int w, int H, int d_att, int d_v, void* stream);

int aotb_local_attention_tile_f32(const float* q, int ldq, const float* k, int ldk, const float* v, int ldv,
                                  const float* relk_w, const float* relk_b, const float* relv_t, float* out, int ldo,
                                  int h, int w, int H, void* stream);

int aotb_local_gated_tile_f32(const float* q, int ldq, const float* k, int ldk, const float* v, int ldv,
                              const float* relk_w, const float* relk_b, float* out, int ldo, int h, int w, void* stream);

int aotb_id_embed_f32(const float* mask, int Hm, int Wm, const float* wt, const float* bias,
                      const float* ln_gamma, const float* ln_beta, float* out, int ldo, int C, int nid,
                      int ksize, int stride, int pad, void* stream);

int aotb_id_embed_runs_f32(const float* mask, int Hm, int Wm, const float* wp, const float* bias,
                           const float* ln_gamma, const float* ln_beta, float* out, int ldo, int C, int nid,
                           int ksize, int stride, int pad, void* stream);

int aotb_logits_postproc_f32(const float* logits_nhwc, float* lowres_nchw, float* out_nchw, int h, int w,
                             int NC, int obj_num, int Ho, int Wo, int align_corners, void* stream);
int aotb_logits_argmax_f32(const float* lowres_nchw, float* label, int h, int w, int NC, int Ho, int Wo,
                           int align_corners, void* stream);
int aotb_soft_logit_aggregation_f32(const float* const* logits, int n_engines, int max_obj, float* out, int HW,
                                    void* stream);
int aotb_separate_labels_f32(const float* mask, int n_engines, int max_obj, float* out, int HW, void* stream);
int aotb_preprocess_bgr_u8(const void* img, int H, int W, const int* ix, const float* cx, const int* iy, const float* cy,
                           float* out, int Ho, int Wo, int flip, void* stream);
int aotb_label_to_u8(const float* label, void* out_u8, int n, void* stream);
int aotb_nearest_resize_f32(const float* in, float* out, int H, int W, int Ho, int Wo, void* stream);
int aotb_tta_merge_f32(const float* const* logits, const int* sizes, const int* flips, int n_augs, int NC, int H, int W,
                       int align_corners, const float* new_label, float* label, float* pred_prob, void* stream);
int aotb_tta_feedback_f32(const float* logits, int h, int w, int NC, int H, int W, int align_corners, int flip,
                          const float* new_label, float* out, int Hi, int Wi, void* stream);

int aotb_tc_pack_rows_f16x2(const float* src, int ld, void* dst, int cap, int rows, int H, int row_off,
                            const int* row_off_dev, float div, void* stream);
size_t aotb_lt_attn_tc_smem_bytes(void);
int aotb_lt_attn_tc_f16x2(const void* Qp, int Nq_cap, const void* Kp, const void* Vp, int kv_cap, int N, int Tk,
                          const int* Tk_dev, int H, float* O, int ldo, float* Opart, float* Mpart, float* Lpart,
                          int splits, int exact, float* dbg, void* stream);
int aotb_lt_attn_tc_slots_f16x2(const void* Qp, int Nq_cap, const void* Kp, const void* Vp, int kv_cap, int N, int Tk,
                                const int* Tk_dev, int H, float* Opart, float* Mpart, float* Lpart, int splits, int split_rows,
                                int exact, void* stream);

int aotb_split_rows_f16x2(const float* src, int lds, void* hi, void* lo, int ldw, int rows, int C, int row_off,
                          const int* row_off_dev, void* stream);
int aotb_split_cols_f16x2(const float* src, int lds, void* hiT, void* loT, int ldt, int rows, int C, int col_off,
                          const int* col_off_dev, void* stream);
int aotb_row_softmax_f32(float* S, int ld, int N, int cols, int Tk, const int* Tk_dev, float scale, void* stream);

int aotb_gp_attn_tc_f16x2(const void* Qp, int Nq_cap, const void* Kp, const void* Vp, int kv_cap, int N, int Tk,
                          const int* Tk_dev, int dv, float* O, int ldo, float* Opart, float* Mpart, float* Lpart,
                          int splits, int exact, void* stream);
int aotb_gp_attn_tc_slots_f16x2(const void* Qp, int Nq_cap, const void* Kp, const void* Vp, int kv_cap, int N, int Tk,
                                const int* Tk_dev, int dv, float* Opart, float* Mpart, float* Lpart, int splits, int split_rows,
                                int exact, void* stream);

int aotb_bank_append_f32(const float* src, int lds, float* bank, int ldb, int rows, int cols, int offset,
                         const int* offset_dev, void* stream);
int aotb_counter_add(int* counter, int delta, void* stream);

int aotb_bank_ring_store(const float* k_src, int ldk, int k_cols, const float* v_src, int ldv, int v_cols, int rows,
                         float* k_bank, int ldkb, float* v_bank, int ldvb, void* k_packed, void* v_packed, int cap_rows,
                         const int* write, void* stream);
int aotb_ring_advance(int* live, int* write, int rows, int cap_rows, int pinned_rows, void* stream);
int aotb_ring_select_usage(const int* live, int* write, float* U, int* A, int rows, int cap_rows, int pinned_rows,
                           void* stream);

#ifdef __cplusplus
}
#endif
#endif
```

Before: 386.5.

## Feed ResNet conv activations as pre-split fp16 planes loaded by TMA and im2col

Adds an operand-form conv path in which each tensor-core conv epilogue also writes its output as fp16 high and low planes. The next conv then loads its A operand directly with TMA, as 2D tiles for 1x1 convs or im2col tensor maps for KxK convs, instead of having producer warps gather and split fp32 activations. The engine registers these planes for the backbone buffers and skips the fp32 output where it is not needed. The aim is to remove the per-conv fp32 gather and conversion cost. In exchange it adds epilogue work (warp shuffles and extra stores), extra buffers, and Python bookkeeping keyed on tensor pointers.

```diff
diff --git a/aot_benchmark_b200/csrc/conv_tc.cu b/aot_benchmark_b200/csrc/conv_tc.cu
--- a/aot_benchmark_b200/csrc/conv_tc.cu
+++ b/aot_benchmark_b200/csrc/conv_tc.cu
@@ -39,6 +39,9 @@
     int spin;
     int const_w;
     long long* prof;
+    __half* outh;
+    __half* outl;
+    int im2col;
 };
 
 constexpr int AOTB_CONV_CONST_WEIGHTS = 256;
@@ -47,7 +50,13 @@
 
 struct RowInfo { int pix_base, iy0, ix0, valid; };
 
-template <int BN, int S, int NB>
+__device__ __forceinline__ void store_operand(const ConvTcArgs& a, size_t e, float x, float y) {
+    const __half2 h = __floats2half2_rn(x, y);
+    if (a.outh) *reinterpret_cast<__half2*>(a.outh + e) = h;
+    if (a.outl) *reinterpret_cast<__half2*>(a.outl + e) = __floats2half2_rn(x - __low2float(h), y - __high2float(h));
+}
+
+template <int BN, int S, int NB, bool OPF>
 __device__ __forceinline__ void conv_finish_tile(const ConvTcArgs& a, const uint8_t* smem, int tid, int m0, int n0, int zrank) {
     constexpr int LD = BN + 4, C4 = BN / 4, RSTEP = 256 / C4, ROWS = 128 / S, ITERS = ROWS / RSTEP;
     constexpr int B = NB < ITERS ? NB : ITERS;
@@ -84,14 +93,22 @@
             o.x = apply_act(o.x, a.act); o.y = apply_act(o.y, a.act);
             o.z = apply_act(o.z, a.act); o.w = apply_act(o.w, a.act);
             const int m = m0 + r0 + (i0 + b) * RSTEP;
-            if (m < a.M) *reinterpret_cast<float4*>(a.out + (size_t)m * a.ldout + n) = o;
+            if constexpr (OPF) {
+                if (m < a.M) {
+                    if (a.out) *reinterpret_cast<float4*>(a.out + (size_t)m * a.ldout + n) = o;
+                    store_operand(a, (size_t)m * a.Cout + n, o.x, o.y);
+                    store_operand(a, (size_t)m * a.Cout + n + 2, o.z, o.w);
+                }
+            } else if (m < a.M) {
+                *reinterpret_cast<float4*>(a.out + (size_t)m * a.ldout + n) = o;
+            }
         }
     }
 }
 
 __device__ __forceinline__ void prefetch_l1(const void* p) { asm volatile("prefetch.global.L1 [%0];" ::"l"(p)); }
 
-template <int BN, int ACT>
+template <int BN, int ACT, bool OPF>
 __device__ __forceinline__ void conv_finish_frag(const ConvTcArgs& a, float* acc, const float* bs, int m0, int n0) {
     constexpr bool ROLL = ACT == ACT_GELU || ACT == ACT_SILU;
     constexpr int G = (ROLL || BN == 256) ? 1 : 8, NG = BN / 8, PF = 8;
@@ -106,13 +123,44 @@
             if (ok[1]) prefetch_l1(res_at(1, k));
         }
     };
+    uint32_t hw[2][4], lw[2][4];
+    auto flush = [&](__half* plane, const uint32_t* w, int kb, int h) {
+        if (!plane) return;
+        const int q = lane & 3;
+        uint32_t o[4] = {0u, 0u, 0u, 0u};
+#pragma unroll
+        for (int rr = 0; rr < 4; ++rr) {
+            const int i = (q + rr) & 3, s = (q - rr) & 3;
+            const uint32_t send = i == 0 ? w[0] : i == 1 ? w[1] : i == 2 ? w[2] : w[3];
+            const uint32_t recv = __shfl_sync(0xffffffffu, send, (lane & ~3) | s);
+#pragma unroll
+            for (int t = 0; t < 4; ++t) o[t] = t == s ? recv : o[t];
+        }
+        if (ok[h])
+            *reinterpret_cast<uint4*>(plane + (size_t)(r + 8 * h) * a.Cout + n0 + 8 * (kb + q)) =
+                make_uint4(o[0], o[1], o[2], o[3]);
+    };
     auto group = [&](int k, int h, float a0, float a1, float2 rs) {
         const int n = c + 8 * k;
         const float2 b2 = *reinterpret_cast<const float2*>(bs + n), s2 = *reinterpret_cast<const float2*>(bs + BN + n);
         float ox = fmaf(a0, s2.x, b2.x), oy = fmaf(a1, s2.y, b2.y);
         ox += rs.x; oy += rs.y;
         ox = apply_act(ox, ACT); oy = apply_act(oy, ACT);
-        if (ok[h]) *reinterpret_cast<float2*>(a.out + (size_t)(r + 8 * h) * a.ldout + n0 + n) = make_float2(ox, oy);
+        if constexpr (OPF && !ROLL && BN < 256) {
+            if (ok[h] && a.out) *reinterpret_cast<float2*>(a.out + (size_t)(r + 8 * h) * a.ldout + n0 + n) = make_float2(ox, oy);
+            const __half2 hh = __floats2half2_rn(ox, oy);
+            const __half2 ll = __floats2half2_rn(ox - __low2float(hh), oy - __high2float(hh));
+            hw[h][k & 3] = *reinterpret_cast<const uint32_t*>(&hh);
+            lw[h][k & 3] = *reinterpret_cast<const uint32_t*>(&ll);
+            if ((k & 3) == 3) { flush(a.outh, hw[h], k - 3, h); flush(a.outl, lw[h], k - 3, h); }
+        } else if constexpr (OPF) {
+            if (ok[h]) {
+                if (a.out) *reinterpret_cast<float2*>(a.out + (size_t)(r + 8 * h) * a.ldout + n0 + n) = make_float2(ox, oy);
+                store_operand(a, (size_t)(r + 8 * h) * a.Cout + n0 + n, ox, oy);
+            }
+        } else if (ok[h]) {
+            *reinterpret_cast<float2*>(a.out + (size_t)(r + 8 * h) * a.ldout + n0 + n) = make_float2(ox, oy);
+        }
     };
 #pragma unroll
     for (int k = 0; k < PF; ++k) prefetch(k);
@@ -160,9 +208,9 @@
     static_assert(TOTAL <= 227 * 1024, "shared memory of one CTA");
 };
 
-template <int BN, int STAGES, bool SPLIT, bool PERSIST>
-__global__ void __launch_bounds__(384, 1)
-conv_tc_kernel(const __grid_constant__ CUtensorMap tmWh, const __grid_constant__ CUtensorMap tmWl, const ConvTcArgs a) {
+template <int BN, int STAGES, bool SPLIT, bool PERSIST, bool OPF>
+__device__ __forceinline__ void conv_tc_body(const CUtensorMap& tmWh, const CUtensorMap& tmWl, const CUtensorMap* tmAh,
+                                             const CUtensorMap* tmAl, const ConvTcArgs& a) {
     using SM = ConvSmem<BN, STAGES, SPLIT, PERSIST>;
     extern __shared__ uint8_t smem_raw[];
     uint8_t* smem = reinterpret_cast<uint8_t*>((reinterpret_cast<uintptr_t>(smem_raw) + 1023) & ~(uintptr_t)1023);
@@ -218,10 +266,12 @@
     };
 
     if (tid == 0) {
-        for (int s = 0; s < STAGES; ++s) { mbar_init(&a_full[s], 128); mbar_init(&b_full[s], 1); mbar_init(&s_free[s], 8); }
+        for (int s = 0; s < STAGES; ++s) {
+            mbar_init(&a_full[s], OPF ? 1 : 128); mbar_init(&b_full[s], 1); mbar_init(&s_free[s], 8);
+        }
         fence_mbar_init();
     }
-    if (tid >= 256) {
+    if (!OPF && tid >= 256) {
         for (int j = 0; j < min(ntc, 2); ++j) write_rows(j, tid - 256);
     }
     __syncthreads();
@@ -229,6 +279,10 @@
     if (tid == 256) {
         tma_prefetch_desc(&tmWh);
         if constexpr (SPLIT) tma_prefetch_desc(&tmWl);
+        if constexpr (OPF) {
+            tma_prefetch_desc(tmAh);
+            if constexpr (SPLIT) tma_prefetch_desc(tmAl);
+        }
         for (int g = 0; g < npre; ++g) issue_b(g);
     }
     pdl_wait();
@@ -282,11 +336,11 @@
                 asm volatile("bar.sync 1, 256;" ::: "memory");
                 const int m0 = tile_m0(j), n0 = tile_n0(j);
                 switch (a.act) {
-                    case ACT_RELU: conv_finish_frag<BN, ACT_RELU>(a, acc, bs, m0, n0); break;
-                    case ACT_GELU: conv_finish_frag<BN, ACT_GELU>(a, acc, bs, m0, n0); break;
-                    case ACT_SILU: conv_finish_frag<BN, ACT_SILU>(a, acc, bs, m0, n0); break;
-                    case ACT_RELU6: conv_finish_frag<BN, ACT_RELU6>(a, acc, bs, m0, n0); break;
-                    default: conv_finish_frag<BN, ACT_NONE>(a, acc, bs, m0, n0); break;
+                    case ACT_RELU: conv_finish_frag<BN, ACT_RELU, OPF>(a, acc, bs, m0, n0); break;
+                    case ACT_GELU: conv_finish_frag<BN, ACT_GELU, OPF>(a, acc, bs, m0, n0); break;
+                    case ACT_SILU: conv_finish_frag<BN, ACT_SILU, OPF>(a, acc, bs, m0, n0); break;
+                    case ACT_RELU6: conv_finish_frag<BN, ACT_RELU6, OPF>(a, acc, bs, m0, n0); break;
+                    default: conv_finish_frag<BN, ACT_NONE, OPF>(a, acc, bs, m0, n0); break;
                 }
                 if (tid == 0) { if (j == 0) stamp(8); stamp(9); }
             } else {
@@ -294,6 +348,29 @@
                 conv_acc_to_staging<BN>(acc, reinterpret_cast<float*>(smem), SM::STG_LD);
                 if (tid == 0) stamp(6);
             }
+        }
+    } else if constexpr (OPF) {
+        if (tid == 256) {
+#pragma unroll 1
+            for (int g = 0; g < nchk; ++g) {
+                const int s = g % STAGES, j = PERSIST ? g / nloc : 0, it = g - j * nloc;
+                if (g >= STAGES) mbar_wait_cp(&s_free[s], ((g / STAGES) - 1) & 1, a.spin);
+                if (g >= npre) issue_b(g);
+                uint8_t* Ah = smem + s * SM::STAGE_BYTES;
+                const int kc = kbeg + it, tap = kc / cpt, c0 = (kc - tap * cpt) << 6, m0 = tile_m0(j);
+                mbar_arrive_expect_tx(&a_full[s], SM::PARTS * SM::A_BYTES);
+                if (a.im2col) {
+                    const int HoWo = a.Ho * a.Wo, b = m0 / HoWo, r = m0 - b * HoWo, oy = r / a.Wo, ox = r - oy * a.Wo;
+                    const int x0 = ox * a.stride - a.pad, y0 = oy * a.stride - a.pad, ky = tap / a.KW, kx = tap - ky * a.KW;
+                    tma_load_im2col_4d(Ah, tmAh, &a_full[s], c0, x0, y0, b, kx, ky);
+                    if constexpr (SPLIT) tma_load_im2col_4d(Ah + SM::A_BYTES, tmAl, &a_full[s], c0, x0, y0, b, kx, ky);
+                } else {
+                    tma_load_2d(Ah, tmAh, &a_full[s], c0, m0);
+                    if constexpr (SPLIT) tma_load_2d(Ah + SM::A_BYTES, tmAl, &a_full[s], c0, m0);
+                }
+                if (g == 0) stamp(2);
+            }
+            stamp(5);
         }
     } else {
         const int p = tid - 256, q = p & 15, rsub = p >> 4;
@@ -404,9 +481,9 @@
         if (tid == 0) stamp(8);
         if (warp < 8) {
             const int zr = (int)blockIdx.z, m0 = tile_m0(0), n0 = tile_n0(0);
-            if (a.splits == 2) conv_finish_tile<BN, 2, 4>(a, smem, tid, m0, n0, zr);
-            else if (a.splits == 4) conv_finish_tile<BN, 4, 2>(a, smem, tid, m0, n0, zr);
-            else conv_finish_tile<BN, 8, 2>(a, smem, tid, m0, n0, zr);
+            if (a.splits == 2) conv_finish_tile<BN, 2, 4, OPF>(a, smem, tid, m0, n0, zr);
+            else if (a.splits == 4) conv_finish_tile<BN, 4, 2, OPF>(a, smem, tid, m0, n0, zr);
+            else conv_finish_tile<BN, 8, 2, OPF>(a, smem, tid, m0, n0, zr);
         }
         if (tid == 0) stamp(9);
         __syncwarp();
@@ -415,6 +492,19 @@
         prof[11] = ntc;
     }
     if (tid == 0) stamp(7);
+}
+
+template <int BN, int STAGES, bool SPLIT, bool PERSIST>
+__global__ void __launch_bounds__(384, 1)
+conv_tc_kernel(const __grid_constant__ CUtensorMap tmWh, const __grid_constant__ CUtensorMap tmWl, const ConvTcArgs a) {
+    conv_tc_body<BN, STAGES, SPLIT, PERSIST, false>(tmWh, tmWl, nullptr, nullptr, a);
+}
+
+template <int BN, int STAGES, bool SPLIT, bool PERSIST>
+__global__ void __launch_bounds__(384, 1)
+conv_tc_op_kernel(const __grid_constant__ CUtensorMap tmWh, const __grid_constant__ CUtensorMap tmWl,
+                  const __grid_constant__ CUtensorMap tmAh, const __grid_constant__ CUtensorMap tmAl, const ConvTcArgs a) {
+    conv_tc_body<BN, STAGES, SPLIT, PERSIST, true>(tmWh, tmWl, &tmAh, &tmAl, a);
 }
 
 static int make_tmap_weights(CUtensorMap* out, const void* base, int Kpad, int Cout, int BN) {
@@ -434,6 +524,54 @@
     return AOTB_OK;
 }
 
+static int make_tmap_act_2d(CUtensorMap* out, const void* base, long long rows, int C) {
+    PFN_encodeTiled fn = tensor_map_encoder();
+    if (!fn) return AOTB_ERR_CUDA;
+    cuuint64_t dims[2] = {(cuuint64_t)C, (cuuint64_t)rows};
+    cuuint64_t strides[1] = {(cuuint64_t)C * 2};
+    cuuint32_t box[2] = {64, 128};
+    cuuint32_t estr[2] = {1, 1};
+    CUresult r = fn(out, CU_TENSOR_MAP_DATA_TYPE_FLOAT16, 2, const_cast<void*>(base), dims, strides, box, estr,
+                    CU_TENSOR_MAP_INTERLEAVE_NONE, CU_TENSOR_MAP_SWIZZLE_128B, CU_TENSOR_MAP_L2_PROMOTION_L2_256B,
+                    CU_TENSOR_MAP_FLOAT_OOB_FILL_NONE);
+    if (r != CUDA_SUCCESS) {
+        set_error("cuTensorMapEncodeTiled(activations) failed (%d)", (int)r);
+        return AOTB_ERR_CUDA;
+    }
+    return AOTB_OK;
+}
+
+typedef CUresult (*PFN_encodeIm2col)(CUtensorMap*, CUtensorMapDataType, cuuint32_t, void*, const cuuint64_t*,
+                                     const cuuint64_t*, const int*, const int*, cuuint32_t, cuuint32_t, const cuuint32_t*,
+                                     CUtensorMapInterleave, CUtensorMapSwizzle, CUtensorMapL2promotion,
+                                     CUtensorMapFloatOOBfill);
+
+static int make_tmap_act_im2col(CUtensorMap* out, const void* base, int B, int H, int W, int C, int K, int stride, int pad) {
+    static PFN_encodeIm2col fn = nullptr;
+    if (!fn) {
+        void* p = nullptr;
+        cudaDriverEntryPointQueryResult qres;
+        cudaError_t e = cudaGetDriverEntryPoint("cuTensorMapEncodeIm2col", &p, cudaEnableDefault, &qres);
+        if (e != cudaSuccess || qres != cudaDriverEntryPointSuccess || !p) {
+            set_error("cuTensorMapEncodeIm2col entry point unavailable");
+            return AOTB_ERR_CUDA;
+        }
+        fn = (PFN_encodeIm2col)p;
+    }
+    cuuint64_t dims[4] = {(cuuint64_t)C, (cuuint64_t)W, (cuuint64_t)H, (cuuint64_t)B};
+    cuuint64_t strides[3] = {(cuuint64_t)C * 2, (cuuint64_t)W * C * 2, (cuuint64_t)H * W * C * 2};
+    const int lower[2] = {-pad, -pad}, upper[2] = {pad - (K - 1), pad - (K - 1)};
+    cuuint32_t estr[4] = {1, (cuuint32_t)stride, (cuuint32_t)stride, 1};
+    CUresult r = fn(out, CU_TENSOR_MAP_DATA_TYPE_FLOAT16, 4, const_cast<void*>(base), dims, strides, lower, upper, 64, 128, estr,
+                    CU_TENSOR_MAP_INTERLEAVE_NONE, CU_TENSOR_MAP_SWIZZLE_128B, CU_TENSOR_MAP_L2_PROMOTION_L2_256B,
+                    CU_TENSOR_MAP_FLOAT_OOB_FILL_NONE);
+    if (r != CUDA_SUCCESS) {
+        set_error("cuTensorMapEncodeIm2col(activations) failed (%d)", (int)r);
+        return AOTB_ERR_CUDA;
+    }
+    return AOTB_OK;
+}
+
 static int sm_count() {
     static int n = 0;
     if (n == 0) {
@@ -450,27 +588,37 @@
     return dim3(min(a.mtiles * (a.Cout / BN), cap), 1, 1);
 }
 
-template <int BN, int STAGES, bool SPLIT, bool PERSIST>
-static int launch_conv_tc_as(const CUtensorMap& th, const CUtensorMap& tl, const ConvTcArgs& a, cudaStream_t st) {
+template <int BN, int STAGES, bool SPLIT, bool PERSIST, bool OPF>
+static int launch_conv_tc_as(const CUtensorMap& th, const CUtensorMap& tl, const CUtensorMap* ta, const ConvTcArgs& a,
+                             cudaStream_t st) {
     constexpr int smem = ConvSmem<BN, STAGES, SPLIT, PERSIST>::TOTAL;
     static bool configured = false;
     if (!configured) {
-        cudaError_t e = cudaFuncSetAttribute(conv_tc_kernel<BN, STAGES, SPLIT, PERSIST>,
-                                             cudaFuncAttributeMaxDynamicSharedMemorySize, smem);
+        cudaError_t e = OPF ? cudaFuncSetAttribute(conv_tc_op_kernel<BN, STAGES, SPLIT, PERSIST>,
+                                                   cudaFuncAttributeMaxDynamicSharedMemorySize, smem)
+                            : cudaFuncSetAttribute(conv_tc_kernel<BN, STAGES, SPLIT, PERSIST>,
+                                                   cudaFuncAttributeMaxDynamicSharedMemorySize, smem);
         if (e != cudaSuccess) {
             set_error("aotb_conv2d_nhwc_tc: cudaFuncSetAttribute: %s", cudaGetErrorString(e));
             return AOTB_ERR_CUDA;
         }
         configured = true;
     }
-    launch_cluster(conv_tc_kernel<BN, STAGES, SPLIT, PERSIST>, conv_grid(a, BN), dim3(384), smem, st, a.splits, th, tl, a);
+    if constexpr (OPF)
+        launch_cluster(conv_tc_op_kernel<BN, STAGES, SPLIT, PERSIST>, conv_grid(a, BN), dim3(384), smem, st, a.splits, th, tl,
+                       ta[0], ta[1], a);
+    else
+        launch_cluster(conv_tc_kernel<BN, STAGES, SPLIT, PERSIST>, conv_grid(a, BN), dim3(384), smem, st, a.splits, th, tl, a);
     return check_launch("aotb_conv2d_nhwc_tc");
 }
 
 template <int BN, int STAGES, bool SPLIT>
-static int launch_conv_tc(const CUtensorMap& th, const CUtensorMap& tl, const ConvTcArgs& a, cudaStream_t st) {
-    return a.splits > 1 ? launch_conv_tc_as<BN, STAGES, SPLIT, false>(th, tl, a, st)
-                        : launch_conv_tc_as<BN, STAGES, SPLIT, true>(th, tl, a, st);
+static int launch_conv_tc(const CUtensorMap& th, const CUtensorMap& tl, const CUtensorMap* ta, const ConvTcArgs& a,
+                          cudaStream_t st) {
+    if (ta) return a.splits > 1 ? launch_conv_tc_as<BN, STAGES, SPLIT, false, true>(th, tl, ta, a, st)
+                                : launch_conv_tc_as<BN, STAGES, SPLIT, true, true>(th, tl, ta, a, st);
+    return a.splits > 1 ? launch_conv_tc_as<BN, STAGES, SPLIT, false, false>(th, tl, ta, a, st)
+                        : launch_conv_tc_as<BN, STAGES, SPLIT, true, false>(th, tl, ta, a, st);
 }
 
 }
@@ -490,27 +638,40 @@
     return AOTB_OK;
 }
 
-extern "C" int aotb_conv2d_nhwc_tc(const float* in, const void* wh, const void* wl, const float* bias, const float* wscale,
-                                   const float* res, float* out, int B, int H, int W, int Cin, int ldin, int Cout, int ldout, int ldres,
-                                   int KH, int KW, int stride, int pad, int act, void* workspace, size_t workspace_bytes,
-                                   void* stream) {
-    AOTB_REQUIRE(in && wh && out, "aotb_conv2d_nhwc_tc: null pointer");
-    const bool split = wl != nullptr;
+static int conv_tc_entry(const char* name, const float* in, const void* wh, const void* wl, const float* bias,
+                         const float* wscale, const float* res, float* out, int B, int H, int W, int Cin, int ldin, int Cout,
+                         int ldout, int ldres, int KH, int KW, int stride, int pad, int act, void* workspace,
+                         size_t workspace_bytes, void* stream, const void* in_h, const void* in_l, void* out_h, void* out_l) {
+    const bool split = wl != nullptr, opf = in_h != nullptr;
+    AOTB_REQUIRE((in || opf) && wh && (out || out_h || out_l), "%s: null pointer", name);
+    if (opf) {
+        AOTB_REQUIRE(Cin % 64 == 0 && ldin == Cin, "%s: the operand form needs Cin %% 64 == 0 and unsliced channels", name);
+        AOTB_REQUIRE(!split || in_l, "%s: the split kernel reads both planes of the operand form", name);
+        AOTB_REQUIRE((uintptr_t)in_h % 16 == 0 && (uintptr_t)in_l % 16 == 0, "%s: operand planes must be 16-byte aligned", name);
+        AOTB_REQUIRE(KH == KW && stride >= 1 && stride <= 8 && pad >= 0 && pad <= 127 && KH <= 128,
+                     "%s: the operand form needs a square filter, stride <= 8 and pad <= 127", name);
+    } else {
+        AOTB_REQUIRE(!in_l, "%s: in_l without in_h", name);
+        AOTB_REQUIRE(!out_h && !out_l, "%s: an operand-form output needs the operand form of the input", name);
+    }
+    AOTB_REQUIRE((uintptr_t)out_h % 4 == 0 && (uintptr_t)out_l % 4 == 0, "%s: operand planes must be 4-byte aligned", name);
     const int const_w = (act & tc::AOTB_CONV_CONST_WEIGHTS) ? 1 : 0;
     act &= ~tc::AOTB_CONV_CONST_WEIGHTS;
-    AOTB_REQUIRE(Cin % 4 == 0 && Cout % 64 == 0, "aotb_conv2d_nhwc_tc: Cin must be a multiple of 4, Cout of 64");
-    AOTB_REQUIRE(act >= aotb::ACT_NONE && act <= aotb::ACT_RELU6, "aotb_conv2d_nhwc_tc: activation %d not supported (0-4)", act);
+    AOTB_REQUIRE(Cin % 4 == 0 && Cout % 64 == 0, "%s: Cin must be a multiple of 4, Cout of 64", name);
+    AOTB_REQUIRE(act >= aotb::ACT_NONE && act <= aotb::ACT_RELU6, "%s: activation %d not supported (0-4)", name, act);
     AOTB_REQUIRE(ldin % 4 == 0 && ldout % 4 == 0 && (!res || ldres % 4 == 0) && ((uintptr_t)in % 16 == 0) &&
                      ((uintptr_t)out % 16 == 0) && (!res || (uintptr_t)res % 16 == 0) && (!bias || (uintptr_t)bias % 16 == 0) &&
                      (!wscale || (uintptr_t)wscale % 16 == 0),
-                 "aotb_conv2d_nhwc_tc: 16-byte alignment required");
-    AOTB_REQUIRE((size_t)B * H * W * ldin / 4 < 0xFFFFFFFFull, "aotb_conv2d_nhwc_tc: input larger than 2^32 float4");
+                 "%s: 16-byte alignment required", name);
+    AOTB_REQUIRE((size_t)B * H * W * ldin / 4 < 0xFFFFFFFFull, "%s: input larger than 2^32 float4", name);
     tc::ConvTcArgs a;
     a.in = in; a.bias = bias; a.wscale = wscale; a.res = res; a.out = out;
+    a.outh = (__half*)out_h; a.outl = (__half*)out_l;
+    a.im2col = !(KH == 1 && stride == 1 && pad == 0);
     a.B = B; a.H = H; a.W = W; a.Cin = Cin; a.ldin = ldin;
     a.Ho = (H + 2 * pad - KH) / stride + 1;
     a.Wo = (W + 2 * pad - KW) / stride + 1;
-    AOTB_REQUIRE(a.Ho > 0 && a.Wo > 0, "aotb_conv2d_nhwc_tc: empty output");
+    AOTB_REQUIRE(a.Ho > 0 && a.Wo > 0, "%s: empty output", name);
     a.Cout = Cout; a.ldout = ldout; a.ldres = ldres; a.KH = KH; a.KW = KW; a.stride = stride; a.pad = pad;
     a.M = B * a.Ho * a.Wo;
     a.mtiles = cdiv(a.M, 128);
@@ -520,8 +681,10 @@
     a.const_w = const_w;
     const int mt = cdiv(a.M, 128);
     int BN = 64, best_s = 1;
-    const float kGather = 2.5f, kGather1 = 2.0f;
-    if ((tc::g_conv_tiling & 1) == 0) {
+    const float kGather = 2.5f, kGather1 = 2.0f, kTma = 1.5f, kTma1 = 0.75f;
+    for (int row = 0; row < (opf ? 2 : 1) && (tc::g_conv_tiling & 1) == 0; ++row) {
+        const bool tma = row == 1;
+        const int only_s = best_s;
         float best = 1e30f;
         const int bns[3] = {256, 128, 64};
         const float t_mma[3] = {4.0f, 2.0f, 1.0f}, t_mma1[3] = {4.0f / 3, 2.0f / 3, 1.0f / 3};
@@ -529,9 +692,11 @@
         for (int bi = 0; bi < 3; ++bi) {
             const float tf = t_fin[bi] * (bi == 0 && res ? 2.0f : 1.0f);
             if (Cout % bns[bi]) continue;
-            const float tm = split ? t_mma[bi] : t_mma1[bi], tc = fmaxf(split ? kGather : kGather1, tm);
+            const float tm = split ? t_mma[bi] : t_mma1[bi];
+            const float tc = fmaxf(tma ? (split ? kTma : kTma1) : (split ? kGather : kGather1), tm);
             for (int sp = 1; sp <= 8; sp <<= 1) {
                 if (sp > a.nchunks) break;
+                if (tma && sp != only_s) continue;
                 const int ctas = mt * (Cout / bns[bi]) * sp;
                 const int slots = sp == 8 ? 128 : 132;
                 if (sp > 1 && ctas > slots) continue;
@@ -545,7 +710,8 @@
                 if (t < best) { best = t; BN = bns[bi]; best_s = sp; }
             }
         }
-    } else {
+    }
+    if (tc::g_conv_tiling & 1) {
         if (Cout % 128 == 0 && mt * (Cout / 128) >= 120) BN = 128;
         const int ctas = mt * (Cout / BN);
         if (ctas < 100 && a.nchunks >= 4) {
@@ -556,12 +722,12 @@
     const int force_bn = (tc::g_conv_tiling >> 4) & 15, force_s = (tc::g_conv_tiling >> 8) & 15;
     if (force_bn) {
         BN = 32 << force_bn;
-        AOTB_REQUIRE((BN == 64 || BN == 128 || BN == 256) && Cout % BN == 0, "aotb_conv2d_nhwc_tc: forced tile %d invalid", BN);
+        AOTB_REQUIRE((BN == 64 || BN == 128 || BN == 256) && Cout % BN == 0, "%s: forced tile %d invalid", name, BN);
     }
     a.splits = force_bn ? 1 : best_s;
     if (force_s) {
         AOTB_REQUIRE((force_s == 1 || force_s == 2 || force_s == 4 || force_s == 8) && force_s <= a.nchunks,
-                     "aotb_conv2d_nhwc_tc: forced split %d invalid", force_s);
+                     "%s: forced split %d invalid", name, force_s);
         a.splits = force_s;
     }
     a.spin = (tc::g_conv_tiling & 2) ? 1 : 0;
@@ -569,20 +735,48 @@
     if (tc::g_conv_tiling & 4) {
         const dim3 grid = tc::conv_grid(a, BN);
         const size_t need = (size_t)grid.x * grid.y * grid.z * 12 * sizeof(long long);
-        AOTB_REQUIRE(workspace && workspace_bytes >= need, "aotb_conv2d_nhwc_tc: profile mode needs %zu workspace bytes", need);
+        AOTB_REQUIRE(workspace && workspace_bytes >= need, "%s: profile mode needs %zu workspace bytes", name, need);
         a.prof = (long long*)workspace;
     }
-    CUtensorMap th, tl;
+    CUtensorMap th, tl, ta[2];
+    const CUtensorMap* tap = nullptr;
     int rc;
     if ((rc = tc::make_tmap_weights(&th, wh, K, Cout, BN)) != AOTB_OK) return rc;
+    if (opf) {
+        for (int i = 0; i < (split ? 2 : 1); ++i) {
+            const void* plane = i ? in_l : in_h;
+            rc = a.im2col ? tc::make_tmap_act_im2col(&ta[i], plane, B, H, W, Cin, KH, stride, pad)
+                          : tc::make_tmap_act_2d(&ta[i], plane, (long long)B * H * W, Cin);
+            if (rc != AOTB_OK) return rc;
+        }
+        if (!split) ta[1] = ta[0];
+        tap = ta;
+    }
     cudaStream_t st = (cudaStream_t)stream;
     if (!split) {
-        if (BN == 256) return tc::launch_conv_tc<256, 4, false>(th, th, a, st);
-        if (BN == 128) return tc::launch_conv_tc<128, 6, false>(th, th, a, st);
-        return tc::launch_conv_tc<64, 8, false>(th, th, a, st);
+        if (BN == 256) return tc::launch_conv_tc<256, 4, false>(th, th, tap, a, st);
+        if (BN == 128) return tc::launch_conv_tc<128, 6, false>(th, th, tap, a, st);
+        return tc::launch_conv_tc<64, 8, false>(th, th, tap, a, st);
     }
     if ((rc = tc::make_tmap_weights(&tl, wl, K, Cout, BN)) != AOTB_OK) return rc;
-    if (BN == 256) return tc::launch_conv_tc<256, 2, true>(th, tl, a, st);
-    if (BN == 128) return tc::launch_conv_tc<128, 3, true>(th, tl, a, st);
-    return tc::launch_conv_tc<64, 4, true>(th, tl, a, st);
-}
+    if (BN == 256) return tc::launch_conv_tc<256, 2, true>(th, tl, tap, a, st);
+    if (BN == 128) return tc::launch_conv_tc<128, 3, true>(th, tl, tap, a, st);
+    return tc::launch_conv_tc<64, 4, true>(th, tl, tap, a, st);
+}
+
+extern "C" int aotb_conv2d_nhwc_tc(const float* in, const void* wh, const void* wl, const float* bias, const float* wscale,
+                                   const float* res, float* out, int B, int H, int W, int Cin, int ldin, int Cout, int ldout, int ldres,
+                                   int KH, int KW, int stride, int pad, int act, void* workspace, size_t workspace_bytes,
+                                   void* stream) {
+    return conv_tc_entry("aotb_conv2d_nhwc_tc", in, wh, wl, bias, wscale, res, out, B, H, W, Cin, ldin, Cout, ldout, ldres, KH,
+                         KW, stride, pad, act, workspace, workspace_bytes, stream, nullptr, nullptr, nullptr, nullptr);
+}
+
+extern "C" int aotb_conv2d_nhwc_tc_op(const float* in, const void* in_h, const void* in_l, const void* wh, const void* wl,
+                                      const float* bias, const float* wscale, const float* res, float* out, void* out_h,
+                                      void* out_l, int B, int H, int W, int Cin, int ldin, int Cout, int ldout, int ldres,
+                                      int KH, int KW, int stride, int pad, int act, void* workspace, size_t workspace_bytes,
+                                      void* stream) {
+    return conv_tc_entry("aotb_conv2d_nhwc_tc_op", in, wh, wl, bias, wscale, res, out, B, H, W, Cin, ldin, Cout, ldout, ldres,
+                         KH, KW, stride, pad, act, workspace, workspace_bytes, stream, in_h, in_l, out_h, out_l);
+}
diff --git a/aot_benchmark_b200/csrc/tc_common.cuh b/aot_benchmark_b200/csrc/tc_common.cuh
--- a/aot_benchmark_b200/csrc/tc_common.cuh
+++ b/aot_benchmark_b200/csrc/tc_common.cuh
@@ -78,6 +78,15 @@
     asm volatile(
         "cp.async.bulk.tensor.3d.shared::cluster.global.mbarrier::complete_tx::bytes [%0], [%1, {%3, %4, %5}], [%2];"
         ::"r"(smem_u32(dst)), "l"(reinterpret_cast<uint64_t>(m)), "r"(smem_u32(bar)), "r"(c0), "r"(c1), "r"(c2)
+        : "memory");
+}
+__device__ __forceinline__ void tma_load_im2col_4d(void* dst, const CUtensorMap* m, uint64_t* bar, int c, int x, int y, int n,
+                                                   int off_x, int off_y) {
+    asm volatile(
+        "cp.async.bulk.tensor.4d.shared::cluster.global.im2col.mbarrier::complete_tx::bytes [%0], [%1, {%3, %4, %5, %6}], [%2], "
+        "{%7, %8};"
+        ::"r"(smem_u32(dst)), "l"(reinterpret_cast<uint64_t>(m)), "r"(smem_u32(bar)), "r"(c), "r"(x), "r"(y), "r"(n),
+        "h"((unsigned short)off_x), "h"((unsigned short)off_y)
         : "memory");
 }
 __device__ __forceinline__ void fence_proxy_async() { asm volatile("fence.proxy.async.shared::cta;" ::: "memory"); }
diff --git a/aot_benchmark_b200/engine.py b/aot_benchmark_b200/engine.py
--- a/aot_benchmark_b200/engine.py
+++ b/aot_benchmark_b200/engine.py
@@ -229,6 +229,7 @@
         self.H, self.W = H, W
         dev = plan.device
         self.bufs = {}
+        self.opbufs = {}
         self.dev = dev
 
     def _buf(self, key, shape):
@@ -236,6 +237,17 @@
         if b is None or tuple(b.shape) != tuple(shape):
             b = torch.empty(shape, dtype=torch.float32, device=self.dev)
             self.bufs[key] = b
+        return b
+
+    def _opbuf(self, key, shape, fp32=True):
+        b = self._buf(key, shape)
+        if not b.is_cuda:
+            return b
+        pl = self.opbufs.get(key)
+        if pl is None or pl[2] is not b:
+            hi = torch.empty(shape, dtype=torch.float16, device=self.dev)
+            pl = self.opbufs[key] = (hi, torch.empty_like(hi), b)
+        ops.operand_form(b, pl[0], pl[1], fp32=fp32)
         return b
 
     @staticmethod
@@ -284,22 +296,25 @@
         c1 = self._buf("stem", (1, h1, w1, 64))
         ops.conv2d(x, e.stem.w, e.stem.b, c1, KH=7, KW=7, stride=2, pad=3, act=A_RELU, stream=st)
         h, w = self._osz(h1, 3, 2, 1), self._osz(w1, 3, 2, 1)
-        cur = self._buf("pool", (1, h, w, 64))
+        cur = self._opbuf("pool", (1, h, w, 64))
         ops.maxpool3x3s2(c1, cur, stream=st)
+        if cur.is_cuda:
+            pool_h, pool_l, _ = self.opbufs["pool"]
+            ops.split_rows(cur.view(-1, 64), pool_h.view(-1, 64), pool_l.view(-1, 64), stream=st)
         feats = []
         for si, blocks in enumerate(e.stages):
             for bi, b in enumerate(blocks):
                 ho, wo = self._osz(h, 3, b.stride, 1), self._osz(w, 3, b.stride, 1)
-                t1 = self._buf(f"s{si}b{bi}t1", (1, h, w, b.c1.cout))
+                t1 = self._opbuf(f"s{si}b{bi}t1", (1, h, w, b.c1.cout), fp32=False)
                 ops.conv2d(cur, b.c1.w, b.c1.b, t1, act=A_RELU, stream=st)
-                t2 = self._buf(f"s{si}b{bi}t2", (1, ho, wo, b.c2.cout))
+                t2 = self._opbuf(f"s{si}b{bi}t2", (1, ho, wo, b.c2.cout), fp32=False)
                 ops.conv2d(t1, b.c2.w, b.c2.b, t2, KH=3, KW=3, stride=b.stride, pad=1, act=A_RELU, stream=st)
                 if b.down is not None:
                     res = self._buf(f"s{si}ds", (1, ho, wo, b.down.cout))
                     ops.conv2d(cur, b.down.w, b.down.b, res, stride=b.stride, stream=st)
                 else:
                     res = cur
-                out = self._buf(f"s{si}o{bi % 2}", (1, ho, wo, b.c3.cout))
+                out = self._opbuf(f"s{si}o{bi % 2}", (1, ho, wo, b.c3.cout))
                 ops.conv2d(t2, b.c3.w, b.c3.b, out, res=res, act=A_RELU, stream=st)
                 cur, h, w = out, ho, wo
             feats.append(cur)
diff --git a/aot_benchmark_b200/ops.py b/aot_benchmark_b200/ops.py
--- a/aot_benchmark_b200/ops.py
+++ b/aot_benchmark_b200/ops.py
@@ -2,6 +2,7 @@
 
 import contextlib
 import os
+import weakref
 
 import torch
 
@@ -80,6 +81,22 @@
     if ws is None:
         ws = _TC_WS[device] = torch.zeros(1 << 20, dtype=torch.uint8, device=device)
     return ws
+
+
+_OPERAND = {}
+
+
+def operand_form(buf, hi, lo, fp32=True):
+    for k in [k for k, v in _OPERAND.items() if v[0]() is None]:
+        del _OPERAND[k]
+    _OPERAND[buf.data_ptr()] = (weakref.ref(buf), hi, lo, fp32)
+
+
+def _operand_of(t):
+    e = _OPERAND.get(t.data_ptr())
+    if e is None or e[0]() is None or tuple(e[1].shape) != tuple(t.shape) or not t.is_contiguous():
+        return None
+    return e
 
 
 def register_tc_weights(w, wh, wl, wscale=None):
@@ -132,12 +149,52 @@
     return out
 
 
+def _half_plane(t, shape, what):
+    if t is None:
+        return None
+    if t.dtype != torch.float16 or not t.is_cuda or not t.is_contiguous() or tuple(t.shape) != tuple(shape):
+        raise AotbError(f"conv2d_tc_op: {what} must be a contiguous fp16 CUDA tensor of shape {tuple(shape)}")
+    return t.data_ptr()
+
+
+def conv2d_tc_op(x, xh, xl, wh, wl, bias, out, outh=None, outl=None, res=None, KH=1, KW=1, stride=1, pad=0, act=ACT_NONE,
+                 stream=None, wscale=None, const_w=False):
+    _chk(x, bias, out, res, wscale)
+    src = x if x is not None else xh
+    B, H, W, Cin = src.shape
+    Cout = wh.shape[0]
+    Ho, Wo = (H + 2 * pad - KH) // stride + 1, (W + 2 * pad - KW) // stride + 1
+    oshape = (B, Ho, Wo, Cout)
+    ldin = _nhwc_ld(x) if x is not None else Cin
+    ldout = _nhwc_ld(out) if out is not None else Cout
+    ws = _tc_workspace(src.device)
+    with _ConvProbe(2.0 * B * Ho * Wo * Cout * KH * KW * Cin, stream):
+        check(lib().aotb_conv2d_nhwc_tc_op(_p(x), _half_plane(xh, src.shape, "xh"), _half_plane(xl, src.shape, "xl"),
+                                           wh.data_ptr(), _p(wl), _p(bias), _p(wscale), _p(res), _p(out),
+                                           _half_plane(outh, oshape, "outh"), _half_plane(outl, oshape, "outl"), B, H, W,
+                                           Cin, ldin, Cout, ldout, _nhwc_ld(res) if res is not None else 0, KH, KW, stride,
+                                           pad, act | (CONV_CONST_WEIGHTS if const_w else 0), ws.data_ptr(), ws.numel(),
+                                           _st(stream)), "aotb_conv2d_nhwc_tc_op")
+    return out
+
+
 def conv2d(x, w, bias, out, res=None, KH=1, KW=1, stride=1, pad=0, dil=1, act=ACT_NONE, stream=None):
     if CONV_IMPL == "tc" and dil == 1:
         t = _TC_WEIGHTS.get(w.data_ptr())
         if t is not None:
-            return conv2d_tc(x, t[0], None if _PRECISION == "fp16" else t[1], bias, out, res=res, KH=KH, KW=KW, stride=stride, pad=pad, act=act,
+            wl = None if _PRECISION == "fp16" else t[1]
+            ix, io = _operand_of(x), _operand_of(out)
+            if ix is not None and x.shape[3] % 64 == 0 and KH == KW:
+                return conv2d_tc_op(None, ix[1], ix[2] if wl is not None else None, t[0], wl, bias,
+                                    out if io is None or io[3] else None, io[1] if io else None,
+                                    io[2] if io and wl is not None else None, res=res, KH=KH, KW=KW, stride=stride,
+                                    pad=pad, act=act, stream=stream, wscale=t[2], const_w=True)
+            if io is not None:
+                raise AotbError("conv2d: the output has an operand form, which needs the operand form of the input")
+            return conv2d_tc(x, t[0], wl, bias, out, res=res, KH=KH, KW=KW, stride=stride, pad=pad, act=act,
                              stream=stream, wscale=t[2], const_w=True)
+    if CONV_IMPL == "tc" and _operand_of(out) is not None:
+        raise AotbError("conv2d: the output has an operand form, which only the tensor-core conv writes")
     _chk(x, w, bias, out, res)
     B, H, W, Cin = x.shape
     Cout = w.shape[1]
diff --git a/include/aotb200.h b/include/aotb200.h
--- a/include/aotb200.h
+++ b/include/aotb200.h
@@ -22,6 +22,10 @@
                         const float* res, float* out, int B, int H, int W, int Cin, int ldin, int Cout, int ldout, int ldres,
                         int KH, int KW, int stride, int pad, int act, void* workspace, size_t workspace_bytes,
                         void* stream);
+int aotb_conv2d_nhwc_tc_op(const float* in, const void* in_h, const void* in_l, const void* wh, const void* wl,
+                           const float* bias, const float* wscale, const float* res, float* out, void* out_h, void* out_l,
+                           int B, int H, int W, int Cin, int ldin, int Cout, int ldout, int ldres, int KH, int KW, int stride,
+                           int pad, int act, void* workspace, size_t workspace_bytes, void* stream);
 
 int aotb_linear_f32(const float* in, const float* wt, const float* bias, const float* res, float* out,
                     int M, int K, int ldin, int N, int ldout, int ldres, int act, void* stream);
```

Result: faster. 413.0, median of 6 (+6.8%).
